# Transconnectome/multimodal_neuroimage

Hardware: NVIDIA B200
Metric: window_attn_fwd_bwd (higher is better)
Workload: dtype bf16

## Files before the change

### include/mmn_b200.h

```cpp
#ifndef MMN_B200_H_
#define MMN_B200_H_

#include <stddef.h>
#include <stdint.h>

#ifdef __cplusplus
extern "C" {
#endif

#define MMN_ABI_VERSION 6
#define MMN_WINATTN_WORK_BYTES 2048

enum { MMN_OK = 0, MMN_ERR_INVALID = -1, MMN_ERR_UNSUPPORTED = -2, MMN_ERR_CUDA = -3 };
enum { MMN_DT_F32 = 0, MMN_DT_BF16 = 1 };
enum { MMN_SCORE_SCALED = 0,
       MMN_SCORE_COSINE = 1 };
enum { MMN_MASK_NONE = 0,
       MMN_MASK_SHIFT = 1,
       MMN_MASK_TENSOR = 2,
       MMN_MASK_FUTURE = 3 };
enum { MMN_PATH_AUTO = 0, MMN_PATH_GENERIC = 1, MMN_PATH_TCGEN05 = 2 };

typedef struct mmn_winattn_desc {
  int32_t ndim;
  int32_t batch;
  int32_t grid[3];
  int32_t window[3];
  int32_t shift[3];
  int32_t num_heads, head_dim;
  int32_t score_kind;
  int32_t mask_kind;
  int32_t mask_windows;
  int32_t io_dtype;
  int32_t path;
  float scale;
  float dropout_p;
  uint64_t seed, offset;
  int64_t q_row_stride, k_row_stride, v_row_stride, o_row_stride;
  int64_t do_row_stride, dq_row_stride, dk_row_stride, dv_row_stride;
  int32_t deterministic;
  const uint64_t* rng;
} mmn_winattn_desc;

typedef struct mmn_mha_desc {
  int32_t tgt_len, src_len, batch, num_heads, head_dim;
  int32_t mask_kind;
  int32_t mask_diagonal;
  int32_t io_dtype, path;
  float scale;
  float dropout_p;
  uint64_t seed, offset;
  int64_t q_stride_t, q_stride_b, k_stride_t, k_stride_b, v_stride_t, v_stride_b;
  int64_t o_stride_t, o_stride_b;
  int64_t do_stride_t, do_stride_b, dq_stride_t, dq_stride_b, dk_stride_t, dk_stride_b;
  int64_t dv_stride_t, dv_stride_b;
  const uint64_t* rng;
} mmn_mha_desc;

int mmn_abi_version(void);
const char* mmn_last_error(void);
const char* mmn_winattn_path(const mmn_winattn_desc* desc);
const char* mmn_mha_path(const mmn_mha_desc* desc);
uint64_t mmn_launch_count(void);

int mmn_winattn_fwd(const mmn_winattn_desc* desc, const void* q, const void* k, const void* v,
                    const float* bias, const float* head_scale, const float* mask,
                    void* out, float* lse, void* workspace, int device, void* stream);

size_t mmn_winattn_bwd_workspace_bytes(const mmn_winattn_desc* desc);
int mmn_winattn_bwd(const mmn_winattn_desc* desc, const void* q, const void* k, const void* v,
                    const float* bias, const float* head_scale, const float* mask,
                    const void* out, const float* lse, const void* dout,
                    void* dq, void* dk, void* dv, float* dbias, float* dhead_scale, float* dcolsum,
                    float* workspace, int device, void* stream);

int mmn_mha_fwd(const mmn_mha_desc* desc, const void* q, const void* k, const void* v,
                const float* mask, void* out, float* lse, int device, void* stream);

int mmn_mha_bwd(const mmn_mha_desc* desc, const void* q, const void* k, const void* v,
                const float* mask, const void* out, const float* lse, const void* dout,
                void* dq, void* dk, void* dv, float* workspace ,
                int device, void* stream);

int mmn_mha_avg_weights(const mmn_mha_desc* desc, const void* q, const void* k, const float* mask,
                        const float* lse, float* avg, int device, void* stream);

size_t mmn_colsum_workspace_bytes(int64_t rows, int32_t cols);
int mmn_colsum(const void* x, int io_dtype, int64_t rows, int32_t cols, int64_t row_stride, float* out,
               float* workspace, int deterministic, int device, void* stream);

int mmn_cpb_bias_fwd(const float* coords, const float* w1, const float* b1, const float* w2, const int64_t* index,
                     int32_t T, int32_t n_in, int32_t J, int32_t num_heads, int32_t NN,
                     float* tab16, float* bias, int device, void* stream);
int mmn_cpb_bias_bwd(const float* coords, const float* w1, const float* b1, const float* w2, const int64_t* index,
                     const int32_t* inv_perm, const int32_t* inv_offsets,
                     const float* tab16, const float* dbias, int32_t T, int32_t n_in, int32_t J, int32_t num_heads, int32_t NN,
                     float* scratch, float* dw1, float* db1, float* dw2, int device, void* stream);

int mmn_table_bias_fwd(const float* table, const int64_t* index, int32_t T, int32_t num_heads, int32_t NN, float* bias,
                       int device, void* stream);
int mmn_table_bias_bwd(const float* dbias, const int64_t* index, const int32_t* inv_perm, const int32_t* inv_offsets, int32_t T,
                       int32_t num_heads, int32_t NN, float* dtable, int device, void* stream);

enum { MMN_ACT_NONE = 0, MMN_ACT_RELU = 1, MMN_ACT_GELU = 2 };
int mmn_linear_supported(int io_dtype, int64_t rows, int32_t in_features, int32_t out_features, int64_t ld_x, int64_t ld_y);
int mmn_linear_fwd(const void* x, const void* w, const float* bias, void* y, void* y_pre, int act, int io_dtype, int64_t rows,
                   int32_t in_features, int32_t out_features, int64_t ld_x, int64_t ld_y, int device, void* stream);
int mmn_linear_bwd_supported(int io_dtype, int64_t rows, int32_t in_features, int32_t out_features,
                             int64_t ld_dy, int64_t ld_x, int64_t ld_dx);
size_t mmn_linear_bwd_workspace_bytes(int64_t rows, int32_t in_features, int32_t out_features, int deterministic);
int mmn_linear_bwd(const void* dy, const void* x, const void* w, void* dx, float* dw, float* db, void* workspace,
                   const void* act_aux, int64_t ld_aux, int act, int io_dtype, int64_t rows, int32_t in_features,
                   int32_t out_features, int64_t ld_dy, int64_t ld_x, int64_t ld_dx, int deterministic, int device, void* stream);

enum { MMN_LN_PRE = 0, MMN_LN_POST = 1 };
int mmn_layernorm_supported(int32_t cols);
int mmn_layernorm_fwd(const void* resid, int resid_dtype, const void* delta, int delta_dtype, const float* gamma, const float* beta,
                      float eps, int mode, void* out_sum, int sum_dtype, void* out_norm, int norm_dtype, float* mean, float* rstd,
                      int64_t rows, int32_t cols, int device, void* stream);
size_t mmn_layernorm_bwd_workspace_bytes(int64_t rows, int32_t cols);
int mmn_layernorm_bwd(const void* g_sum, int gs_dtype, const void* g_norm, int gn_dtype, const void* x, int x_dtype,
                      const float* gamma, const float* mean, const float* rstd, int mode, void* d_resid, int dr_dtype,
                      void* d_delta, int dd_dtype, float* dgamma, float* dbeta, float* workspace, int deterministic,
                      int64_t rows, int32_t cols, int device, void* stream);

#ifdef __cplusplus
}
#endif
#endif
```

### multimodal_neuroimage_b200/_lib.py

```python
from __future__ import annotations

import ctypes as C
import os
import shutil
import subprocess
import threading

PKG_DIR = os.path.dirname(os.path.abspath(__file__))
ROOT = os.path.dirname(PKG_DIR)
CSRC = os.path.join(PKG_DIR, "csrc")
LIB_PATH = os.environ.get("MMN_LIB") or os.path.join(PKG_DIR, "libmmn_b200.so")
SOURCES = {"mmn_abi.cu": ["generic_launch.h", "attn_generic.cuh", "winattn_tc.h", "dropout_rng.cuh", "zero_fill.h"],
           "generic_launch.cu": ["generic_launch.h", "attn_generic.cuh", "dropout_rng.cuh", "zero_fill.h"],
           "winattn_tc.cu": ["winattn_tc.h", "winattn_tc_fwd.cuh", "winattn_tc_bwd.cuh", "tc_window.cuh", "tc_sched.cuh", "tc_common.cuh",
                             "zero_fill.h"],
           "linbwd_tc.cu": ["winattn_tc.h", "tc_window.cuh", "tc_common.cuh"],
           "gemm_tc.cu": ["winattn_tc.h", "tc_window.cuh", "tc_common.cuh"],
           "mha_tc.cu": ["winattn_tc.h", "tc_window.cuh", "tc_common.cuh", "dropout_rng.cuh"],
           "layernorm.cu": ["generic_launch.h", "attn_generic.cuh", "dropout_rng.cuh"],
           "cpb_bias.cu": ["generic_launch.h", "attn_generic.cuh", "dropout_rng.cuh", "zero_fill.h"]}
NVCC_FLAGS = ["-gencode", "arch=compute_100a,code=sm_100a", "-lineinfo", "-O3", "-std=c++17",
              "-Xcompiler", "-fPIC"]
if os.environ.get("MMN_BUILD_TRACE"):
    NVCC_FLAGS.append("-DMMN_TC_TRACING")
NVCC_FLAGS += os.environ.get("MMN_NVCC_DEFINES", "").split()

DT_F32, DT_BF16 = 0, 1
SCORE_SCALED, SCORE_COSINE = 0, 1
MASK_NONE, MASK_SHIFT, MASK_TENSOR, MASK_FUTURE = 0, 1, 2, 3
PATH_AUTO, PATH_GENERIC, PATH_TCGEN05 = 0, 1, 2
ACT_NONE, ACT_RELU, ACT_GELU = 0, 1, 2
LN_PRE, LN_POST = 0, 1
ABI_VERSION = 6
WINATTN_WORK_BYTES = 2048

EXPORTS = ["mmn_abi_version", "mmn_last_error", "mmn_winattn_path", "mmn_mha_path", "mmn_launch_count",
           "mmn_winattn_fwd", "mmn_winattn_bwd", "mmn_winattn_bwd_workspace_bytes", "mmn_mha_fwd", "mmn_mha_bwd", "mmn_mha_avg_weights",
           "mmn_colsum", "mmn_colsum_workspace_bytes", "mmn_layernorm_bwd_workspace_bytes",
           "mmn_linear_supported", "mmn_linear_fwd", "mmn_linear_bwd", "mmn_linear_bwd_supported", "mmn_linear_bwd_workspace_bytes",
           "mmn_cpb_bias_fwd", "mmn_cpb_bias_bwd", "mmn_table_bias_fwd", "mmn_table_bias_bwd", "mmn_layernorm_supported", "mmn_layernorm_fwd", "mmn_layernorm_bwd"]


class WinAttnDesc(C.Structure):
    _fields_ = [("ndim", C.c_int32), ("batch", C.c_int32),
                ("grid", C.c_int32 * 3), ("window", C.c_int32 * 3), ("shift", C.c_int32 * 3),
                ("num_heads", C.c_int32), ("head_dim", C.c_int32),
                ("score_kind", C.c_int32), ("mask_kind", C.c_int32), ("mask_windows", C.c_int32),
                ("io_dtype", C.c_int32), ("path", C.c_int32),
                ("scale", C.c_float), ("dropout_p", C.c_float),
                ("seed", C.c_uint64), ("offset", C.c_uint64),
                ("q_row_stride", C.c_int64), ("k_row_stride", C.c_int64), ("v_row_stride", C.c_int64),
                ("o_row_stride", C.c_int64), ("do_row_stride", C.c_int64), ("dq_row_stride", C.c_int64),
                ("dk_row_stride", C.c_int64), ("dv_row_stride", C.c_int64), ("deterministic", C.c_int32),
                ("rng", C.c_void_p)]


class MhaDesc(C.Structure):
    _fields_ = [("tgt_len", C.c_int32), ("src_len", C.c_int32), ("batch", C.c_int32),
                ("num_heads", C.c_int32), ("head_dim", C.c_int32),
                ("mask_kind", C.c_int32), ("mask_diagonal", C.c_int32),
                ("io_dtype", C.c_int32), ("path", C.c_int32),
                ("scale", C.c_float), ("dropout_p", C.c_float),
                ("seed", C.c_uint64), ("offset", C.c_uint64)] + \
               [(f"{t}_stride_{a}", C.c_int64) for t in ("q", "k", "v", "o", "do", "dq", "dk", "dv") for a in ("t", "b")] + \
               [("rng", C.c_void_p)]


def _stamp(files) -> float:
    return max(os.path.getmtime(f) for f in files if os.path.exists(f))


def build(force: bool = False, verbose: bool = False) -> str:
    nvcc = shutil.which("nvcc") or "/usr/local/cuda/bin/nvcc"
    if not os.path.exists(nvcc):
        raise RuntimeError("nvcc not found: cannot build libmmn_b200.so")
    objdir = os.path.join(PKG_DIR, "build")
    os.makedirs(objdir, exist_ok=True)
    header = os.path.join(ROOT, "include", "mmn_b200.h")
    objs, procs = [], []
    for src, deps in SOURCES.items():
        obj = os.path.join(objdir, src.replace(".cu", ".o"))
        objs.append(obj)
        stamp = _stamp([os.path.join(CSRC, src), header] + [os.path.join(CSRC, d) for d in deps])
        if force or os.environ.get("MMN_BUILD_TRACE") or os.environ.get("MMN_NVCC_DEFINES") or not os.path.exists(obj) or os.path.getmtime(obj) < stamp:
            cmd = [nvcc] + NVCC_FLAGS + ["-c", os.path.join(CSRC, src), "-o", obj]
            if verbose:
                print(" ".join(cmd), flush=True)
            procs.append((src, subprocess.Popen(cmd, stdout=subprocess.PIPE, stderr=subprocess.STDOUT, text=True)))
    for src, p in procs:
        out, _ = p.communicate()
        if p.returncode != 0:
            raise RuntimeError(f"nvcc failed on {src}:\n{out}")
    if procs or not os.path.exists(LIB_PATH) or os.path.getmtime(LIB_PATH) < _stamp(objs):
        cmd = [nvcc, "-shared", "-o", LIB_PATH + ".tmp"] + objs
        if verbose:
            print(" ".join(cmd), flush=True)
        res = subprocess.run(cmd, capture_output=True, text=True)
        if res.returncode != 0:
            raise RuntimeError("link failed:\n" + res.stdout + res.stderr)
        os.replace(LIB_PATH + ".tmp", LIB_PATH)
    return LIB_PATH


_lock = threading.Lock()
_lib = None


def load() -> C.CDLL:
    global _lib
    with _lock:
        if _lib is not None:
            return _lib
        if not os.path.exists(LIB_PATH):
            raise RuntimeError(f"{LIB_PATH} is missing: run `python -c 'import __graft_entry__ as g; g.build()'` "
                               "(multimodal_neuroimage_b200 has no CPU or PyTorch fallback)")
        lib = C.CDLL(LIB_PATH)
        vp, fp = C.c_void_p, C.c_void_p
        lib.mmn_abi_version.restype = C.c_int
        lib.mmn_last_error.restype = C.c_char_p
        lib.mmn_launch_count.restype = C.c_uint64
        lib.mmn_winattn_path.restype = C.c_char_p
        lib.mmn_winattn_path.argtypes = [C.POINTER(WinAttnDesc)]
        lib.mmn_mha_path.restype = C.c_char_p
        lib.mmn_mha_path.argtypes = [C.POINTER(MhaDesc)]
        lib.mmn_winattn_fwd.restype = C.c_int
        lib.mmn_winattn_fwd.argtypes = [C.POINTER(WinAttnDesc), vp, vp, vp, fp, fp, fp, vp, fp, vp, C.c_int, vp]
        lib.mmn_winattn_bwd_workspace_bytes.restype = C.c_size_t
        lib.mmn_winattn_bwd_workspace_bytes.argtypes = [C.POINTER(WinAttnDesc)]
        lib.mmn_winattn_bwd.restype = C.c_int
        lib.mmn_winattn_bwd.argtypes = [C.POINTER(WinAttnDesc), vp, vp, vp, fp, fp, fp, vp, fp, vp, vp, vp, vp, fp, fp, fp, fp,
                                        C.c_int, vp]
        lib.mmn_mha_fwd.restype = C.c_int
        lib.mmn_mha_fwd.argtypes = [C.POINTER(MhaDesc), vp, vp, vp, fp, vp, fp, C.c_int, vp]
        lib.mmn_mha_bwd.restype = C.c_int
        lib.mmn_mha_bwd.argtypes = [C.POINTER(MhaDesc), vp, vp, vp, fp, vp, fp, vp, vp, vp, vp, fp, C.c_int, vp]
        lib.mmn_mha_avg_weights.restype = C.c_int
        lib.mmn_mha_avg_weights.argtypes = [C.POINTER(MhaDesc), vp, vp, fp, fp, fp, C.c_int, vp]
        lib.mmn_colsum.restype = C.c_int
        lib.mmn_colsum.argtypes = [vp, C.c_int, C.c_int64, C.c_int32, C.c_int64, fp, fp, C.c_int, C.c_int, vp]
        lib.mmn_colsum_workspace_bytes.restype = C.c_size_t
        lib.mmn_colsum_workspace_bytes.argtypes = [C.c_int64, C.c_int32]
        lib.mmn_cpb_bias_fwd.restype = C.c_int
        lib.mmn_cpb_bias_fwd.argtypes = [fp, fp, fp, fp, vp, C.c_int32, C.c_int32, C.c_int32, C.c_int32, C.c_int32, fp, fp, C.c_int, vp]
        lib.mmn_table_bias_fwd.restype = C.c_int
        lib.mmn_table_bias_fwd.argtypes = [fp, vp, C.c_int32, C.c_int32, C.c_int32, fp, C.c_int, vp]
        lib.mmn_table_bias_bwd.restype = C.c_int
        lib.mmn_table_bias_bwd.argtypes = [fp, vp, vp, vp, C.c_int32, C.c_int32, C.c_int32, fp, C.c_int, vp]
        lib.mmn_cpb_bias_bwd.restype = C.c_int
        lib.mmn_cpb_bias_bwd.argtypes = [fp, fp, fp, fp, vp, vp, vp, fp, fp, C.c_int32, C.c_int32, C.c_int32, C.c_int32, C.c_int32,
                                         fp, fp, fp, fp, C.c_int, vp]
        lib.mmn_linear_bwd_supported.restype = C.c_int
        lib.mmn_linear_bwd_supported.argtypes = [C.c_int, C.c_int64, C.c_int32, C.c_int32, C.c_int64, C.c_int64, C.c_int64]
        lib.mmn_linear_bwd_workspace_bytes.restype = C.c_size_t
        lib.mmn_linear_bwd_workspace_bytes.argtypes = [C.c_int64, C.c_int32, C.c_int32, C.c_int]
        lib.mmn_linear_bwd.restype = C.c_int
        lib.mmn_linear_bwd.argtypes = [vp, vp, vp, vp, fp, fp, vp, vp, C.c_int64, C.c_int, C.c_int, C.c_int64, C.c_int32, C.c_int32,
                                       C.c_int64, C.c_int64, C.c_int64, C.c_int, C.c_int, vp]
        lib.mmn_linear_supported.restype = C.c_int
        lib.mmn_linear_supported.argtypes = [C.c_int, C.c_int64, C.c_int32, C.c_int32, C.c_int64, C.c_int64]
        lib.mmn_linear_fwd.restype = C.c_int
        lib.mmn_linear_fwd.argtypes = [vp, vp, fp, vp, vp, C.c_int, C.c_int, C.c_int64, C.c_int32, C.c_int32, C.c_int64, C.c_int64,
                                       C.c_int, vp]
        lib.mmn_layernorm_supported.restype = C.c_int
        lib.mmn_layernorm_supported.argtypes = [C.c_int32]
        lib.mmn_layernorm_fwd.restype = C.c_int
        lib.mmn_layernorm_fwd.argtypes = [vp, C.c_int, vp, C.c_int, fp, fp, C.c_float, C.c_int, vp, C.c_int, vp, C.c_int, fp, fp,
                                          C.c_int64, C.c_int32, C.c_int, vp]
        lib.mmn_layernorm_bwd.restype = C.c_int
        lib.mmn_layernorm_bwd.argtypes = [vp, C.c_int, vp, C.c_int, vp, C.c_int, fp, fp, fp, C.c_int, vp, C.c_int, vp, C.c_int, fp, fp,
                                          fp, C.c_int, C.c_int64, C.c_int32, C.c_int, vp]
        lib.mmn_layernorm_bwd_workspace_bytes.restype = C.c_size_t
        lib.mmn_layernorm_bwd_workspace_bytes.argtypes = [C.c_int64, C.c_int32]
        if lib.mmn_abi_version() != ABI_VERSION:
            raise RuntimeError("libmmn_b200.so ABI version mismatch")
        _lib = lib
        return lib


def check(rc: int, what: str) -> None:
    if rc != 0:
        msg = load().mmn_last_error().decode("utf-8", "replace")
        raise RuntimeError(f"{what} failed (code {rc}): {msg}")


def launch_count() -> int:
    return int(load().mmn_launch_count())
```

### multimodal_neuroimage_b200/csrc/mmn_abi.cu

```cuda
#include <atomic>
#include <cstdarg>
#include <cstdio>
#include <cstring>

#include "../../include/mmn_b200.h"
#include "generic_launch.h"
#include "zero_fill.h"
#include "winattn_tc.h"

namespace {

thread_local char g_err[512] = "";
std::atomic<uint64_t> g_launches{0};

int fail(int code, const char* fmt, ...) {
  va_list ap;
  va_start(ap, fmt);
  vsnprintf(g_err, sizeof(g_err), fmt, ap);
  va_end(ap);
  return code;
}

struct DeviceGuard {
  int prev = -1;
  bool ok = false;
  explicit DeviceGuard(int dev) {
    if (cudaGetDevice(&prev) != cudaSuccess) { cudaGetLastError(); return; }
    if (dev != prev && cudaSetDevice(dev) != cudaSuccess) { cudaGetLastError(); return; }
    ok = true;
  }
  ~DeviceGuard() { if (ok && prev >= 0) cudaSetDevice(prev); }
};

int finish(cudaError_t e, int launches, const char* what) {
  g_launches.fetch_add((uint64_t)launches, std::memory_order_relaxed);
  if (e != cudaSuccess) return fail(MMN_ERR_CUDA, "%s: %s", what, cudaGetErrorString(e));
  return MMN_OK;
}

int validate_win(const mmn_winattn_desc* d) {
  if (!d) return fail(MMN_ERR_INVALID, "null descriptor");
  if (d->ndim < 1 || d->ndim > 3) return fail(MMN_ERR_INVALID, "ndim %d not in 1..3", d->ndim);
  if (d->batch < 1 || d->num_heads < 1 || d->head_dim < 1) return fail(MMN_ERR_INVALID, "batch/heads/head_dim must be positive");
  for (int a = 0; a < d->ndim; ++a) {
    if (d->window[a] < 1 || d->grid[a] < 1 || d->grid[a] % d->window[a] != 0)
      return fail(MMN_ERR_INVALID, "axis %d: window %d does not divide grid %d", a, d->window[a], d->grid[a]);
    if (d->shift[a] < 0 || d->shift[a] >= d->window[a])
      return fail(MMN_ERR_INVALID, "axis %d: shift %d not in [0, window %d)", a, d->shift[a], d->window[a]);
  }
  if (d->score_kind != MMN_SCORE_SCALED && d->score_kind != MMN_SCORE_COSINE) return fail(MMN_ERR_INVALID, "bad score_kind");
  if (d->mask_kind != MMN_MASK_NONE && d->mask_kind != MMN_MASK_SHIFT && d->mask_kind != MMN_MASK_TENSOR)
    return fail(MMN_ERR_INVALID, "bad mask_kind %d for window attention", d->mask_kind);
  if (d->mask_kind == MMN_MASK_TENSOR && d->mask_windows < 1) return fail(MMN_ERR_INVALID, "mask_windows must be >= 1");
  if (d->io_dtype != MMN_DT_F32 && d->io_dtype != MMN_DT_BF16) return fail(MMN_ERR_INVALID, "bad io_dtype");
  if (d->dropout_p < 0.f || d->dropout_p >= 1.f) return fail(MMN_ERR_INVALID, "dropout_p must be in [0,1)");
  if (d->head_dim > 128) return fail(MMN_ERR_UNSUPPORTED, "head_dim %d > 128", d->head_dim);
  return MMN_OK;
}

int validate_mha(const mmn_mha_desc* d) {
  if (!d) return fail(MMN_ERR_INVALID, "null descriptor");
  if (d->tgt_len < 1 || d->src_len < 1 || d->batch < 1 || d->num_heads < 1 || d->head_dim < 1)
    return fail(MMN_ERR_INVALID, "sizes must be positive");
  if (d->mask_kind != MMN_MASK_NONE && d->mask_kind != MMN_MASK_FUTURE && d->mask_kind != MMN_MASK_TENSOR)
    return fail(MMN_ERR_INVALID, "bad mask_kind %d for multi-head attention", d->mask_kind);
  if (d->io_dtype != MMN_DT_F32 && d->io_dtype != MMN_DT_BF16) return fail(MMN_ERR_INVALID, "bad io_dtype");
  if (d->dropout_p < 0.f || d->dropout_p >= 1.f) return fail(MMN_ERR_INVALID, "dropout_p must be in [0,1)");
  if (d->head_dim > 128) return fail(MMN_ERR_UNSUPPORTED, "head_dim %d > 128", d->head_dim);
  return MMN_OK;
}

mmn::GenericProblem problem_from(const mmn_winattn_desc* d, const float* bias, const float* head_scale, const float* mask) {
  mmn::GenericProblem P{};
  P.kind = 0;
  for (int a = 0; a < 3; ++a) { P.grid[a] = 1; P.win[a] = 1; P.shift[a] = 0; P.nwin[a] = 1; }
  for (int a = 0; a < d->ndim; ++a) {
    int t = 3 - d->ndim + a;
    P.grid[t] = d->grid[a]; P.win[t] = d->window[a]; P.shift[t] = d->shift[a]; P.nwin[t] = d->grid[a] / d->window[a];
  }
  P.nW = P.nwin[0] * P.nwin[1] * P.nwin[2];
  P.nq = P.nk = P.win[0] * P.win[1] * P.win[2];
  P.d = d->head_dim; P.nH = d->num_heads;
  P.n_items = d->batch * P.nW * P.nH;
  P.q_s0 = d->q_row_stride; P.k_s0 = d->k_row_stride; P.v_s0 = d->v_row_stride; P.o_s0 = d->o_row_stride;
  P.do_s0 = d->do_row_stride; P.dq_s0 = d->dq_row_stride; P.dk_s0 = d->dk_row_stride; P.dv_s0 = d->dv_row_stride;
  P.cosine = d->score_kind == MMN_SCORE_COSINE;
  P.mask_kind = d->mask_kind; P.mask_windows = d->mask_windows > 0 ? d->mask_windows : 1;
  P.scale = d->scale; P.dropout_p = d->dropout_p; P.seed = d->seed; P.offset = d->offset;
  P.drop = mmn::make_dropout(d->dropout_p, d->seed, d->offset);
  P.rng = reinterpret_cast<const unsigned long long*>(d->rng);
  P.bias = bias; P.head_scale = head_scale; P.mask = mask;
  return P;
}

mmn::GenericProblem problem_from(const mmn_mha_desc* d, const float* mask) {
  mmn::GenericProblem P{};
  P.kind = 1;
  for (int a = 0; a < 3; ++a) { P.grid[a] = 1; P.win[a] = 1; P.shift[a] = 0; P.nwin[a] = 1; }
  P.nW = 1;
  P.nq = d->tgt_len; P.nk = d->src_len; P.d = d->head_dim; P.nH = d->num_heads;
  P.n_items = d->batch * d->num_heads;
  P.q_s0 = d->q_stride_t; P.q_s1 = d->q_stride_b; P.k_s0 = d->k_stride_t; P.k_s1 = d->k_stride_b;
  P.v_s0 = d->v_stride_t; P.v_s1 = d->v_stride_b; P.o_s0 = d->o_stride_t; P.o_s1 = d->o_stride_b;
  P.do_s0 = d->do_stride_t; P.do_s1 = d->do_stride_b; P.dq_s0 = d->dq_stride_t; P.dq_s1 = d->dq_stride_b;
  P.dk_s0 = d->dk_stride_t; P.dk_s1 = d->dk_stride_b; P.dv_s0 = d->dv_stride_t; P.dv_s1 = d->dv_stride_b;
  P.cosine = 0;
  P.mask_kind = d->mask_kind; P.mask_diag = d->mask_diagonal; P.mask_windows = 1;
  P.scale = d->scale; P.dropout_p = d->dropout_p; P.seed = d->seed; P.offset = d->offset;
  P.drop = mmn::make_dropout(d->dropout_p, d->seed, d->offset);
  P.rng = reinterpret_cast<const unsigned long long*>(d->rng);
  P.mask = mask;
  return P;
}

bool have_device() {
  int n = 0;
  if (cudaGetDeviceCount(&n) != cudaSuccess) { cudaGetLastError(); return false; }
  return n > 0;
}

}

extern "C" {

int mmn_abi_version(void) { return MMN_ABI_VERSION; }
const char* mmn_last_error(void) { return g_err; }
uint64_t mmn_launch_count(void) { return g_launches.load(std::memory_order_relaxed); }

const char* mmn_winattn_path(const mmn_winattn_desc* d) {
  if (validate_win(d) != MMN_OK) return "invalid";
  if (d->path == MMN_PATH_GENERIC) return "generic";
  return mmn::tc::fwd_why_not(d) == nullptr ? "tcgen05" : "generic";
}

const char* mmn_mha_path(const mmn_mha_desc* d) {
  if (validate_mha(d) != MMN_OK) return "invalid";
  if (d->path == MMN_PATH_GENERIC) return "generic";
  return mmn::tc::mha_why_not(d, false) == nullptr ? "tcgen05" : "generic";
}

int mmn_winattn_fwd(const mmn_winattn_desc* d, const void* q, const void* k, const void* v, const float* bias,
                    const float* head_scale, const float* mask, void* out, float* lse, void* workspace, int device,
                    void* stream) {
  int rc = validate_win(d);
  if (rc) return rc;
  if (!q || !k || !v || !out || !lse || !workspace) return fail(MMN_ERR_INVALID, "null tensor pointer");
  if (d->score_kind == MMN_SCORE_COSINE && !head_scale) return fail(MMN_ERR_INVALID, "cosine attention needs head_scale");
  if (d->mask_kind == MMN_MASK_TENSOR && !mask) return fail(MMN_ERR_INVALID, "MMN_MASK_TENSOR needs a mask");
  if (!have_device()) return fail(MMN_ERR_CUDA, "no CUDA device: libmmn_b200 has no CPU path");
  DeviceGuard g(device);
  if (!g.ok) return fail(MMN_ERR_CUDA, "cannot select device %d", device);
  cudaStream_t st = (cudaStream_t)stream;
  const char* why = mmn::tc::fwd_why_not(d);
  bool tc_ok = why == nullptr;
  if (d->path == MMN_PATH_TCGEN05 && !tc_ok) return fail(MMN_ERR_UNSUPPORTED, "shape not supported by the tcgen05 path: %s", why);
  if (d->path != MMN_PATH_GENERIC && tc_ok) {
    rc = mmn::tc::winattn_fwd(d, q, k, v, bias, head_scale, mask, out, lse, workspace, st, g_err, sizeof(g_err));
    if (rc == MMN_OK) g_launches.fetch_add(1, std::memory_order_relaxed);
    return rc;
  }
  int n = 0;
  cudaError_t e = mmn::generic_fwd(problem_from(d, bias, head_scale, mask), d->io_dtype, q, k, v, out, lse, st, &n);
  return finish(e, n, "attn_fwd_generic");
}

size_t mmn_winattn_bwd_workspace_bytes(const mmn_winattn_desc* d) {
  if (validate_win(d) != MMN_OK) return 0;
  const mmn::GenericProblem P = problem_from(d, nullptr, nullptr, nullptr);
  const size_t base = mmn::generic_bwd_workspace_floats(P, false) * sizeof(float);
  size_t bytes = base > MMN_WINATTN_WORK_BYTES ? base : MMN_WINATTN_WORK_BYTES;
  if (!d->deterministic) return bytes;
  const size_t det = d->path != MMN_PATH_GENERIC && mmn::tc::bwd_why_not(d) == nullptr ? mmn::tc::bwd_det_workspace_bytes(d)
                                                                                      : mmn::generic_bwd_workspace_floats(P, true) * sizeof(float);
  return det > bytes ? det : bytes;
}

int mmn_winattn_bwd(const mmn_winattn_desc* d, const void* q, const void* k, const void* v, const float* bias,
                    const float* head_scale, const float* mask, const void* out, const float* lse, const void* dout,
                    void* dq, void* dk, void* dv, float* dbias, float* dhead_scale, float* dcolsum, float* workspace,
                    int device, void* stream) {
  int rc = validate_win(d);
  if (rc) return rc;
  if (!q || !k || !v || !lse || !dout || !dq || !dk || !dv || !workspace) return fail(MMN_ERR_INVALID, "null tensor pointer");
  if (d->score_kind == MMN_SCORE_COSINE && !head_scale) return fail(MMN_ERR_INVALID, "cosine attention needs head_scale");
  if (d->mask_kind == MMN_MASK_TENSOR && !mask) return fail(MMN_ERR_INVALID, "MMN_MASK_TENSOR needs a mask");
  if (!have_device()) return fail(MMN_ERR_CUDA, "no CUDA device: libmmn_b200 has no CPU path");
  DeviceGuard g(device);
  if (!g.ok) return fail(MMN_ERR_CUDA, "cannot select device %d", device);
  cudaStream_t st = (cudaStream_t)stream;
  const char* why = mmn::tc::bwd_why_not(d);
  bool tc_ok = why == nullptr;
  if (d->path == MMN_PATH_TCGEN05 && !tc_ok) return fail(MMN_ERR_UNSUPPORTED, "shape not supported by the tcgen05 backward path: %s", why);
  if (d->path != MMN_PATH_GENERIC && tc_ok) {
    int n = 0;
    rc = mmn::tc::winattn_bwd(d, q, k, v, bias, head_scale, mask, out, lse, dout, dq, dk, dv, dbias, dhead_scale, dcolsum, workspace, st, g_err, sizeof(g_err), &n);
    g_launches.fetch_add((uint64_t)n, std::memory_order_relaxed);
    return rc;
  }
  mmn::GenericProblem P = problem_from(d, bias, head_scale, mask);
  int n = 0;
  cudaError_t e = mmn::generic_bwd(P, d->io_dtype, q, k, v, lse, dout, dq, dk, dv, bias ? dbias : nullptr,
                                 P.cosine ? dhead_scale : nullptr, workspace, dcolsum, d->deterministic != 0, st, &n);
  return finish(e, n, "attn_bwd_generic");
}

int mmn_mha_fwd(const mmn_mha_desc* d, const void* q, const void* k, const void* v, const float* mask, void* out,
                float* lse, int device, void* stream) {
  int rc = validate_mha(d);
  if (rc) return rc;
  if (!q || !k || !v || !out || !lse) return fail(MMN_ERR_INVALID, "null tensor pointer");
  if (d->mask_kind == MMN_MASK_TENSOR && !mask) return fail(MMN_ERR_INVALID, "MMN_MASK_TENSOR needs a mask");
  if (!have_device()) return fail(MMN_ERR_CUDA, "no CUDA device: libmmn_b200 has no CPU path");
  DeviceGuard g(device);
  if (!g.ok) return fail(MMN_ERR_CUDA, "cannot select device %d", device);
  int n = 0;
  const char* why = mmn::tc::mha_why_not(d, false);
  if (d->path == MMN_PATH_TCGEN05 && why) return fail(MMN_ERR_UNSUPPORTED, "shape not supported by the tcgen05 MHA path: %s", why);
  if (d->path != MMN_PATH_GENERIC && !why) {
    rc = mmn::tc::mha_fwd(d, q, k, v, mask, out, lse, (cudaStream_t)stream, g_err, sizeof(g_err), &n);
    g_launches.fetch_add((uint64_t)n, std::memory_order_relaxed);
    return rc;
  }
  cudaError_t e = mmn::generic_fwd(problem_from(d, mask), d->io_dtype, q, k, v, out, lse, (cudaStream_t)stream, &n);
  return finish(e, n, "attn_fwd_generic");
}

int mmn_mha_bwd(const mmn_mha_desc* d, const void* q, const void* k, const void* v, const float* mask, const void* out,
                const float* lse, const void* dout, void* dq, void* dk, void* dv, float* workspace, int device,
                void* stream) {
  int rc = validate_mha(d);
  if (rc) return rc;
  if (!q || !k || !v || !lse || !dout || !dq || !dk || !dv || !workspace) return fail(MMN_ERR_INVALID, "null tensor pointer");
  if (d->mask_kind == MMN_MASK_TENSOR && !mask) return fail(MMN_ERR_INVALID, "MMN_MASK_TENSOR needs a mask");
  if (!have_device()) return fail(MMN_ERR_CUDA, "no CUDA device: libmmn_b200 has no CPU path");
  DeviceGuard g(device);
  if (!g.ok) return fail(MMN_ERR_CUDA, "cannot select device %d", device);
  int n = 0;
  const char* why = mmn::tc::mha_why_not(d, true);
  if (d->path == MMN_PATH_TCGEN05 && why) return fail(MMN_ERR_UNSUPPORTED, "shape not supported by the tcgen05 MHA backward path: %s", why);
  if (d->path != MMN_PATH_GENERIC && !why) {
    rc = mmn::tc::mha_bwd(d, q, k, v, mask, out, lse, dout, dq, dk, dv, workspace, (cudaStream_t)stream, g_err, sizeof(g_err), &n);
    g_launches.fetch_add((uint64_t)n, std::memory_order_relaxed);
    return rc;
  }
  cudaError_t e = mmn::generic_bwd(problem_from(d, mask), d->io_dtype, q, k, v, lse, dout, dq, dk, dv, nullptr, nullptr, workspace,
                                 nullptr, false, (cudaStream_t)stream, &n);
  return finish(e, n, "attn_bwd_generic");
}

int mmn_mha_avg_weights(const mmn_mha_desc* d, const void* q, const void* k, const float* mask, const float* lse,
                        float* avg, int device, void* stream) {
  int rc = validate_mha(d);
  if (rc) return rc;
  if (!q || !k || !lse || !avg) return fail(MMN_ERR_INVALID, "null tensor pointer");
  if (!have_device()) return fail(MMN_ERR_CUDA, "no CUDA device: libmmn_b200 has no CPU path");
  DeviceGuard g(device);
  if (!g.ok) return fail(MMN_ERR_CUDA, "cannot select device %d", device);
  int n = 0;
  cudaError_t e = mmn::generic_avg_weights(problem_from(d, mask), d->io_dtype, d->batch, q, k, lse, avg, (cudaStream_t)stream, &n);
  return finish(e, n, "mha_avg_weights_generic");
}

size_t mmn_colsum_workspace_bytes(int64_t rows, int32_t cols) {
  if (rows < 1 || cols < 8 || cols % 8 != 0 || cols > 2048) return 0;
  return mmn::colsum_workspace_floats(rows, cols) * sizeof(float);
}

int mmn_colsum(const void* x, int io_dtype, int64_t rows, int32_t cols, int64_t row_stride, float* out, float* workspace,
               int deterministic, int device, void* stream) {
  if (!x || !out || rows < 0 || cols < 1) return fail(MMN_ERR_INVALID, "bad colsum arguments");
  if (deterministic && !workspace) return fail(MMN_ERR_INVALID, "deterministic colsum needs a workspace");
  if (io_dtype != MMN_DT_F32 && io_dtype != MMN_DT_BF16) return fail(MMN_ERR_INVALID, "bad io_dtype");
  if (cols % 8 != 0 || cols > 2048) return fail(MMN_ERR_UNSUPPORTED, "colsum needs cols %% 8 == 0 and cols <= 2048 (got %d)", cols);
  if (!have_device()) return fail(MMN_ERR_CUDA, "no CUDA device: libmmn_b200 has no CPU path");
  DeviceGuard g(device);
  if (!g.ok) return fail(MMN_ERR_CUDA, "cannot select device %d", device);
  if (rows == 0) return MMN_OK;
  int n = 0;
  cudaError_t e = mmn::colsum(io_dtype, x, rows, cols, row_stride, out, deterministic ? workspace : nullptr, (cudaStream_t)stream, &n);
  return finish(e, n, "colsum_kernel");
}

static int cpb_check(int T, int n_in, int J, int nH, int NN) {
  if (T < 1 || n_in < 1 || n_in > 3 || J < 1 || nH < 1 || nH > 64 || NN < 1) return fail(MMN_ERR_INVALID, "bad cpb_bias sizes");
  if ((long long)T * nH > 12288) return fail(MMN_ERR_UNSUPPORTED, "cpb_bias: T * num_heads = %lld > 12288", (long long)T * nH);
  if (mmn::cpb_bwd_smem_bytes(T) > 227 * 1024) return fail(MMN_ERR_UNSUPPORTED, "cpb_bias: table of %d entries exceeds the backward kernel's shared memory", T);
  if (!have_device()) return fail(MMN_ERR_CUDA, "no CUDA device: libmmn_b200 has no CPU path");
  return MMN_OK;
}

int mmn_table_bias_fwd(const float* table, const int64_t* index, int32_t T, int32_t nH, int32_t NN, float* bias, int device, void* stream) {
  if (!table || !index || !bias) return fail(MMN_ERR_INVALID, "null tensor pointer");
  if (T < 1 || nH < 1 || NN < 1) return fail(MMN_ERR_INVALID, "bad bias table dimensions");
  if (!have_device()) return fail(MMN_ERR_CUDA, "no CUDA device: libmmn_b200 has no CPU path");
  DeviceGuard g(device);
  if (!g.ok) return fail(MMN_ERR_CUDA, "cannot select device %d", device);
  int n = 0;
  cudaError_t e = mmn::table_bias_fwd(table, (const long long*)index, nH, NN, bias, (cudaStream_t)stream, &n);
  return finish(e, n, "table_bias_fwd");
}

int mmn_table_bias_bwd(const float* dbias, const int64_t* index, const int32_t* inv_perm, const int32_t* inv_offsets, int32_t T, int32_t nH,
                       int32_t NN, float* dtable, int device, void* stream) {
  if (!dbias || !index || !dtable) return fail(MMN_ERR_INVALID, "null tensor pointer");
  if (!inv_perm != !inv_offsets) return fail(MMN_ERR_INVALID, "inv_perm and inv_offsets go together");
  if (T < 1 || nH < 1 || NN < 1) return fail(MMN_ERR_INVALID, "bad bias table dimensions");
  if (!have_device()) return fail(MMN_ERR_CUDA, "no CUDA device: libmmn_b200 has no CPU path");
  DeviceGuard g(device);
  if (!g.ok) return fail(MMN_ERR_CUDA, "cannot select device %d", device);
  int n = 0;
  cudaError_t e = mmn::table_bias_bwd(dbias, (const long long*)index, inv_perm, inv_offsets, T, nH, NN, dtable, (cudaStream_t)stream, &n);
  return finish(e, n, "table_bias_bwd");
}

int mmn_cpb_bias_fwd(const float* coords, const float* w1, const float* b1, const float* w2, const int64_t* index, int32_t T,
                     int32_t n_in, int32_t J, int32_t nH, int32_t NN, float* tab16, float* bias, int device, void* stream) {
  if (!coords || !w1 || !b1 || !w2 || !index || !tab16 || !bias) return fail(MMN_ERR_INVALID, "null tensor pointer");
  int rc = cpb_check(T, n_in, J, nH, NN);
  if (rc) return rc;
  DeviceGuard g(device);
  if (!g.ok) return fail(MMN_ERR_CUDA, "cannot select device %d", device);
  int n = 0;
  cudaError_t e = mmn::cpb_bias_fwd(coords, w1, b1, w2, (const long long*)index, T, n_in, J, nH, NN, tab16, bias, (cudaStream_t)stream, &n);
  return finish(e, n, "cpb_bias_fwd");
}

int mmn_cpb_bias_bwd(const float* coords, const float* w1, const float* b1, const float* w2, const int64_t* index,
                     const int32_t* inv_perm, const int32_t* inv_offsets,
                     const float* tab16, const float* dbias, int32_t T, int32_t n_in, int32_t J, int32_t nH, int32_t NN,
                     float* scratch, float* dw1, float* db1, float* dw2, int device, void* stream) {
  if (!coords || !w1 || !b1 || !w2 || !index || !tab16 || !dbias || !scratch || !dw1 || !db1 || !dw2)
    return fail(MMN_ERR_INVALID, "null tensor pointer");
  if (!inv_perm != !inv_offsets) return fail(MMN_ERR_INVALID, "inv_perm and inv_offsets go together");
  int rc = cpb_check(T, n_in, J, nH, NN);
  if (rc) return rc;
  DeviceGuard g(device);
  if (!g.ok) return fail(MMN_ERR_CUDA, "cannot select device %d", device);
  int n = 0;
  cudaError_t e = mmn::cpb_bias_bwd(coords, w1, b1, w2, (const long long*)index, inv_perm, inv_offsets, tab16, dbias, T, n_in, J, nH, NN,
                                    scratch, dw1, db1, dw2, (cudaStream_t)stream, &n);
  return finish(e, n, "cpb_bias_bwd");
}

int mmn_linear_supported(int io_dtype, int64_t rows, int32_t in_features, int32_t out_features, int64_t ld_x, int64_t ld_y) {
  return have_device() && mmn::tc::linear_why_not(io_dtype, rows, in_features, out_features, ld_x, ld_y) == nullptr;
}

int mmn_linear_fwd(const void* x, const void* w, const float* bias, void* y, void* y_pre, int act, int io_dtype, int64_t rows,
                   int32_t in_features, int32_t out_features, int64_t ld_x, int64_t ld_y, int device, void* stream) {
  if (!x || !w || !y) return fail(MMN_ERR_INVALID, "null tensor pointer");
  if (act != MMN_ACT_NONE && act != MMN_ACT_RELU && act != MMN_ACT_GELU) return fail(MMN_ERR_INVALID, "bad activation %d", act);
  if (y_pre && act == MMN_ACT_NONE) return fail(MMN_ERR_INVALID, "y_pre only makes sense with an activation");
  if (!have_device()) return fail(MMN_ERR_CUDA, "no CUDA device: libmmn_b200 has no CPU path");
  const char* why = mmn::tc::linear_why_not(io_dtype, rows, in_features, out_features, ld_x, ld_y);
  if (why) return fail(MMN_ERR_UNSUPPORTED, "shape not supported by the tensor-core projection: %s", why);
  DeviceGuard g(device);
  if (!g.ok) return fail(MMN_ERR_CUDA, "cannot select device %d", device);
  int n = 0;
  int rc = mmn::tc::linear_fwd(x, w, bias, y, y_pre, act, rows, in_features, out_features, ld_x, ld_y, (cudaStream_t)stream, g_err,
                               sizeof(g_err), &n);
  g_launches.fetch_add((uint64_t)n, std::memory_order_relaxed);
  return rc;
}

static bool linbwd_fused_ok(int io_dtype, int64_t rows, int32_t in_features, int32_t out_features, int64_t ld_dy, int64_t ld_x,
                            int64_t ld_dx) {
  return mmn::tc::linbwd_why_not(io_dtype, rows, in_features, out_features, ld_dy, ld_x, ld_dx) == nullptr;
}

int mmn_linear_bwd_supported(int io_dtype, int64_t rows, int32_t in_features, int32_t out_features, int64_t ld_dy, int64_t ld_x,
                             int64_t ld_dx) {
  if (!have_device()) return 0;
  if (linbwd_fused_ok(io_dtype, rows, in_features, out_features, ld_dy, ld_x, ld_dx)) return 1;
  return mmn::tc::linear_why_not(io_dtype, rows, in_features, out_features, ld_x, ld_dy) == nullptr && ld_dx % 8 == 0;
}

size_t mmn_linear_bwd_workspace_bytes(int64_t rows, int32_t in_features, int32_t out_features, int deterministic) {
  const size_t a = mmn::tc::linbwd_workspace_bytes(out_features);
  const size_t b = mmn::tc::linear_wgrad_workspace_bytes(rows, in_features, out_features);
  size_t bytes = a > b ? a : b;
  if (deterministic && rows > 0 && out_features >= 8) {
    const size_t c = mmn::colsum_workspace_floats(rows, out_features < 2048 ? out_features : 2048) * sizeof(float);
    if (c > bytes) bytes = c;
  }
  return bytes;
}

int mmn_linear_bwd(const void* dy, const void* x, const void* w, void* dx, float* dw, float* db, void* workspace,
                   const void* act_aux, int64_t ld_aux, int act, int io_dtype, int64_t rows, int32_t in_features,
                   int32_t out_features, int64_t ld_dy, int64_t ld_x, int64_t ld_dx, int deterministic, int device, void* stream) {
  if (!dy || !w || !workspace || (!dx && !dw)) return fail(MMN_ERR_INVALID, "null tensor pointer");
  if (dw && !x) return fail(MMN_ERR_INVALID, "dw needs x");
  if (act != MMN_ACT_NONE && act != MMN_ACT_RELU && act != MMN_ACT_GELU) return fail(MMN_ERR_INVALID, "bad activation %d", act);
  if (act != MMN_ACT_NONE && (!act_aux || ld_aux % 8 || reinterpret_cast<uintptr_t>(act_aux) % 16))
    return fail(MMN_ERR_INVALID, "activation gradient needs a 16-byte aligned act'(pre) tensor");
  if (!have_device()) return fail(MMN_ERR_CUDA, "no CUDA device: libmmn_b200 has no CPU path");
  if (!mmn_linear_bwd_supported(io_dtype, rows, in_features, out_features, ld_dy, ld_x ? ld_x : in_features, ld_dx ? ld_dx : in_features))
    return fail(MMN_ERR_UNSUPPORTED, "shape not supported by the tensor-core projection backward (bf16, widths multiples of 32)");
  DeviceGuard g(device);
  if (!g.ok) return fail(MMN_ERR_CUDA, "cannot select device %d", device);
  cudaStream_t st = (cudaStream_t)stream;
  int n = 0, rc;
  if (dx && dw && act == MMN_ACT_NONE && linbwd_fused_ok(io_dtype, rows, in_features, out_features, ld_dy, ld_x, ld_dx)) {
    rc = mmn::tc::linbwd(dy, x, w, dx, dw, db, (float*)workspace, rows, in_features, out_features, ld_dy, ld_x, ld_dx, st, g_err,
                         sizeof(g_err), &n);
  } else {
    rc = mmn::tc::linear_bwd_general(dy, x, w, dx, dw, (float*)workspace, act_aux, ld_aux,
                                     act != MMN_ACT_NONE ? 3 : 0, rows, in_features, out_features, ld_dy,
                                     ld_x, ld_dx, st, g_err, sizeof(g_err), &n);
    if (rc == MMN_OK && db) {
      cudaError_t e = mmn::zero_words_async(db, (size_t)out_features, st);
      for (int c0 = 0; e == cudaSuccess && c0 < out_features; c0 += 2048)
        e = mmn::colsum(MMN_DT_BF16, static_cast<const uint16_t*>(dy) + c0, rows, out_features - c0 < 2048 ? out_features - c0 : 2048, ld_dy,
                        db + c0, deterministic ? static_cast<float*>(workspace) : nullptr, st, &n);
      if (e != cudaSuccess) { g_launches.fetch_add((uint64_t)n, std::memory_order_relaxed); return finish(e, 0, "colsum_kernel"); }
    }
  }
  g_launches.fetch_add((uint64_t)n, std::memory_order_relaxed);
  return rc;
}

int mmn_layernorm_supported(int32_t cols) { return have_device() && mmn::layernorm_supported(cols); }

static bool ln_dt_ok(int dt) { return dt == MMN_DT_F32 || dt == MMN_DT_BF16; }

int mmn_layernorm_fwd(const void* resid, int resid_dtype, const void* delta, int delta_dtype, const float* gamma, const float* beta,
                      float eps, int mode, void* out_sum, int sum_dtype, void* out_norm, int norm_dtype, float* mean, float* rstd,
                      int64_t rows, int32_t cols, int device, void* stream) {
  if ((!resid && !delta) || !gamma || !mean || !rstd || (!out_sum && !out_norm)) return fail(MMN_ERR_INVALID, "null tensor pointer");
  if (mode != MMN_LN_PRE && mode != MMN_LN_POST) return fail(MMN_ERR_INVALID, "bad layernorm mode %d", mode);
  if (mode == MMN_LN_POST && !delta) return fail(MMN_ERR_INVALID, "MMN_LN_POST normalises delta: it cannot be null");
  if (!ln_dt_ok(resid_dtype) || !ln_dt_ok(delta_dtype) || !ln_dt_ok(sum_dtype) || !ln_dt_ok(norm_dtype)) return fail(MMN_ERR_INVALID, "bad dtype");
  if (rows < 0) return fail(MMN_ERR_INVALID, "negative row count");
  if (!mmn::layernorm_supported(cols)) return fail(MMN_ERR_UNSUPPORTED, "layernorm: cols = %d (even, <= 1536)", cols);
  if (!have_device()) return fail(MMN_ERR_CUDA, "no CUDA device: libmmn_b200 has no CPU path");
  DeviceGuard g(device);
  if (!g.ok) return fail(MMN_ERR_CUDA, "cannot select device %d", device);
  if (rows == 0) return MMN_OK;
  int n = 0;
  cudaError_t e = mmn::layernorm_fwd(resid, resid_dtype, delta, delta_dtype, gamma, beta, eps, mode, out_sum, sum_dtype, out_norm, norm_dtype,
                                     mean, rstd, rows, cols, (cudaStream_t)stream, &n);
  return finish(e, n, "ln_fwd_kernel");
}

size_t mmn_layernorm_bwd_workspace_bytes(int64_t rows, int32_t cols) {
  if (rows < 1 || !mmn::layernorm_supported(cols)) return 0;
  return mmn::layernorm_bwd_workspace_floats(rows, cols) * sizeof(float);
}

int mmn_layernorm_bwd(const void* g_sum, int gs_dtype, const void* g_norm, int gn_dtype, const void* x, int x_dtype, const float* gamma,
                      const float* mean, const float* rstd, int mode, void* d_resid, int dr_dtype, void* d_delta, int dd_dtype,
                      float* dgamma, float* dbeta, float* workspace, int deterministic, int64_t rows, int32_t cols, int device,
                      void* stream) {
  if ((!g_sum && !g_norm) || !x || !gamma || !mean || !rstd) return fail(MMN_ERR_INVALID, "null tensor pointer");
  if (deterministic && (dgamma || dbeta) && !workspace) return fail(MMN_ERR_INVALID, "deterministic layernorm backward needs a workspace");
  if (mode != MMN_LN_PRE && mode != MMN_LN_POST) return fail(MMN_ERR_INVALID, "bad layernorm mode %d", mode);
  if (!ln_dt_ok(gs_dtype) || !ln_dt_ok(gn_dtype) || !ln_dt_ok(x_dtype) || !ln_dt_ok(dr_dtype) || !ln_dt_ok(dd_dtype)) return fail(MMN_ERR_INVALID, "bad dtype");
  if (!mmn::layernorm_supported(cols)) return fail(MMN_ERR_UNSUPPORTED, "layernorm: cols = %d (even, <= 1536)", cols);
  if (!have_device()) return fail(MMN_ERR_CUDA, "no CUDA device: libmmn_b200 has no CPU path");
  DeviceGuard g(device);
  if (!g.ok) return fail(MMN_ERR_CUDA, "cannot select device %d", device);
  if (rows <= 0) return MMN_OK;
  int n = 0;
  cudaError_t e = mmn::layernorm_bwd(g_sum, gs_dtype, g_norm, gn_dtype, x, x_dtype, gamma, mean, rstd, mode, d_resid, dr_dtype, d_delta,
                                     dd_dtype, dgamma, dbeta, deterministic ? workspace : nullptr, rows, cols, (cudaStream_t)stream, &n);
  return finish(e, n, "ln_bwd_kernel");
}

}
```

### multimodal_neuroimage_b200/csrc/tc_sched.cuh

```cuda
#pragma once

#include <cstdio>
#include <cstdlib>

#include "tc_window.cuh"

namespace mmn { namespace tc {

struct Sched {
  int cnt[8];
  int dim[8][4];
  int wt[8];
  int n_items;
  long long total_wt;
};

inline const int* sched_weights(bool backward) {
  static int wt[2][4] = {{16, 18, 20, 22}, {16, 18, 20, 22}};
  static std::once_flag once;
  std::call_once(once, [] {
    const char* names[2] = {"MMN_SCHED_WT_FWD", "MMN_SCHED_WT_BWD"};
    for (int k = 0; k < 2; ++k)
      if (const char* e = getenv(names[k])) {
        int w[4];
        if (sscanf(e, "%d,%d,%d,%d", &w[0], &w[1], &w[2], &w[3]) == 4 && w[0] > 0 && w[1] > 0 && w[2] > 0 && w[3] > 0)
          for (int i = 0; i < 4; ++i) wt[k][i] = w[i];
      }
  });
  return wt[backward ? 1 : 0];
}

inline Sched make_sched(const WinShape& S, int batch, bool backward) {
  const int* wts = sched_weights(backward);
  Sched sc;
  sc.n_items = 0;
  sc.total_wt = 0;
  for (int c = 0; c < 8; ++c) {
    long long n = batch;
    sc.dim[c][0] = batch;
    for (int a = 0; a < 3; ++a) {
      const int bit = (c >> a) & 1;
      const int d = S.shift[a] ? (bit ? 1 : S.nwin[a] - 1) : (bit ? 0 : S.nwin[a]);
      sc.dim[c][1 + a] = d;
      n *= d;
    }
    sc.cnt[c] = (int)n;
    sc.wt[c] = wts[__builtin_popcount(c)];
    sc.n_items += (sc.cnt[c] + 1) / 2;
    sc.total_wt += (long long)((sc.cnt[c] + 1) / 2) * sc.wt[c];
  }
  return sc;
}

__device__ __forceinline__ int sched_range_begin(const Sched& sc, int k, int G) {
  if (k >= G) return sc.n_items;
  long long target = sc.total_wt * k / G;
  int base = 0;
  for (int c = 0; c < 8; ++c) {
    const int np = (sc.cnt[c] + 1) >> 1;
    const long long cw = (long long)np * sc.wt[c];
    if (target < cw) return base + (int)(target / sc.wt[c]);
    target -= cw;
    base += np;
  }
  return sc.n_items;
}

struct ItemCursor {
  int cls, b, j0, j1, j2;
  int d0, d1, d2;
  int left;

  __device__ __forceinline__ void load_dims(const Sched& sc) {
    d0 = sc.dim[cls][1]; d1 = sc.dim[cls][2]; d2 = sc.dim[cls][3];
  }
  __device__ __forceinline__ void seek(const Sched& sc, int item) {
    cls = 0;
    while (cls < 8) {
      const int np = (sc.cnt[cls] + 1) >> 1;
      if (item < np) break;
      item -= np;
      ++cls;
    }
    if (cls == 8) { left = 0; b = j0 = j1 = j2 = 0; d0 = d1 = d2 = 1; return; }
    load_dims(sc);
    int w = 2 * item;
    left = sc.cnt[cls] - w;
    j2 = w % d2; w /= d2;
    j1 = w % d1; w /= d1;
    j0 = w % d0;
    b = w / d0;
  }
  __device__ __forceinline__ void step_window() {
    if (++j2 == d2) {
      j2 = 0;
      if (++j1 == d1) {
        j1 = 0;
        if (++j0 == d0) { j0 = 0; ++b; }
      }
    }
  }
  __device__ __forceinline__ void next_item(const Sched& sc) {
    if (left <= 2) {
      do { ++cls; } while (cls < 8 && sc.cnt[cls] == 0);
      b = j0 = j1 = j2 = 0;
      if (cls < 8) { left = sc.cnt[cls]; load_dims(sc); } else { left = 0; d0 = d1 = d2 = 1; }
    } else {
      step_window();
      step_window();
      left -= 2;
    }
  }
  __device__ __forceinline__ bool slot_valid(int slot) const { return slot == 0 || left >= 2; }
};

constexpr int kWorkDone = 511, kWorkSlotInts = 512;
struct ClassQueue {
  int cls, pend, tried;
  static __device__ __forceinline__ int chunk_of(int chunk, int c) { return max(1, chunk >> __popc(c)); }
  __device__ __forceinline__ void init(const Sched& sc, int home_item, int* work, int chunk, int lane) {
    cls = 0;
    while (cls < 7) {
      const int np = (sc.cnt[cls] + 1) >> 1;
      if (home_item < np) break;
      home_item -= np;
      ++cls;
    }
    tried = 0;
    pend = 0;
    if (lane == 0) pend = atomicAdd(work + cls, chunk_of(chunk, cls));
  }
  __device__ __forceinline__ bool next(const Sched& sc, int* work, int chunk, int lane, int& item0, int& m) {
    for (;;) {
      const int c0 = __shfl_sync(0xffffffffu, pend, 0);
      const int np = (sc.cnt[cls] + 1) >> 1;
      if (c0 < np) {
        int base = 0;
        for (int c = 0; c < cls; ++c) base += (sc.cnt[c] + 1) >> 1;
        item0 = base + c0;
        m = min(chunk_of(chunk, cls), np - c0);
        if (lane == 0) pend = atomicAdd(work + cls, chunk_of(chunk, cls));
        tried = 0;
        return true;
      }
      if (++tried >= 8) return false;
      cls = (cls + 1) & 7;
      if (lane == 0) pend = atomicAdd(work + cls, chunk_of(chunk, cls));
    }
  }
};

__device__ __forceinline__ int class_region_id(const WinShape& S, int cls, int p) {
  const int a2 = p % S.win[2]; const int t = p / S.win[2];
  const int a1 = t % S.win[1]; const int a0 = t / S.win[1];
  const int a[3] = {a0, a1, a2};
  int rid = 0;
#pragma unroll
  for (int x = 0; x < 3; ++x) rid = rid * 3 + ((cls >> x) & 1 ? (a[x] < S.win[x] - S.shift[x] ? 1 : 2) : 0);
  return rid;
}

__device__ __forceinline__ void build_class_table(float* tbl, int ld, const float* bias, const uint8_t* pos, const uint8_t* rid,
                                                  bool shift_mask, int t, int nthreads) {
  for (int e0 = t; e0 < kN * kN; e0 += 8 * nthreads) {
    float v[8];
#pragma unroll
    for (int u = 0; u < 8; ++u) {
      const int e = e0 + u * nthreads;
      v[u] = (bias && e < kN * kN) ? __ldg(bias + (int)pos[e >> 6] * kN + pos[e & 63]) : 0.f;
    }
#pragma unroll
    for (int u = 0; u < 8; ++u) {
      const int e = e0 + u * nthreads;
      if (e < kN * kN) {
        const int i = e >> 6, j = e & 63;
        if (shift_mask && rid[pos[i]] != rid[pos[j]]) v[u] -= 100.f;
        tbl[i * ld + j] = v[u] * 1.4426950408889634f;
      }
    }
  }
}

struct WinStart {
  int b, s0, s1, s2;
};

__device__ __forceinline__ WinStart cursor_start(const WinShape& S, const ItemCursor& c, int slot, int& w) {
  ItemCursor t = c;
  if (slot) t.step_window();
  const int i0 = (t.cls & 1) ? S.nwin[0] - 1 : t.j0, i1 = (t.cls & 2) ? S.nwin[1] - 1 : t.j1, i2 = (t.cls & 4) ? S.nwin[2] - 1 : t.j2;
  w = t.b * S.nW + (i0 * S.nwin[1] + i1) * S.nwin[2] + i2;
  WinStart r;
  r.b = t.b;
  r.s0 = i0 * S.win[0] + S.shift[0]; r.s1 = i1 * S.win[1] + S.shift[1]; r.s2 = i2 * S.win[2] + S.shift[2];
  return r;
}
template <int T>
struct BoxPlan {
  int cls = -1, nbox = 0;
  int slot[2], o0[2], o1[2], o2[2], dst[2];
  const CUtensorMap* map[2];

  __device__ __forceinline__ void build(const WinShape& S, int c, int lane, const CUtensorMap* const (&maps)[T], const int (&dst_base)[T],
                                        const int (&slot_stride)[T]) {
    cls = c;
    const int lp = __popc(c);
    nbox = (2 * T) << lp;
    const int psize_bytes = (kN >> lp) * 64;
#pragma unroll
    for (int r = 0; r < 2; ++r) {
      const int x = lane + 32 * r;
      const int piece = x & ((1 << lp) - 1);
      const int rest = x >> lp;
      const int sl = rest / T, t = rest - sl * T;
      int qq = piece, off[3];
#pragma unroll
      for (int a = 2; a >= 0; --a) {
        const int bit = (c >> a) & 1;
        off[a] = bit ? (qq & 1) * (S.win[a] >> 1) : 0;
        if (bit) qq >>= 1;
      }
      slot[r] = sl; o0[r] = off[0]; o1[r] = off[1]; o2[r] = off[2];
      const CUtensorMap* m = maps[0];
      int d = dst_base[0], ss = slot_stride[0];
#pragma unroll
      for (int u = 1; u < T; ++u)
        if (t == u) { m = maps[u]; d = dst_base[u]; ss = slot_stride[u]; }
      map[r] = m + c;
      dst[r] = d + sl * ss + piece * psize_bytes;
    }
  }

  template <bool LOAD>
  __device__ __forceinline__ void issue(const WinShape& S, const WinStart& w0, const WinStart& w1, int nvalid, int chan, uint8_t* stage,
                                        uint64_t* bar, int lane, int map_ofs = 0) const {
#pragma unroll
    for (int r = 0; r < 2; ++r) {
      if (lane + 32 * r < nbox && slot[r] < nvalid) {
        const WinStart& w = slot[r] ? w1 : w0;
        int c0 = w.s0 + o0[r], c1 = w.s1 + o1[r], c2 = w.s2 + o2[r];
        if (c0 >= S.grid[0]) c0 -= S.grid[0];
        if (c1 >= S.grid[1]) c1 -= S.grid[1];
        if (c2 >= S.grid[2]) c2 -= S.grid[2];
        if (LOAD) tma_load_5d(map[r] + map_ofs, bar, stage + dst[r], chan, c2, c1, c0, w.b);
        else tma_store_5d(map[r] + map_ofs, stage + dst[r], chan, c2, c1, c0, w.b);
      }
    }
  }
};

}}
```

### multimodal_neuroimage_b200/csrc/winattn_tc.cu

```cuda
#include "winattn_tc.h"

#include "winattn_tc_bwd.cuh"

namespace mmn { namespace tc {

EncodeTiledFn encode_fn() {
  static EncodeTiledFn fn = nullptr;
  static std::once_flag once;
  std::call_once(once, [] {
    void* p = nullptr;
    cudaDriverEntryPointQueryResult qr;
    if (cudaGetDriverEntryPoint("cuTensorMapEncodeTiled", &p, cudaEnableDefault, &qr) == cudaSuccess &&
        qr == cudaDriverEntryPointSuccess)
      fn = reinterpret_cast<EncodeTiledFn>(p);
    else
      cudaGetLastError();
  });
  return fn;
}

namespace {
struct MapKey {
  const void* ptr; long long row_stride; int batch, channels, grid[3], win[3];
  bool operator==(const MapKey& o) const {
    return ptr == o.ptr && row_stride == o.row_stride && batch == o.batch && channels == o.channels && grid[0] == o.grid[0] &&
           grid[1] == o.grid[1] && grid[2] == o.grid[2] && win[0] == o.win[0] && win[1] == o.win[1] && win[2] == o.win[2];
  }
};
struct MapEntry { bool valid = false; MapKey key; CUtensorMap maps[8]; };
constexpr int kMapCacheSize = 256;
std::mutex g_map_mu;
MapEntry g_map_cache[kMapCacheSize];
}

bool make_window_maps(CUtensorMap* out, const void* ptr, long long row_stride, int batch, int channels, const WinShape& g) {
  EncodeTiledFn enc = encode_fn();
  if (!enc) return false;
  if (reinterpret_cast<uintptr_t>(ptr) % 16) return false;
  MapKey key{ptr, row_stride, batch, channels, {g.grid[0], g.grid[1], g.grid[2]}, {g.win[0], g.win[1], g.win[2]}};
  const size_t hsh = (reinterpret_cast<uintptr_t>(ptr) >> 4) * 0x9E3779B97F4A7C15ull ^ (size_t)row_stride * 1315423911u ^
                     (size_t)batch * 2654435761u ^ (size_t)(g.win[0] * 31 + g.win[1] * 7 + g.win[2]);
  MapEntry& slot = g_map_cache[(hsh >> 17) % kMapCacheSize];
  std::lock_guard<std::mutex> lock(g_map_mu);
  if (slot.valid && slot.key == key) {
    for (int c = 0; c < 8; ++c) out[c] = slot.maps[c];
    return true;
  }
  cuuint64_t dims[5] = {(cuuint64_t)channels, (cuuint64_t)g.grid[2], (cuuint64_t)g.grid[1], (cuuint64_t)g.grid[0], (cuuint64_t)batch};
  cuuint64_t rs = (cuuint64_t)row_stride * 2;
  cuuint64_t strides[4] = {rs, rs * g.grid[2], rs * g.grid[2] * g.grid[1], rs * g.grid[2] * g.grid[1] * g.grid[0]};
  cuuint32_t estr[5] = {1, 1, 1, 1, 1};
  for (int cls = 0; cls < 8; ++cls) {
    cuuint32_t box[5] = {kD, (cuuint32_t)(cls & 4 ? g.win[2] / 2 : g.win[2]), (cuuint32_t)(cls & 2 ? g.win[1] / 2 : g.win[1]),
                         (cuuint32_t)(cls & 1 ? g.win[0] / 2 : g.win[0]), 1};
    for (int i = 1; i < 4; ++i) if (box[i] < 1) box[i] = 1;
    CUresult r = enc(&out[cls], CU_TENSOR_MAP_DATA_TYPE_BFLOAT16, 5, const_cast<void*>(ptr), dims, strides, box, estr,
                     CU_TENSOR_MAP_INTERLEAVE_NONE, CU_TENSOR_MAP_SWIZZLE_64B, CU_TENSOR_MAP_L2_PROMOTION_L2_128B,
                     CU_TENSOR_MAP_FLOAT_OOB_FILL_NONE);
    if (r != CUDA_SUCCESS) return false;
  }
  slot.key = key;
  for (int c = 0; c < 8; ++c) slot.maps[c] = out[c];
  slot.valid = true;
  return true;
}

const char* fwd_why_not(const mmn_winattn_desc* d) { return fwd_why_not_impl(d); }
const char* bwd_why_not(const mmn_winattn_desc* d) { return bwd_why_not_impl(d); }

int winattn_fwd(const mmn_winattn_desc* d, const void* q, const void* k, const void* v, const float* bias,
                const float* head_scale, const float* mask, void* out, float* lse, void* workspace, cudaStream_t st, char* err,
                size_t errlen) {
  return winattn_fwd_launch(d, q, k, v, bias, head_scale, mask, out, lse, workspace, st, err, errlen);
}

int winattn_bwd(const mmn_winattn_desc* d, const void* q, const void* k, const void* v, const float* bias,
                const float* head_scale, const float* mask, const void* , const float* lse, const void* dout, void* dq,
                void* dk, void* dv, float* dbias, float* dhead_scale, float* dcolsum, float* workspace, cudaStream_t st,
                char* err, size_t errlen, int* launches) {
  return winattn_bwd_launch(d, q, k, v, bias, head_scale, mask, lse, dout, dq, dk, dv, dbias, dhead_scale, dcolsum, workspace, st, err, errlen,
                            launches);
}

size_t bwd_det_workspace_bytes(const mmn_winattn_desc* d) { return bwd_det_workspace_bytes_impl(d); }

}}
```

### multimodal_neuroimage_b200/csrc/winattn_tc.h

```cpp
#pragma once
#include <cuda_runtime.h>
#include <stddef.h>

#include "../../include/mmn_b200.h"

namespace mmn { namespace tc {
const char* fwd_why_not(const mmn_winattn_desc* d);
const char* bwd_why_not(const mmn_winattn_desc* d);
int winattn_fwd(const mmn_winattn_desc* d, const void* q, const void* k, const void* v, const float* bias,
                const float* head_scale, const float* mask, void* out, float* lse, void* workspace, cudaStream_t st, char* err,
                size_t errlen);
int winattn_bwd(const mmn_winattn_desc* d, const void* q, const void* k, const void* v, const float* bias,
                const float* head_scale, const float* mask, const void* out, const float* lse, const void* dout, void* dq,
                void* dk, void* dv, float* dbias, float* dhead_scale, float* dcolsum, float* workspace, cudaStream_t st,
                char* err, size_t errlen, int* launches);
size_t bwd_det_workspace_bytes(const mmn_winattn_desc* d);
const char* linbwd_why_not(int io_dtype, long long rows, int in_features, int out_features, long long ld_dy, long long ld_x, long long ld_dx);
size_t linbwd_workspace_bytes(int out_features);
int linbwd(const void* dy, const void* x, const void* w, void* dx, float* dw, float* db, float* workspace, long long rows,
           int in_features, int out_features, long long ld_dy, long long ld_x, long long ld_dx, cudaStream_t st, char* err,
           size_t errlen, int* launches);
const char* linear_why_not(int io_dtype, long long rows, int in_features, int out_features, long long ld_x, long long ld_y);
int linear_fwd(const void* x, const void* w, const float* bias, void* y, void* y_pre, int act, long long rows, int in_features,
               int out_features, long long ld_x, long long ld_y, cudaStream_t st, char* err, size_t errlen, int* launches);
size_t linear_wgrad_workspace_bytes(long long rows, int in_features, int out_features);
int linear_bwd_general(const void* dy, const void* x, const void* w, void* dx, float* dw, float* workspace, const void* aux, long long ld_aux,
                       int act_grad, long long rows, int in_features, int out_features, long long ld_dy, long long ld_x, long long ld_dx,
                       cudaStream_t st, char* err, size_t errlen, int* launches);
const char* mha_why_not(const mmn_mha_desc* d, bool backward);
int mha_fwd(const mmn_mha_desc* d, const void* q, const void* k, const void* v, const float* mask, void* out, float* lse, cudaStream_t st,
            char* err, size_t errlen, int* launches);
int mha_bwd(const mmn_mha_desc* d, const void* q, const void* k, const void* v, const float* mask, const void* out, const float* lse,
            const void* dout, void* dq, void* dk, void* dv, float* workspace, cudaStream_t st, char* err, size_t errlen, int* launches);
}}
```

### multimodal_neuroimage_b200/csrc/winattn_tc_fwd.cuh

```cuda
#pragma once

#include <cstdio>
#include <cstdlib>
#include <mutex>

#include "tc_sched.cuh"
#include "zero_fill.h"

namespace mmn { namespace tc {

constexpr int kStagesF = 5;
constexpr int kWinBytes = 64 * 64;
constexpr int kTile = 2 * kWinBytes;
constexpr int kQRegion = 3 * kWinBytes;
constexpr int kStageBytesF = kQRegion + 2 * kTile;
constexpr int kGroupThreads = 128;
constexpr int kGroupsF = 3;
constexpr int kProducerWarp = 4 * kGroupsF, kMmaWarp = kProducerWarp + 1, kStoreWarp = kProducerWarp + 2, kProducerWarpKV = kProducerWarp + 3;
constexpr int kFwdThreads = 32 * (kProducerWarp + 4);
constexpr int kRegSoftmaxF = 136, kRegAuxF = 104;
constexpr int kTblLd = 68;
constexpr int kTmemColsF = 512;
constexpr int kTmemGroup = 160;
constexpr int kItemRing = 16;
constexpr int kChunkF = 16;
constexpr float kLog2e = 1.4426950408889634f;
constexpr float kLn2 = 0.6931471805599453f;

constexpr int kTraceCtaOfs = 5 * 32 * 16;
constexpr int kTraceWords = kTraceCtaOfs + 2 * 1024;
struct TraceCfg { long long* buf; int cta; int item0; };
__device__ __forceinline__ long long global_ns() { long long t; asm volatile("mov.u64 %0, %%globaltimer;" : "=l"(t)); return t; }

struct FwdParams {
  CUtensorMap q[8], k[8], v[8], o[8];
  WinShape S;
  Sched sc;
  int nH, per_head;
  int mask_windows;
  float scale;
  const float* bias;
  const float* head_scale;
  const float* mask;
  float* lse;
  long long slab;
  int* work;
  TraceCfg trace;
};

__device__ __forceinline__ void trace_stamp(const TraceCfg& t, int role, int item, int ev) {
  if (t.buf && (int)blockIdx.x == t.cta && (threadIdx.x & 31) == 0 && (unsigned)(item - t.item0) < 32u)
    t.buf[(role * 32 + item - t.item0) * 16 + ev] = clock64();
}
__device__ __forceinline__ void trace_cta_time(const TraceCfg& t, int which) {
  if (t.buf && threadIdx.x == 0 && blockIdx.x < 1024) t.buf[kTraceCtaOfs + 2 * blockIdx.x + which] = global_ns();
}
__device__ __forceinline__ void trace_ev(const TraceCfg& trace, int role, int item, int ev) {
#ifdef MMN_TC_TRACING
  trace_stamp(trace, role, item, ev);
#endif
}
__device__ __forceinline__ void trace_evf(const TraceCfg& trace, int role, int item, int ev) { trace_ev(trace, role, item, ev); }

__device__ __forceinline__ float row_sumsq(const uint8_t* rowp, int row) {
  const int sw = (row >> 1) & 3;
  uint64_t ss[4] = {0ull, 0ull, 0ull, 0ull};
#pragma unroll
  for (int c = 0; c < 4; ++c) {
    const uint4 a = *reinterpret_cast<const uint4*>(rowp + ((c ^ sw) << 4));
    const uint32_t u[4] = {a.x, a.y, a.z, a.w};
#pragma unroll
    for (int e = 0; e < 4; ++e) {
      const uint64_t x = pk2u(u[e] << 16, u[e] & 0xffff0000u);
      ss[c] = fma2(x, x, ss[c]);
    }
  }
  float lo, hi;
  upk2(add2(add2(ss[0], ss[1]), add2(ss[2], ss[3])), lo, hi);
  return lo + hi;
}

template <bool COS, int MASK>
__global__ void __launch_bounds__(kFwdThreads, 1)
winattn_fwd_tc_kernel(const __grid_constant__ FwdParams P) {
  constexpr int G = kGroupsF;
  extern __shared__ uint8_t smem_raw[];
  uint8_t* smem = smem_raw + ((1024u - (smem_u32(smem_raw) & 1023u)) & 1023u);
  uint8_t* sStage = smem;
  uint8_t* sO = sStage + kStagesF * kStageBytesF;
  float* sTbl = reinterpret_cast<float*>(sO + G * kTile);
  float* sRk = sTbl + G * kN * kTblLd;
  uint8_t* sPos = reinterpret_cast<uint8_t*>(sRk + G * 256);
  uint8_t* sRid = sPos + 512;
  int4* sItem = reinterpret_cast<int4*>(sRid + 512);
  int4* sGeo = sItem + kItemRing;
  int* sEnd = reinterpret_cast<int*>(sGeo + 2 * kItemRing);
  uint64_t* bars = reinterpret_cast<uint64_t*>(sEnd + 4);
  uint64_t* full = bars;
  uint64_t* empty = bars + kStagesF;
  uint64_t* s_full = bars + 2 * kStagesF;
  uint64_t* p_full = s_full + G;
  uint64_t* o_full = s_full + 2 * G;
  uint64_t* so_ready = s_full + 3 * G;
  uint64_t* so_free = s_full + 4 * G;
  uint64_t* desc_ready = s_full + 5 * G;
  uint32_t* tmem_slot = reinterpret_cast<uint32_t*>(desc_ready + kStagesF);

  const WinShape& S = P.S;
  const Sched& sc = P.sc;
  const int tid = threadIdx.x, warp = tid >> 5, lane = tid & 31;
  const int h = blockIdx.x % P.nH;

  for (int i = tid; i < (kStagesF * kStageBytesF) / 16; i += kFwdThreads)
    reinterpret_cast<uint4*>(smem)[i] = make_uint4(0, 0, 0, 0);
  for (int i = tid; i < 512; i += kFwdThreads) {
    sPos[i] = (uint8_t)piece_position(S, i >> 6, i & 63);
    sRid[i] = (uint8_t)class_region_id(S, i >> 6, i & 63);
  }
  if (tid == 0) {
    for (int g = 0; g < G; ++g) sEnd[g] = 0x7fffffff;
    for (int s = 0; s < kStagesF; ++s) { mbar_init(&full[s], 2); mbar_init(&empty[s], 1); mbar_init(&desc_ready[s], 1); }
    for (int g = 0; g < G; ++g) {
      mbar_init(&s_full[g], 1); mbar_init(&p_full[g], kGroupThreads / 32); mbar_init(&o_full[g], 1);
      mbar_init(&so_ready[g], kGroupThreads / 32); mbar_init(&so_free[g], 1);
    }
    fence_barrier_init();
  }
  if (warp == kProducerWarp && lane == 0)
    for (int i = 0; i < 8; ++i) tma_prefetch_desc(&P.q[i]);
  if (warp == kProducerWarpKV && lane == 0)
    for (int i = 0; i < 8; ++i) { tma_prefetch_desc(&P.k[i]); tma_prefetch_desc(&P.v[i]); }
  if (warp == kStoreWarp && lane == 0)
    for (int i = 0; i < 8; ++i) tma_prefetch_desc(&P.o[i]);
  if (warp == kMmaWarp) tmem_alloc<kTmemColsF>(tmem_slot);
  fence_proxy_async_smem();
  tcgen05_fence_before();
  __syncthreads();
  tcgen05_fence_after();
  const uint32_t tmem = *tmem_slot;
  trace_cta_time(P.trace, 0);

  if (warp >= kProducerWarp) {
    setmaxnreg_dec<kRegAuxF>();
    if (warp == kProducerWarp) {
      const CUtensorMap* const maps[1] = {P.q};
      const int dst_base[1] = {0};
      const int slot_stride[1] = {2 * kWinBytes};
      BoxPlan<1> plan;
      int n = 0;
      ClassQueue wq;
      const int chunk = max(1, min(kChunkF, sc.n_items / (P.per_head * 8)));
      wq.init(sc, sched_range_begin(sc, blockIdx.x / P.nH, P.per_head), P.work + h * 8, chunk, lane);
      for (int c0, m; wq.next(sc, P.work + h * 8, chunk, lane, c0, m);) {
        ItemCursor cur;
        cur.seek(sc, c0);
        for (int t = 0; t < m; ++t, ++n, cur.next_item(sc)) {
          const int stage = n % kStagesF, phase = (n / kStagesF) & 1;
          if (cur.cls != plan.cls) plan.build(S, cur.cls, lane, maps, dst_base, slot_stride);
          const int nvalid = cur.slot_valid(1) ? 2 : 1;
          int w0, w1;
          const WinStart ws0 = cursor_start(S, cur, 0, w0), ws1 = cursor_start(S, cur, 1, w1);
          trace_evf(P.trace, 2, n, 0);
          mbar_wait(&empty[stage], phase ^ 1);
          trace_evf(P.trace, 2, n, 1);
          if (lane == 0) {
            sItem[n % kItemRing] = make_int4(cur.cls, w0, w1, nvalid);
            sGeo[(n % kItemRing) * 2] = make_int4(ws0.b, ws0.s0, ws0.s1, ws0.s2);
            sGeo[(n % kItemRing) * 2 + 1] = make_int4(ws1.b, ws1.s0, ws1.s1, ws1.s2);
            mbar_arrive(&desc_ready[stage]);
            mbar_arrive_expect_tx(&full[stage], nvalid * kWinBytes);
          }
          __syncwarp();
          plan.issue<true>(S, ws0, ws1, nvalid, h * kD, sStage + stage * kStageBytesF, &full[stage], lane);
          trace_evf(P.trace, 2, n, 2);
        }
      }
      for (int e = 0; e < G; ++e, ++n) {
        const int stage = n % kStagesF, phase = (n / kStagesF) & 1;
        mbar_wait(&empty[stage], phase ^ 1);
        if (lane == 0) {
          sItem[n % kItemRing] = make_int4(-1, 0, 0, 0);
          mbar_arrive(&desc_ready[stage]);
          mbar_arrive(&full[stage]);
        }
        __syncwarp();
      }
    } else if (warp == kMmaWarp) {
      constexpr uint32_t idescS = umma_idesc_bf16(128, 64, 0, 0);
      constexpr uint32_t idescO = umma_idesc_bf16(128, 32, 0, 1);
      const uint64_t dQK = umma_smem_desc(0, 0, 512, kSwz64);
      const uint64_t dV = umma_smem_desc(0, 8192, 512, kSwz64);
      const uint32_t stage0 = smem_u32(sStage) >> 4;
      int total = 0x7fffffff;
      int ns = 0, np = 0;
      uint32_t idle = 0;
      while (np < total) {
        bool progressed = false;
        if (total == 0x7fffffff && ns < np + G) {
          const int stage = ns % kStagesF, phase = (ns / kStagesF) & 1;
          if (mbar_test(&full[stage], phase)) {
            progressed = true;
            if (sItem[ns % kItemRing].x < 0) {
              total = ns;
            } else {
              tcgen05_fence_after();
              if (elect_one()) {
                const uint64_t aq = dQK + (stage0 + stage * (kStageBytesF >> 4)), bk = aq + (kQRegion >> 4);
                const uint32_t tS = tmem + (ns % G) * kTmemGroup;
#pragma unroll
                for (int ks = 0; ks < 4; ++ks)
                  umma_bf16_ss(tS, aq + ((ks >> 1) * (kWinBytes >> 4) + (ks & 1) * 2), bk + ((ks >> 1) * (kWinBytes >> 4) + (ks & 1) * 2), idescS, ks);
                umma_commit(&s_full[ns % G]);
              }
              __syncwarp();
              ++ns;
            }
          }
        }
        if (np < ns) {
          const int g = np % G, kk = np / G, stage = np % kStagesF;
          if (mbar_test(&p_full[g], kk & 1)) {
            progressed = true;
            trace_evf(P.trace, 3, np, 1);
            tcgen05_fence_after();
            if (elect_one()) {
              const uint32_t tP = tmem + g * kTmemGroup + 64, tO = tmem + g * kTmemGroup + 128;
              const uint64_t bv = dV + (stage0 + stage * (kStageBytesF >> 4) + ((kQRegion + kTile) >> 4));
#pragma unroll
              for (int ks = 0; ks < 8; ++ks)
                umma_bf16_ts(tO, tP + ks * 8, bv + ks * (1024 >> 4), idescO, ks);
              umma_commit(&o_full[g]);
              umma_commit(&empty[stage]);
            }
            __syncwarp();
            trace_evf(P.trace, 3, np, 2);
            ++np;
          }
        }
        if (progressed) idle = 0;
        else if (++idle > (1u << 24)) __trap();
      }
    } else if (warp == kStoreWarp) {
      const CUtensorMap* const maps[1] = {P.o};
      const int dst_base[1] = {0};
      const int slot_stride[1] = {kWinBytes};
      BoxPlan<1> plan;
      int n = 0;
      for (;; ++n) {
        const int g = n % G, kk = n / G;
        trace_evf(P.trace, 4, n, 0);
        mbar_wait(&so_ready[g], kk & 1);
        if (kk >= *reinterpret_cast<volatile int*>(&sEnd[g])) break;
        trace_evf(P.trace, 4, n, 1);
        const int4 item = sItem[n % kItemRing], a0 = sGeo[(n % kItemRing) * 2], a1 = sGeo[(n % kItemRing) * 2 + 1];
        if (item.x != plan.cls) plan.build(S, item.x, lane, maps, dst_base, slot_stride);
        WinStart w0, w1;
        w0.b = a0.x; w0.s0 = a0.y; w0.s1 = a0.z; w0.s2 = a0.w;
        w1.b = a1.x; w1.s0 = a1.y; w1.s1 = a1.z; w1.s2 = a1.w;
        plan.issue<false>(S, w0, w1, item.w, h * kD, sO + g * kTile, nullptr, lane);
        tma_store_commit();
        tma_store_wait_read<1>();
        __syncwarp();
        if (lane == 0 && n > 0) mbar_arrive(&so_free[(n - 1) % G]);
        trace_evf(P.trace, 4, n, 2);
      }
      tma_store_wait_read<0>();
      __syncwarp();
      if (lane == 0 && n > 0) mbar_arrive(&so_free[(n - 1) % G]);
      tma_store_wait_all<0>();
    } else {
      const CUtensorMap* const maps[2] = {P.k, P.v};
      const int dst_base[2] = {kQRegion, kQRegion + kTile};
      const int slot_stride[2] = {kWinBytes, kWinBytes};
      BoxPlan<2> plan;
      int ends = 0;
      for (int n = 0; ends < G; ++n) {
        const int stage = n % kStagesF, phase = (n / kStagesF) & 1;
        mbar_wait(&desc_ready[stage], phase);
        const int4 item = sItem[n % kItemRing], a0 = sGeo[(n % kItemRing) * 2], a1 = sGeo[(n % kItemRing) * 2 + 1];
        if (item.x < 0) {
          if (lane == 0) mbar_arrive(&full[stage]);
          __syncwarp();
          ++ends;
          continue;
        }
        if (item.x != plan.cls) plan.build(S, item.x, lane, maps, dst_base, slot_stride);
        WinStart w0, w1;
        w0.b = a0.x; w0.s0 = a0.y; w0.s1 = a0.z; w0.s2 = a0.w;
        w1.b = a1.x; w1.s0 = a1.y; w1.s1 = a1.z; w1.s2 = a1.w;
        if (lane == 0) mbar_arrive_expect_tx(&full[stage], item.w * 2 * kWinBytes);
        __syncwarp();
        plan.issue<true>(S, w0, w1, item.w, h * kD, sStage + stage * kStageBytesF, &full[stage], lane);
      }
    }
  } else {
    setmaxnreg_inc<kRegSoftmaxF>();
    const int g = warp >> 2;
    const int r = tid & 127;
    const int slot = r >> 6, i = r & 63;
    const uint32_t lane_base = (uint32_t)((warp & 3) * 32) << 16;
    const uint32_t tS = tmem + lane_base + g * kTmemGroup, tP = tS + 64 + slot * 32, tO = tS + 128;
    const float hscale = COS ? __ldg(P.head_scale + h) * kLog2e : P.scale * kLog2e;
    float* tbl = sTbl + g * kN * kTblLd;
    uint8_t* obuf = sO + g * kTile + r * 64;
    const float* bias_h = P.bias ? P.bias + (size_t)h * kN * kN : nullptr;
    const int trole = (warp & 3) == 0 && g < 2 ? g : -1;
#define TR(item, ev) do { if (trole >= 0) trace_evf(P.trace, trole, item, ev); } while (0)

    {
      uint32_t z[32];
#pragma unroll
      for (int j = 0; j < 32; ++j) z[j] = 0u;
      tmem_st_32x32b_x32(tS + 64, z);
      tmem_st_32x32b_x32(tS + 96, z);
      tmem_st_wait();
    }

    int cls_loaded = -1;
    int kk = 0;
    for (int n = g;; n += G, ++kk) {
      const int stage = n % kStagesF, phase = (n / kStagesF) & 1;
      TR(n, 0);
      mbar_wait(&full[stage], phase);
      const int4 item = sItem[n % kItemRing];
      if (item.x < 0) break;
      const int cls = item.x, gw = slot ? item.z : item.y;
      const bool valid = slot < item.w;
      if (cls != cls_loaded) {
        named_bar_sync(1 + g, kGroupThreads);
        build_class_table(tbl, kTblLd, bias_h, sPos + cls * 64, sRid + cls * 64, MASK == MMN_MASK_SHIFT && cls != 0, r, kGroupThreads);
        cls_loaded = cls;
      }
      const int ipos = sPos[cls * 64 + i];
      const int gwh = gw * P.nH + h;
      const uint8_t* base = sStage + stage * kStageBytesF;
      float* rkbuf = sRk + (g * 2 + (kk & 1)) * 128;
      TR(n, 1);
      float a_i = hscale;
      if (COS) {
        const float ssq = row_sumsq(base + slot * 2 * kWinBytes + i * 64, i);
        const float ssk = row_sumsq(base + kQRegion + r * 64, i);
        const float rq = rsqrtf(fmaxf(ssq, 1e-24f)), rkk = rsqrtf(fmaxf(ssk, 1e-24f));
        a_i *= rq;
        rkbuf[r] = rkk;
        if (valid) {
          float* rec = P.lse + P.slab + (long long)gwh * (3 * kN) + i;
          rec[0] = rq;
          rec[kN] = rkk;
        }
      }
      named_bar_sync(1 + g, kGroupThreads);
      TR(n, 2);

      mbar_wait(&s_full[g], kk & 1);
      tcgen05_fence_after();
      TR(n, 3);
      uint64_t s2[32];
      {
        uint32_t raw0[32], raw1[32];
        tmem_ld_32x32b_x32(tS, raw0);
        tmem_ld_32x32b_x32(tS + 32, raw1);
        tmem_ld_wait();
#pragma unroll
        for (int j = 0; j < 16; ++j) { s2[j] = pk2u(raw0[2 * j], raw0[2 * j + 1]); s2[16 + j] = pk2u(raw1[2 * j], raw1[2 * j + 1]); }
      }
      TR(n, 4);
      {
        const float4* trow = reinterpret_cast<const float4*>(tbl + i * kTblLd);
        const float4* krow = reinterpret_cast<const float4*>(rkbuf + slot * 64);
        const float* mrow = (MASK == MMN_MASK_TENSOR) ? P.mask + ((size_t)(gw % P.mask_windows) * kN + ipos) * kN : nullptr;
        const uint64_t a2 = pk2(a_i, a_i);
#pragma unroll
        for (int j4 = 0; j4 < 16; ++j4) {
          float4 tt = trow[j4];
          if (MASK == MMN_MASK_TENSOR) {
            const float4 mm = __ldg(reinterpret_cast<const float4*>(mrow) + j4);
            tt.x = fmaf(mm.x, kLog2e, tt.x); tt.y = fmaf(mm.y, kLog2e, tt.y); tt.z = fmaf(mm.z, kLog2e, tt.z); tt.w = fmaf(mm.w, kLog2e, tt.w);
          }
          if (COS) {
            const float4 kv = krow[j4];
            s2[j4 * 2 + 0] = fma2(s2[j4 * 2 + 0], mul2(pk2(kv.x, kv.y), a2), pk2(tt.x, tt.y));
            s2[j4 * 2 + 1] = fma2(s2[j4 * 2 + 1], mul2(pk2(kv.z, kv.w), a2), pk2(tt.z, tt.w));
          } else {
            s2[j4 * 2 + 0] = fma2(s2[j4 * 2 + 0], a2, pk2(tt.x, tt.y));
            s2[j4 * 2 + 1] = fma2(s2[j4 * 2 + 1], a2, pk2(tt.z, tt.w));
          }
        }
      }
      float mx;
      {
        float m8[8];
#pragma unroll
        for (int j = 0; j < 4; ++j) upk2(s2[j], m8[2 * j], m8[2 * j + 1]);
#pragma unroll
        for (int j = 4; j < 32; j += 2) {
          float a, b, c, d;
          upk2(s2[j], a, b); upk2(s2[j + 1], c, d);
          const int ch = (j >> 1) & 7;
          m8[ch] = fmaxf(fmaxf(m8[ch], a), b);
          m8[(ch + 4) & 7] = fmaxf(fmaxf(m8[(ch + 4) & 7], c), d);
        }
        mx = fmaxf(fmaxf(fmaxf(m8[0], m8[1]), fmaxf(m8[2], m8[3])), fmaxf(fmaxf(m8[4], m8[5]), fmaxf(m8[6], m8[7])));
      }
      uint32_t pp[32];
      float l;
      {
        const uint64_t nmx2 = pk2(-mx, -mx);
        uint64_t l2[4] = {0ull, 0ull, 0ull, 0ull};
#pragma unroll
        for (int j = 0; j < 32; ++j) {
          float a, b;
          upk2(add2(s2[j], nmx2), a, b);
          a = fast_exp2(a); b = fast_exp2(b);
          l2[j & 3] = add2(l2[j & 3], pk2(a, b));
          pp[j] = valid ? pack_bf16x2(a, b) : 0u;
        }
        float la, lb;
        upk2(add2(add2(l2[0], l2[1]), add2(l2[2], l2[3])), la, lb);
        l = la + lb;
      }
      TR(n, 5);
      tmem_st_32x32b_x32(tP, pp);
      tmem_st_wait();
      tcgen05_fence_before();
      mbar_arrive_warp(&p_full[g]);
      TR(n, 6);

      const float lse2 = mx + __log2f(l), inv_l = __frcp_rn(l);
      if (valid) {
        P.lse[(long long)gwh * kN + ipos] = lse2 * kLn2;
        P.lse[P.slab + (long long)gwh * (3 * kN) + 2 * kN + i] = lse2;
      }

      mbar_wait(&o_full[g], kk & 1);
      tcgen05_fence_after();
      TR(n, 7);
      uint32_t oraw[32];
      tmem_ld_32x32b_x32(tO, oraw);
      tmem_ld_wait();
      tcgen05_fence_before();
      mbar_wait(&so_free[g], (kk & 1) ^ 1);
      const uint64_t inv2 = pk2(inv_l, inv_l);
#pragma unroll
      for (int c = 0; c < 4; ++c) {
        uint4 v4 = make_uint4(pack_bf16x2(mul2(pk2u(oraw[c * 8 + 0], oraw[c * 8 + 1]), inv2)), pack_bf16x2(mul2(pk2u(oraw[c * 8 + 2], oraw[c * 8 + 3]), inv2)),
                              pack_bf16x2(mul2(pk2u(oraw[c * 8 + 4], oraw[c * 8 + 5]), inv2)), pack_bf16x2(mul2(pk2u(oraw[c * 8 + 6], oraw[c * 8 + 7]), inv2)));
        *reinterpret_cast<uint4*>(obuf + ((c ^ ((r >> 1) & 3)) << 4)) = v4;
      }
      fence_proxy_async_smem();
      mbar_arrive_warp(&so_ready[g]);
      TR(n, 8);
    }
    if (kk > 0) mbar_wait(&so_free[g], (kk - 1) & 1);
    if (r == 0) sEnd[g] = kk;
    mbar_arrive_warp(&so_ready[g]);
#undef TR
  }

  tcgen05_fence_before();
  __syncthreads();
  trace_cta_time(P.trace, 1);
  if (warp == kMmaWarp) tmem_dealloc<kTmemColsF>(tmem);
}

constexpr size_t kFwdSmemBytes = 1024  + kStagesF * kStageBytesF + kGroupsF * kTile + kGroupsF * kN * kTblLd * 4 +
                                 kGroupsF * 256 * 4 + 1024 + kItemRing * 48 + 16 + (3 * kStagesF + 5 * kGroupsF + 1) * 8;

inline const char* fwd_why_not_impl(const mmn_winattn_desc* d) {
  if (d->io_dtype != MMN_DT_BF16) return "io dtype is not bf16";
  if (d->head_dim != kD) return "head_dim != 32";
  if (d->num_heads * 8 > kWorkDone) return "more than 63 heads";
  if (d->dropout_p > 0.f) return "attention dropout is only implemented in the generic path";
  WinShape g = shape_from(d);
  if (g.win[0] * g.win[1] * g.win[2] != kN) return "window does not hold 64 tokens";
  for (int a = 0; a < 3; ++a)
    if (g.shift[a] != 0 && (2 * g.shift[a] != g.win[a] || g.nwin[a] < 2)) return "shift is neither 0 nor window/2";
  if (d->mask_kind == MMN_MASK_TENSOR && (g.shift[0] | g.shift[1] | g.shift[2])) return "mask tensor together with a cyclic shift";
  if (d->q_row_stride % 8 || d->k_row_stride % 8 || d->v_row_stride % 8 || d->o_row_stride % 8) return "row stride not 16-byte aligned";
  if (!encode_fn()) return "cuTensorMapEncodeTiled unavailable";
  return nullptr;
}

inline void dump_trace(long long* dev, const char* path, cudaStream_t st) {
  static long long host[kTraceWords];
  cudaStreamSynchronize(st);
  cudaMemcpy(host, dev, sizeof(host), cudaMemcpyDeviceToHost);
  cudaFree(dev);
  if (FILE* f = fopen(path, "w")) {
    for (int role = 0; role < 5; ++role)
      for (int item = 0; item < 32; ++item) {
        fprintf(f, "%d %d", role, item);
        for (int ev = 0; ev < 16; ++ev) fprintf(f, " %lld", host[(role * 32 + item) * 16 + ev]);
        fprintf(f, "\n");
      }
    for (int cta = 0; cta < 1024; ++cta)
      if (host[kTraceCtaOfs + 2 * cta]) fprintf(f, "cta %d %lld %lld\n", cta, host[kTraceCtaOfs + 2 * cta], host[kTraceCtaOfs + 2 * cta + 1]);
    fclose(f);
  }
}
inline TraceCfg trace_setup(const char* path, cudaStream_t st) {
  TraceCfg t{nullptr, 0, 0};
  if (path && *path) {
    cudaMalloc(&t.buf, kTraceWords * sizeof(long long));
    cudaMemsetAsync(t.buf, 0, kTraceWords * sizeof(long long), st);
    const char* cta = getenv("MMN_TC_TRACE_CTA");
    const char* it0 = getenv("MMN_TC_TRACE_ITEM0");
    t.cta = cta ? atoi(cta) : 0;
    t.item0 = it0 ? atoi(it0) : 0;
  }
  return t;
}

inline int* arm_work_counters(void* workspace, cudaStream_t st, char* err, size_t errlen) {
  if (!workspace || reinterpret_cast<uintptr_t>(workspace) % 4) { snprintf(err, errlen, "workspace missing or misaligned"); return nullptr; }
  if (mmn::zero_words_async(workspace, kWorkSlotInts, st) != cudaSuccess) {
    snprintf(err, errlen, "zeroing the work counters: %s", cudaGetErrorString(cudaGetLastError()));
    return nullptr;
  }
  return static_cast<int*>(workspace);
}

inline int winattn_fwd_launch(const mmn_winattn_desc* d, const void* q, const void* k, const void* v, const float* bias,
                              const float* head_scale, const float* mask, void* out, float* lse, void* workspace, cudaStream_t st,
                              char* err, size_t errlen) {
  FwdParams P;
  P.S = shape_from(d);
  P.sc = make_sched(P.S, d->batch, false);
  const int C = d->num_heads * d->head_dim;
  if (!make_window_maps(P.q, q, d->q_row_stride, d->batch, C, P.S) || !make_window_maps(P.k, k, d->k_row_stride, d->batch, C, P.S) ||
      !make_window_maps(P.v, v, d->v_row_stride, d->batch, C, P.S) || !make_window_maps(P.o, out, d->o_row_stride, d->batch, C, P.S)) {
    snprintf(err, errlen, "cuTensorMapEncodeTiled failed (pointer alignment or strides)");
    return MMN_ERR_CUDA;
  }
  P.nH = d->num_heads;
  P.mask_windows = d->mask_windows > 0 ? d->mask_windows : 1;
  P.scale = d->scale;
  P.bias = bias; P.head_scale = head_scale; P.mask = mask; P.lse = lse;
  P.slab = (long long)P.S.n_windows * d->num_heads * kN;
  P.work = arm_work_counters(workspace, st, err, errlen);
  if (!P.work) return MMN_ERR_CUDA;
  const char* trace_path = getenv("MMN_TC_TRACE");
  P.trace = trace_setup(trace_path, st);

  using Kern = void (*)(const FwdParams);
  static const Kern kernels[2][3] = {
      {winattn_fwd_tc_kernel<false, MMN_MASK_NONE>, winattn_fwd_tc_kernel<false, MMN_MASK_SHIFT>, winattn_fwd_tc_kernel<false, MMN_MASK_TENSOR>},
      {winattn_fwd_tc_kernel<true, MMN_MASK_NONE>, winattn_fwd_tc_kernel<true, MMN_MASK_SHIFT>, winattn_fwd_tc_kernel<true, MMN_MASK_TENSOR>}};
  static std::once_flag once;
  std::call_once(once, [] {
    for (int c = 0; c < 2; ++c)
      for (int m = 0; m < 3; ++m) cudaFuncSetAttribute(kernels[c][m], cudaFuncAttributeMaxDynamicSharedMemorySize, (int)kFwdSmemBytes);
  });
  const Kern kern = kernels[d->score_kind == MMN_SCORE_COSINE ? 1 : 0][d->mask_kind];
  int per_head = num_sms_cached() / P.nH;
  if (per_head < 1) per_head = 1;
  if (per_head > P.sc.n_items) per_head = P.sc.n_items;
  P.per_head = per_head;
  kern<<<per_head * P.nH, kFwdThreads, kFwdSmemBytes, st>>>(P);
  cudaError_t e = cudaGetLastError();
  if (e != cudaSuccess) {
    snprintf(err, errlen, "winattn_fwd_tc_kernel: %s", cudaGetErrorString(e));
    return MMN_ERR_CUDA;
  }
  if (P.trace.buf) dump_trace(P.trace.buf, trace_path, st);
  return MMN_OK;
}

}}
```

### multimodal_neuroimage_b200/fused.py

```python
from __future__ import annotations

from typing import Optional

import torch
import torch.nn.functional as F

from . import _lib, ops


def _mm_f32(a: torch.Tensor, b: torch.Tensor) -> torch.Tensor:
    if a.dtype == torch.float32:
        return a @ b
    try:
        return torch.mm(a, b, out_dtype=torch.float32)
    except TypeError:
        return (a @ b).float()


def _project(x2: torch.Tensor, w: torch.Tensor, b) -> torch.Tensor:
    if ops.linear_supported(x2, w):
        return torch.ops.mmn_b200.linear_fwd(x2, w, None if b is None else b.float(), _lib.ACT_NONE, False)[0]
    return F.linear(x2, w, None if b is None else b.to(x2.dtype))


class WindowAttentionModuleFn(torch.autograd.Function):
    @staticmethod
    def forward(ctx, x, y, w_a, b_a, w_b, b_b, w_proj, b_proj, bias, head_scale, grid, window, shift, num_heads,
                score_kind, mask_kind, scale, dropout, path):
        odt = torch.get_autocast_dtype("cuda") if torch.is_autocast_enabled("cuda") else x.dtype
        cdt = torch.bfloat16 if odt == torch.float16 else odt
        B, L, C = x.shape
        with torch.autocast("cuda", enabled=False):
            cast = lambda t: None if t is None else t.to(cdt)
            xc, yc = cast(x).reshape(B * L, C), (cast(y).reshape(B * L, C) if y is not None else None)
            castw = (lambda t: None if t is None else ops.weight_bf16(t)) if cdt == torch.bfloat16 else cast
            wa, wb, wp = castw(w_a), castw(w_b), castw(w_proj)
            a = _project(xc, wa, b_a).view(B, *grid, -1)
            b = _project(yc, wb, b_b).view(B, *grid, -1) if y is not None else None
            p, seed, off, rng = dropout
            out, lse = torch.ops.mmn_b200.winattn_fwd(a, b, bias, head_scale, None, list(grid), list(window), list(shift),
                                                      num_heads, score_kind, mask_kind, scale, p, seed, off, path, rng)
            res = _project(out.view(B * L, C), wp, b_proj).view(B, L, C).to(odt)
        ctx.save_for_backward(xc, yc, a, b, out, lse, wa, wb, wp, bias, head_scale, rng)
        ctx.cfg = (list(grid), list(window), list(shift), num_heads, score_kind, mask_kind, scale, p, seed, off, path)
        ctx.meta = (x.dtype, None if y is None else y.dtype, w_a.dtype, None if b_a is None else b_a.dtype,
                    None if w_b is None else w_b.dtype, None if b_b is None else b_b.dtype, w_proj.dtype,
                    None if b_proj is None else b_proj.dtype, (B, L, C))
        return res

    @staticmethod
    @torch.autograd.function.once_differentiable
    def backward(ctx, dres):
        xc, yc, a, b, out, lse, wa, wb, wp, bias, head_scale, rng = ctx.saved_tensors
        xdt, ydt, wadt, badt, wbdt, bbdt, wpdt, bpdt, (B, L, C) = ctx.meta
        with torch.autocast("cuda", enabled=False):
            dy = dres.to(xc.dtype).reshape(B * L, C)
            if not dy.is_contiguous():
                dy = dy.contiguous()
            out2 = out.view(B * L, C)
            if ops.linear_bwd_supported(dy, out2, wp):
                dout2, d_wp, d_bp = torch.ops.mmn_b200.linear_bwd(dy, out2, wp)
                dout = dout2.view(out.shape)
                d_wp = d_wp.to(wpdt)
                d_bp = d_bp.to(bpdt) if bpdt is not None else None
            else:
                d_bp = None
                if bpdt is not None:
                    d_bp = (torch.ops.mmn_b200.colsum(dy) if C % 8 == 0 and C <= 2048 else dy.float().sum(0)).to(bpdt)
                d_wp = _mm_f32(dy.t(), out2).to(wpdt)
                dout = (dy @ wp).view(out.shape)
            da, db, dbias, dhs, dcs = torch.ops.mmn_b200.winattn_bwd(dout, a, b, bias, head_scale, None, out, lse, *ctx.cfg,
                                                                     True, rng)
            da2 = da.view(B * L, -1)
            if ops.linear_bwd_supported(da2, xc, wa):
                dx, d_wa, _ = torch.ops.mmn_b200.linear_bwd(da2, xc, wa)
                dx, d_wa = dx.view(B, L, C).to(xdt), d_wa.to(wadt)
            else:
                d_wa = _mm_f32(da2.t(), xc).to(wadt)
                dx = (da2 @ wa).view(B, L, C).to(xdt)
            if b is None:
                d_ba = dcs.reshape(-1).to(badt) if badt is not None else None
                d_y = d_wb = d_bb = None
            else:
                db2 = db.view(B * L, -1)
                d_ba = dcs[0].to(badt) if badt is not None else None
                d_bb = dcs[1:].reshape(-1).to(bbdt) if bbdt is not None else None
                if ops.linear_bwd_supported(db2, yc, wb):
                    d_y, d_wb, _ = torch.ops.mmn_b200.linear_bwd(db2, yc, wb)
                    d_y, d_wb = d_y.view(B, L, C).to(ydt), d_wb.to(wbdt)
                else:
                    d_wb = _mm_f32(db2.t(), yc).to(wbdt)
                    d_y = (db2 @ wb).view(B, L, C).to(ydt)
        return (dx, d_y, d_wa, d_ba, d_wb, d_bb, d_wp, d_bp, dbias if bias is not None else None,
                dhs if head_scale is not None else None) + (None,) * 9


def window_attention_module(x: torch.Tensor, y: Optional[torch.Tensor], w_a, b_a, w_b, b_b, w_proj, b_proj, bias, head_scale,
                            grid, window, shift, num_heads: int, score_kind: int, mask_kind: int, scale: float,
                            dropout=(0.0, 0, 0, None), path: int = 0) -> torch.Tensor:
    return WindowAttentionModuleFn.apply(x, y, w_a, b_a, w_b, b_b, w_proj, b_proj, bias, head_scale, tuple(grid), tuple(window),
                                         tuple(shift), num_heads, score_kind, mask_kind, float(scale), dropout, path)


class MlpFn(torch.autograd.Function):

    @staticmethod
    def forward(ctx, x, w1, b1, w2, b2, act):
        x2 = x.reshape(-1, x.shape[-1])
        w1c, w2c = ops.weight_bf16(w1), ops.weight_bf16(w2)
        h, dact = torch.ops.mmn_b200.linear_fwd(x2, w1c, None if b1 is None else b1.float(), act, True)
        y, _ = torch.ops.mmn_b200.linear_fwd(h, w2c, None if b2 is None else b2.float(), _lib.ACT_NONE, False)
        ctx.save_for_backward(x2, dact, h, w1c, w2c)
        ctx.meta = (x.shape, w1.dtype, None if b1 is None else b1.dtype, w2.dtype, None if b2 is None else b2.dtype, act,
                    x.requires_grad)
        return y.view(*x.shape[:-1], w2.shape[0])

    @staticmethod
    @torch.autograd.function.once_differentiable
    def backward(ctx, dy):
        x2, dact, h, w1c, w2c = ctx.saved_tensors
        shape, w1dt, b1dt, w2dt, b2dt, act, need_dx = ctx.meta
        dy2 = dy.reshape(-1, dy.shape[-1]).to(torch.bfloat16)
        if not dy2.is_contiguous():
            dy2 = dy2.contiguous()
        dpre, dw2, db2 = torch.ops.mmn_b200.linear_bwd(dy2, h, w2c, dact, act, True, True)
        dx, dw1, db1 = torch.ops.mmn_b200.linear_bwd(dpre, x2, w1c, None, 0, need_dx, True)
        return (dx.view(shape) if need_dx else None, dw1.to(w1dt), db1.to(b1dt) if b1dt is not None else None, dw2.to(w2dt),
                db2.to(b2dt) if b2dt is not None else None, None)


def mlp(x: torch.Tensor, fc1: torch.nn.Linear, fc2: torch.nn.Linear, act: str, drop: float = 0.0, training: bool = False,
        drop_out=None):
    drop_out = drop if drop_out is None else drop_out
    cdt = torch.get_autocast_dtype("cuda") if torch.is_autocast_enabled("cuda") else x.dtype
    odt = cdt
    if cdt == torch.float16:
        cdt = torch.bfloat16
    widths_ok = all(d % 32 == 0 for d in (fc1.in_features, fc1.out_features, fc2.out_features))
    if x.is_cuda and cdt == torch.bfloat16 and widths_ok and x.numel() > 0 and not (training and (drop > 0.0 or drop_out > 0.0)):
        with torch.autocast("cuda", enabled=False):
            xc = x.to(torch.bfloat16)
            if not xc.is_contiguous():
                xc = xc.contiguous()
            return MlpFn.apply(xc, fc1.weight, fc1.bias, fc2.weight, fc2.bias, ops._ACT[act]).to(odt)
    h = fc1(x)
    h = F.gelu(h) if act == "gelu" else F.relu(h)
    h = F.dropout(h, drop, training)
    return F.dropout(fc2(h), drop_out, training)


def _ln_ok(x: torch.Tensor, ln) -> bool:
    return (isinstance(ln, torch.nn.LayerNorm) and ln.weight is not None and len(ln.normalized_shape) == 1
            and ops.layernorm_supported(x, x.shape[-1]) and ln.normalized_shape[0] == x.shape[-1])


def _act_dtype(x: torch.Tensor):
    if torch.is_autocast_enabled("cuda"):
        dt = torch.get_autocast_dtype("cuda")
        return torch.bfloat16 if dt == torch.float16 else dt
    return x.dtype


def layer_norm(x: torch.Tensor, ln, out_dtype=None) -> torch.Tensor:
    if not _ln_ok(x, ln):
        return ln(x)
    out_dtype = out_dtype or _act_dtype(x)
    with torch.autocast("cuda", enabled=False):
        return ops.AddLayerNormFn.apply(x, None, ln.weight, ln.bias, ln.eps, _lib.LN_PRE, out_dtype)[1]


def add_layer_norm(resid: torch.Tensor, delta: torch.Tensor, ln, out_dtype=None):
    if not _ln_ok(resid, ln) or delta.dtype not in (torch.float32, torch.bfloat16) or delta.shape != resid.shape:
        s = resid + delta
        return s, ln(s)
    out_dtype = out_dtype or _act_dtype(resid)
    with torch.autocast("cuda", enabled=False):
        return ops.AddLayerNormFn.apply(resid, delta, ln.weight, ln.bias, ln.eps, _lib.LN_PRE, out_dtype)


def post_norm_add(resid: torch.Tensor, delta: torch.Tensor, ln, copy_dtype=None):
    if not _ln_ok(resid, ln) or delta.dtype not in (torch.float32, torch.bfloat16) or delta.shape != resid.shape:
        s = resid + ln(delta)
        return s, (s.to(copy_dtype) if copy_dtype is not None else None)
    with torch.autocast("cuda", enabled=False):
        return ops.AddLayerNormFn.apply(resid, delta, ln.weight, ln.bias, ln.eps, _lib.LN_POST, copy_dtype)


PARALLEL_BRANCHES = False
_side_streams = {}


def parallel(fn_a, fn_b, ref: torch.Tensor, inputs_b=()):
    if not (PARALLEL_BRANCHES and ref.is_cuda):
        return fn_a(), fn_b()
    cur = torch.cuda.current_stream(ref.device)
    side = _side_streams.get(ref.device.index)
    if side is None:
        side = _side_streams[ref.device.index] = torch.cuda.Stream(ref.device)
    side.wait_stream(cur)
    for t in inputs_b:
        if isinstance(t, torch.Tensor):
            t.record_stream(side)
    with torch.cuda.stream(side):
        b = fn_b()
    a = fn_a()
    cur.wait_stream(side)
    for t in (b if isinstance(b, (tuple, list)) else (b,)):
        if isinstance(t, torch.Tensor):
            t.record_stream(cur)
    return a, b
```

### multimodal_neuroimage_b200/ops.py

```python
from __future__ import annotations

import ctypes as C
from typing import List, Optional, Tuple

import torch

from . import _lib, geometry
from ._lib import MhaDesc, WinAttnDesc

Tensor = torch.Tensor

_DT = {torch.float32: _lib.DT_F32, torch.bfloat16: _lib.DT_BF16}


def kernel_io(t: Optional[Tensor]) -> Optional[Tensor]:
    return t.to(torch.bfloat16) if t is not None and t.dtype == torch.float16 else t


_BF16_SHADOWS = {}


def weight_bf16(w: Tensor) -> Tensor:
    if w.dtype == torch.bfloat16:
        return w
    hit = _BF16_SHADOWS.get(id(w))
    if hit is not None and hit[0]() is w and hit[2] == w._version:
        return hit[1]
    return w.to(torch.bfloat16)


class Bf16Shadows:

    def __init__(self, params):
        import weakref
        self._ref = weakref.ref
        self.src = [p for p in params if p.dtype == torch.float32 and p.dim() >= 2]
        self.dst = [torch.empty_like(p, dtype=torch.bfloat16) for p in self.src]
        self.refresh()

    def refresh(self):
        if not self.src:
            return
        with torch.no_grad():
            torch._foreach_copy_(self.dst, self.src)
        for p, d in zip(self.src, self.dst):
            key = id(p)
            _BF16_SHADOWS[key] = (self._ref(p, lambda _r, key=key: _BF16_SHADOWS.pop(key, None)), d, p._version)

    def close(self):
        for p in self.src:
            hit = _BF16_SHADOWS.get(id(p))
            if hit is not None and hit[0]() is p:
                del _BF16_SHADOWS[id(p)]
        self.src, self.dst = [], []


def _require_cuda(*ts):
    for t in ts:
        if t is not None and not t.is_cuda:
            raise RuntimeError("multimodal_neuroimage_b200 ops run on CUDA tensors only (there is no CPU path); "
                               f"got a tensor on {t.device}")


def _ptr(t: Optional[Tensor], elem_offset: int = 0):
    if t is None:
        return None
    return C.c_void_p(t.data_ptr() + elem_offset * t.element_size())


def _row_stride(t: Tensor) -> int:
    if t.stride(-1) != 1:
        raise RuntimeError("channel dimension must be contiguous")
    rs = t.stride(-2)
    exp = rs
    for i in range(t.dim() - 2, -1, -1):
        if t.shape[i] != 1 and t.stride(i) != exp:
            raise RuntimeError(f"token rows are not uniformly strided: shape {tuple(t.shape)} strides {t.stride()}")
        exp *= t.shape[i]
    return rs


def _stream(t: Tensor):
    return C.c_void_p(torch.cuda.current_stream(t.device).cuda_stream)


def _deterministic() -> bool:
    return torch.are_deterministic_algorithms_enabled()


def _workspace(nbytes: int, like: Tensor) -> Tensor:
    return torch.empty((nbytes + 3) // 4, dtype=torch.float32, device=like.device)


_INVERSE = {}


def _inverse_index(index: Tensor, T: int) -> Tuple[Tensor, Tensor]:
    key = (index.device, index.data_ptr(), index.numel(), index._version, T)
    hit = _INVERSE.get(key)
    if hit is not None:
        return hit[1], hit[2]
    perm, offsets = geometry.inverse_index(index.reshape(-1), T)
    if not torch.cuda.is_current_stream_capturing():
        _INVERSE[key] = (index, perm, offsets)
    return perm, offsets


KERNEL_EVENTS = None


class _timed:
    def __init__(self, name, t):
        self.name, self.t = name, t

    def __enter__(self):
        if KERNEL_EVENTS is not None:
            self.e0 = torch.cuda.Event(enable_timing=True)
            self.e1 = torch.cuda.Event(enable_timing=True)
            self.e0.record(torch.cuda.current_stream(self.t.device))

    def __exit__(self, *exc):
        if KERNEL_EVENTS is not None:
            self.e1.record(torch.cuda.current_stream(self.t.device))
            KERNEL_EVENTS.setdefault(self.name, []).append((self.e0, self.e1))
        return False


def _rng_ptr(rng: Optional[Tensor], like: Tensor) -> Optional[int]:
    if rng is None:
        return None
    if rng.dtype != torch.int64 or rng.numel() != 2 or not rng.is_contiguous() or rng.device != like.device:
        raise RuntimeError("rng must be a contiguous (2,) int64 tensor {seed, offset} on the attention's device")
    return rng.data_ptr()


def _win_desc(a: Tensor, b: Optional[Tensor], grid, window, shift, num_heads, score_kind, mask_kind, mask_windows,
              scale, dropout_p, seed, offset, path, rng=None) -> Tuple[WinAttnDesc, int]:
    n = len(grid)
    if a.dtype not in _DT:
        raise RuntimeError(f"unsupported dtype {a.dtype}: the window-attention kernels take float32 or bfloat16")
    Cc = a.shape[-1] // 3 if b is None else a.shape[-1]
    if Cc % num_heads:
        raise RuntimeError("channels not divisible by heads")
    d = WinAttnDesc()
    d.ndim, d.batch = n, a.shape[0]
    for i in range(n):
        d.grid[i], d.window[i], d.shift[i] = int(grid[i]), int(window[i]), int(shift[i])
    d.num_heads, d.head_dim = num_heads, Cc // num_heads
    d.score_kind, d.mask_kind, d.mask_windows = score_kind, mask_kind, mask_windows
    d.io_dtype, d.path = _DT[a.dtype], path
    d.scale, d.dropout_p, d.seed, d.offset = scale, dropout_p, seed, offset
    d.rng = _rng_ptr(rng, a)
    return d, Cc


@torch.library.custom_op("mmn_b200::winattn_fwd", mutates_args=())
def winattn_fwd(a: Tensor, b: Optional[Tensor], bias: Optional[Tensor], head_scale: Optional[Tensor],
                mask: Optional[Tensor], grid: List[int], window: List[int], shift: List[int], num_heads: int,
                score_kind: int, mask_kind: int, scale: float, dropout_p: float, seed: int, offset: int,
                path: int, rng: Optional[Tensor] = None) -> Tuple[Tensor, Tensor]:
    _require_cuda(a, b, bias, head_scale, mask)
    lib = _lib.load()
    d, Cc = _win_desc(a, b, grid, window, shift, num_heads, score_kind, mask_kind,
                      mask.shape[0] if mask is not None else 0, scale, dropout_p, seed, offset, path, rng)
    if tuple(a.shape[1:-1]) != tuple(grid):
        raise RuntimeError(f"tensor grid {tuple(a.shape[1:-1])} != geometry {tuple(grid)}")
    out = torch.empty(*a.shape[:-1], Cc, dtype=a.dtype, device=a.device)
    N = 1
    nW = 1
    for g, w in zip(grid, window):
        N *= w
        nW *= g // w
    lse = torch.empty(4, a.shape[0] * nW, num_heads, N, dtype=torch.float32, device=a.device)
    if b is None:
        q, k, v = _ptr(a), _ptr(a, Cc), _ptr(a, 2 * Cc)
        d.q_row_stride = d.k_row_stride = d.v_row_stride = _row_stride(a)
    else:
        q, k, v = _ptr(a), _ptr(b), _ptr(b, Cc)
        d.q_row_stride = _row_stride(a)
        d.k_row_stride = d.v_row_stride = _row_stride(b)
    d.o_row_stride = Cc
    for t in (bias, head_scale, mask):
        if t is not None and (t.dtype != torch.float32 or not t.is_contiguous()):
            raise RuntimeError("bias / head_scale / mask must be contiguous float32")
    work = torch.empty(_lib.WINATTN_WORK_BYTES, dtype=torch.uint8, device=a.device)
    with _timed("winattn_fwd", a):
        _lib.check(lib.mmn_winattn_fwd(C.byref(d), q, k, v, _ptr(bias), _ptr(head_scale), _ptr(mask), _ptr(out),
                                       _ptr(lse), _ptr(work), a.device.index, _stream(a)), "mmn_winattn_fwd")
    return out, lse


@winattn_fwd.register_fake
def _(a, b, bias, head_scale, mask, grid, window, shift, num_heads, score_kind, mask_kind, scale, dropout_p, seed,
      offset, path, rng=None):
    Cc = a.shape[-1] // 3 if b is None else a.shape[-1]
    N = nW = 1
    for g, w in zip(grid, window):
        N *= w
        nW *= g // w
    return a.new_empty(*a.shape[:-1], Cc), a.new_empty(4, a.shape[0] * nW, num_heads, N, dtype=torch.float32)


@torch.library.custom_op("mmn_b200::winattn_bwd", mutates_args=())
def winattn_bwd(dout: Tensor, a: Tensor, b: Optional[Tensor], bias: Optional[Tensor], head_scale: Optional[Tensor],
                mask: Optional[Tensor], out: Tensor, lse: Tensor, grid: List[int], window: List[int], shift: List[int],
                num_heads: int, score_kind: int, mask_kind: int, scale: float, dropout_p: float, seed: int,
                offset: int, path: int, want_colsum: bool = False,
                rng: Optional[Tensor] = None) -> Tuple[Tensor, Tensor, Tensor, Tensor, Tensor]:
    _require_cuda(dout, a, b, bias, head_scale, mask, out, lse)
    lib = _lib.load()
    d, Cc = _win_desc(a, b, grid, window, shift, num_heads, score_kind, mask_kind,
                      mask.shape[0] if mask is not None else 0, scale, dropout_p, seed, offset, path, rng)
    dout = dout.contiguous()
    da = torch.empty(a.shape, dtype=a.dtype, device=a.device)
    db = torch.empty(b.shape, dtype=b.dtype, device=b.device) if b is not None else a.new_empty(0)
    if b is None:
        q, k, v = _ptr(a), _ptr(a, Cc), _ptr(a, 2 * Cc)
        dq, dk, dv = _ptr(da), _ptr(da, Cc), _ptr(da, 2 * Cc)
        d.q_row_stride = d.k_row_stride = d.v_row_stride = _row_stride(a)
        d.dq_row_stride = d.dk_row_stride = d.dv_row_stride = 3 * Cc
    else:
        q, k, v = _ptr(a), _ptr(b), _ptr(b, Cc)
        dq, dk, dv = _ptr(da), _ptr(db), _ptr(db, Cc)
        d.q_row_stride = _row_stride(a)
        d.k_row_stride = d.v_row_stride = _row_stride(b)
        d.dq_row_stride = Cc
        d.dk_row_stride = d.dv_row_stride = 2 * Cc
    d.o_row_stride = _row_stride(out)
    d.do_row_stride = Cc
    d.deterministic = int(_deterministic())
    dbias = torch.zeros_like(bias) if bias is not None else a.new_empty(0, dtype=torch.float32)
    dhs = torch.zeros_like(head_scale) if head_scale is not None else a.new_empty(0, dtype=torch.float32)
    ws = _workspace(lib.mmn_winattn_bwd_workspace_bytes(C.byref(d)), lse)
    dcs = torch.zeros(3, Cc, dtype=torch.float32, device=a.device) if want_colsum else a.new_empty(0, dtype=torch.float32)
    with _timed("winattn_bwd", a):
        _lib.check(lib.mmn_winattn_bwd(C.byref(d), q, k, v, _ptr(bias), _ptr(head_scale), _ptr(mask), _ptr(out), _ptr(lse),
                                       _ptr(dout), dq, dk, dv, _ptr(dbias) if bias is not None else None,
                                       _ptr(dhs) if head_scale is not None else None, _ptr(dcs) if want_colsum else None,
                                       _ptr(ws), a.device.index, _stream(a)), "mmn_winattn_bwd")
    return da, db, dbias, dhs, dcs


@winattn_bwd.register_fake
def _(dout, a, b, bias, head_scale, mask, out, lse, grid, window, shift, num_heads, score_kind, mask_kind, scale,
      dropout_p, seed, offset, path, want_colsum=False, rng=None):
    Cc = a.shape[-1] // 3 if b is None else a.shape[-1]
    return (torch.empty_like(a), torch.empty_like(b) if b is not None else a.new_empty(0),
            torch.empty_like(bias) if bias is not None else a.new_empty(0, dtype=torch.float32),
            torch.empty_like(head_scale) if head_scale is not None else a.new_empty(0, dtype=torch.float32),
            a.new_empty((3, Cc) if want_colsum else (0,), dtype=torch.float32))


def _winattn_setup(ctx, inputs, output):
    (a, b, bias, head_scale, mask, grid, window, shift, num_heads, score_kind, mask_kind, scale, dropout_p, seed,
     offset, path, rng) = inputs
    out, lse = output
    ctx.save_for_backward(a, b, bias, head_scale, mask, out, lse, rng)
    ctx.cfg = (grid, window, shift, num_heads, score_kind, mask_kind, scale, dropout_p, seed, offset, path)


def _winattn_backward(ctx, dout, dlse):
    a, b, bias, head_scale, mask, out, lse, rng = ctx.saved_tensors
    da, db, dbias, dhs, _ = torch.ops.mmn_b200.winattn_bwd(dout, a, b, bias, head_scale, mask, out, lse, *ctx.cfg, False, rng)
    return (da, db if b is not None else None, dbias if bias is not None else None,
            dhs if head_scale is not None else None, None) + (None,) * 12


torch.library.register_autograd("mmn_b200::winattn_fwd", _winattn_backward, setup_context=_winattn_setup)


def _tb_strides(t: Tensor) -> Tuple[int, int]:
    if t.dim() != 3 or t.stride(2) != 1:
        raise RuntimeError("expected a (len, batch, embed) tensor with contiguous embed dimension")
    return t.stride(0), t.stride(1)


def _mha_desc(q, k, num_heads, mask_kind, mask_diag, scale, dropout_p, seed, offset, rng=None) -> MhaDesc:
    if q.dtype not in _DT:
        raise RuntimeError(f"unsupported dtype {q.dtype}: the attention kernels take float32 or bfloat16")
    d = MhaDesc()
    d.tgt_len, d.batch, E = q.shape
    d.src_len = k.shape[0]
    if E % num_heads:
        raise RuntimeError("embed_dim not divisible by heads")
    d.num_heads, d.head_dim = num_heads, E // num_heads
    d.mask_kind, d.mask_diagonal = mask_kind, mask_diag
    d.io_dtype, d.path = _DT[q.dtype], _lib.PATH_AUTO
    d.scale, d.dropout_p, d.seed, d.offset = scale, dropout_p, seed, offset
    d.rng = _rng_ptr(rng, q)
    return d


@torch.library.custom_op("mmn_b200::mha_fwd", mutates_args=())
def mha_fwd(q: Tensor, k: Tensor, v: Tensor, mask: Optional[Tensor], num_heads: int, mask_kind: int, mask_diag: int,
            scale: float, dropout_p: float, seed: int, offset: int, rng: Optional[Tensor] = None) -> Tuple[Tensor, Tensor]:
    _require_cuda(q, k, v, mask)
    lib = _lib.load()
    d = _mha_desc(q, k, num_heads, mask_kind, mask_diag, scale, dropout_p, seed, offset, rng)
    out = torch.empty(q.shape, dtype=q.dtype, device=q.device)
    lse = torch.empty(q.shape[1] * num_heads, q.shape[0], dtype=torch.float32, device=q.device)
    d.q_stride_t, d.q_stride_b = _tb_strides(q)
    d.k_stride_t, d.k_stride_b = _tb_strides(k)
    d.v_stride_t, d.v_stride_b = _tb_strides(v)
    d.o_stride_t, d.o_stride_b = _tb_strides(out)
    if mask is not None and (mask.dtype != torch.float32 or not mask.is_contiguous()):
        raise RuntimeError("attn_mask must be contiguous float32")
    with _timed("mha_fwd", q):
        _lib.check(lib.mmn_mha_fwd(C.byref(d), _ptr(q), _ptr(k), _ptr(v), _ptr(mask), _ptr(out), _ptr(lse), q.device.index,
                                   _stream(q)), "mmn_mha_fwd")
    return out, lse


@mha_fwd.register_fake
def _(q, k, v, mask, num_heads, mask_kind, mask_diag, scale, dropout_p, seed, offset, rng=None):
    return torch.empty_like(q, memory_format=torch.contiguous_format), q.new_empty(q.shape[1] * num_heads, q.shape[0],
                                                                                    dtype=torch.float32)


@torch.library.custom_op("mmn_b200::mha_bwd", mutates_args=())
def mha_bwd(dout: Tensor, q: Tensor, k: Tensor, v: Tensor, mask: Optional[Tensor], out: Tensor, lse: Tensor,
            num_heads: int, mask_kind: int, mask_diag: int, scale: float, dropout_p: float, seed: int,
            offset: int, rng: Optional[Tensor] = None) -> Tuple[Tensor, Tensor, Tensor]:
    _require_cuda(dout, q, k, v, mask, out, lse)
    lib = _lib.load()
    d = _mha_desc(q, k, num_heads, mask_kind, mask_diag, scale, dropout_p, seed, offset, rng)
    dout = dout.contiguous()
    dq = torch.empty(q.shape, dtype=q.dtype, device=q.device)
    dk = torch.empty(k.shape, dtype=k.dtype, device=k.device)
    dv = torch.empty(v.shape, dtype=v.dtype, device=v.device)
    d.q_stride_t, d.q_stride_b = _tb_strides(q)
    d.k_stride_t, d.k_stride_b = _tb_strides(k)
    d.v_stride_t, d.v_stride_b = _tb_strides(v)
    d.o_stride_t, d.o_stride_b = _tb_strides(out)
    d.do_stride_t, d.do_stride_b = _tb_strides(dout)
    d.dq_stride_t, d.dq_stride_b = _tb_strides(dq)
    d.dk_stride_t, d.dk_stride_b = _tb_strides(dk)
    d.dv_stride_t, d.dv_stride_b = _tb_strides(dv)
    ws = lse.new_empty(2 * lse.shape[0] * ((lse.shape[1] + 127) // 128 * 128))
    with _timed("mha_bwd", q):
        _lib.check(lib.mmn_mha_bwd(C.byref(d), _ptr(q), _ptr(k), _ptr(v), _ptr(mask), _ptr(out), _ptr(lse), _ptr(dout),
                                   _ptr(dq), _ptr(dk), _ptr(dv), _ptr(ws), q.device.index, _stream(q)), "mmn_mha_bwd")
    return dq, dk, dv


@mha_bwd.register_fake
def _(dout, q, k, v, mask, out, lse, num_heads, mask_kind, mask_diag, scale, dropout_p, seed, offset, rng=None):
    c = torch.contiguous_format
    return torch.empty_like(q, memory_format=c), torch.empty_like(k, memory_format=c), torch.empty_like(v, memory_format=c)


def _mha_setup(ctx, inputs, output):
    q, k, v, mask, num_heads, mask_kind, mask_diag, scale, dropout_p, seed, offset, rng = inputs
    out, lse = output
    ctx.save_for_backward(q, k, v, mask, out, lse, rng)
    ctx.cfg = (num_heads, mask_kind, mask_diag, scale, dropout_p, seed, offset)


def _mha_backward(ctx, dout, dlse):
    q, k, v, mask, out, lse, rng = ctx.saved_tensors
    dq, dk, dv = torch.ops.mmn_b200.mha_bwd(dout, q, k, v, mask, out, lse, *ctx.cfg, rng)
    return (dq, dk, dv, None) + (None,) * 8


torch.library.register_autograd("mmn_b200::mha_fwd", _mha_backward, setup_context=_mha_setup)


@torch.library.custom_op("mmn_b200::mha_avg_weights", mutates_args=())
def mha_avg_weights(q: Tensor, k: Tensor, mask: Optional[Tensor], lse: Tensor, num_heads: int, mask_kind: int,
                    mask_diag: int, scale: float, dropout_p: float, seed: int, offset: int,
                    rng: Optional[Tensor] = None) -> Tensor:
    _require_cuda(q, k, mask, lse)
    lib = _lib.load()
    d = _mha_desc(q, k, num_heads, mask_kind, mask_diag, scale, dropout_p, seed, offset, rng)
    d.q_stride_t, d.q_stride_b = _tb_strides(q)
    d.k_stride_t, d.k_stride_b = _tb_strides(k)
    avg = torch.empty(q.shape[1], q.shape[0], k.shape[0], dtype=torch.float32, device=q.device)
    _lib.check(lib.mmn_mha_avg_weights(C.byref(d), _ptr(q), _ptr(k), _ptr(mask), _ptr(lse), _ptr(avg), q.device.index,
                                       _stream(q)), "mmn_mha_avg_weights")
    return avg


@mha_avg_weights.register_fake
def _(q, k, mask, lse, num_heads, mask_kind, mask_diag, scale, dropout_p, seed, offset, rng=None):
    return q.new_empty(q.shape[1], q.shape[0], k.shape[0], dtype=torch.float32)


@torch.library.custom_op("mmn_b200::colsum", mutates_args=())
def colsum(x: Tensor) -> Tensor:
    _require_cuda(x)
    if x.dim() != 2 or x.stride(1) != 1 or x.dtype not in _DT:
        raise RuntimeError("colsum expects a 2-D float32/bfloat16 tensor with contiguous columns")
    out = torch.zeros(x.shape[1], dtype=torch.float32, device=x.device)
    lib, det = _lib.load(), _deterministic()
    ws = _workspace(lib.mmn_colsum_workspace_bytes(x.shape[0], x.shape[1]), x) if det else None
    with _timed("colsum", x):
        _lib.check(lib.mmn_colsum(_ptr(x), _DT[x.dtype], x.shape[0], x.shape[1], x.stride(0), _ptr(out), _ptr(ws), int(det),
                                  x.device.index, _stream(x)), "mmn_colsum")
    return out


@colsum.register_fake
def _(x):
    return x.new_empty(x.shape[1], dtype=torch.float32)


@torch.library.custom_op("mmn_b200::table_bias_fwd", mutates_args=())
def table_bias_fwd(table: Tensor, index: Tensor) -> Tensor:
    _require_cuda(table, index)
    if table.dim() != 2 or table.dtype != torch.float32 or not table.is_contiguous() or index.dtype != torch.int64 or \
            not index.is_contiguous():
        raise RuntimeError("table_bias_fwd expects a contiguous fp32 (T, heads) table and a contiguous int64 index")
    T, nH, NN = table.shape[0], table.shape[1], index.numel()
    bias = torch.empty(nH, NN, dtype=torch.float32, device=table.device)
    _lib.check(_lib.load().mmn_table_bias_fwd(_ptr(table), _ptr(index), T, nH, NN, _ptr(bias), table.device.index, _stream(table)),
               "mmn_table_bias_fwd")
    return bias


@table_bias_fwd.register_fake
def _(table, index):
    return table.new_empty(table.shape[1], index.numel())


@torch.library.custom_op("mmn_b200::table_bias_bwd", mutates_args=())
def table_bias_bwd(dbias: Tensor, index: Tensor, table_rows: int) -> Tensor:
    _require_cuda(dbias, index)
    dbias = dbias.contiguous()
    nH, NN = dbias.shape[0], index.numel()
    dtable = torch.empty(table_rows, nH, dtype=torch.float32, device=dbias.device)
    perm, offsets = _inverse_index(index, table_rows) if _deterministic() else (None, None)
    _lib.check(_lib.load().mmn_table_bias_bwd(_ptr(dbias), _ptr(index), _ptr(perm), _ptr(offsets), table_rows, nH, NN, _ptr(dtable),
                                             dbias.device.index, _stream(dbias)), "mmn_table_bias_bwd")
    return dtable


@table_bias_bwd.register_fake
def _(dbias, index, table_rows):
    return dbias.new_empty(table_rows, dbias.shape[0])


def _table_bias_setup(ctx, inputs, output):
    table, index = inputs
    ctx.save_for_backward(index)
    ctx.rows = table.shape[0]


def _table_bias_backward(ctx, dbias):
    index, = ctx.saved_tensors
    return torch.ops.mmn_b200.table_bias_bwd(dbias.float().reshape(dbias.shape[0], -1), index, ctx.rows), None


torch.library.register_autograd("mmn_b200::table_bias_fwd", _table_bias_backward, setup_context=_table_bias_setup)


def cpb_bias_supported(coords: Tensor, w1: Tensor, w2: Tensor) -> bool:
    ok = coords.is_cuda and all(t.dtype == torch.float32 for t in (coords, w1, w2))
    T = coords.numel() // coords.shape[-1]
    return bool(ok and coords.shape[-1] <= 3 and w2.shape[0] <= 64 and T * w2.shape[0] <= 12288 and (11 * T + 4100) * 4 <= 227 * 1024)


@torch.library.custom_op("mmn_b200::cpb_bias_fwd", mutates_args=())
def cpb_bias_fwd(coords: Tensor, w1: Tensor, b1: Tensor, w2: Tensor, index: Tensor) -> Tuple[Tensor, Tensor]:
    _require_cuda(coords, w1, b1, w2, index)
    T, n_in, J, nH, NN = coords.shape[0], coords.shape[1], w1.shape[0], w2.shape[0], index.numel()
    tab16 = torch.empty(T, nH, dtype=torch.float32, device=coords.device)
    bias = torch.empty(nH, NN, dtype=torch.float32, device=coords.device)
    _lib.check(_lib.load().mmn_cpb_bias_fwd(_ptr(coords), _ptr(w1), _ptr(b1), _ptr(w2), _ptr(index), T, n_in, J, nH, NN,
                                           _ptr(tab16), _ptr(bias), coords.device.index, _stream(coords)), "mmn_cpb_bias_fwd")
    return bias, tab16


@cpb_bias_fwd.register_fake
def _(coords, w1, b1, w2, index):
    return (coords.new_empty(w2.shape[0], index.numel()), coords.new_empty(coords.shape[0], w2.shape[0]))


@torch.library.custom_op("mmn_b200::cpb_bias_bwd", mutates_args=())
def cpb_bias_bwd(dbias: Tensor, coords: Tensor, w1: Tensor, b1: Tensor, w2: Tensor, index: Tensor,
                 tab16: Tensor) -> Tuple[Tensor, Tensor, Tensor]:
    _require_cuda(dbias, coords, w1, b1, w2, index, tab16)
    T, n_in, J, nH, NN = coords.shape[0], coords.shape[1], w1.shape[0], w2.shape[0], index.numel()
    dbias = dbias.contiguous()
    dw1, db1, dw2 = torch.empty_like(w1), torch.empty_like(b1), torch.empty_like(w2)
    scratch = torch.empty(T, nH, dtype=torch.float32, device=coords.device)
    perm, offsets = _inverse_index(index, T) if _deterministic() else (None, None)
    _lib.check(_lib.load().mmn_cpb_bias_bwd(_ptr(coords), _ptr(w1), _ptr(b1), _ptr(w2), _ptr(index), _ptr(perm), _ptr(offsets),
                                           _ptr(tab16), _ptr(dbias),
                                           T, n_in, J, nH, NN, _ptr(scratch), _ptr(dw1), _ptr(db1), _ptr(dw2),
                                           coords.device.index, _stream(coords)), "mmn_cpb_bias_bwd")
    return dw1, db1, dw2


@cpb_bias_bwd.register_fake
def _(dbias, coords, w1, b1, w2, index, tab16):
    return torch.empty_like(w1), torch.empty_like(b1), torch.empty_like(w2)


def _cpb_setup(ctx, inputs, output):
    coords, w1, b1, w2, index = inputs
    ctx.save_for_backward(coords, w1, b1, w2, index, output[1])


def _cpb_backward(ctx, dbias, _dtab16):
    coords, w1, b1, w2, index, tab16 = ctx.saved_tensors
    dw1, db1, dw2 = torch.ops.mmn_b200.cpb_bias_bwd(dbias, coords, w1, b1, w2, index, tab16)
    return None, dw1, db1, dw2, None


cpb_bias_fwd.register_autograd(_cpb_backward, setup_context=_cpb_setup)


_ACT = {"none": _lib.ACT_NONE, "relu": _lib.ACT_RELU, "gelu": _lib.ACT_GELU}


def _rows2d(t: Tensor) -> bool:
    return t.dim() == 2 and t.stride(1) == 1 and t.is_cuda and t.dtype == torch.bfloat16


def linear_supported(x: Tensor, w: Tensor) -> bool:
    if not (_rows2d(x) and w.is_cuda and w.dtype == torch.bfloat16 and w.dim() == 2 and w.is_contiguous()) or x.shape[0] < 1:
        return False
    return bool(_lib.load().mmn_linear_supported(_lib.DT_BF16, x.shape[0], x.shape[1], w.shape[0], x.stride(0), w.shape[0]))


@torch.library.custom_op("mmn_b200::linear_fwd", mutates_args=())
def linear_fwd(x: Tensor, w: Tensor, bias: Optional[Tensor], act: int, want_pre: bool) -> Tuple[Tensor, Tensor]:
    _require_cuda(x, w, bias)
    if not _rows2d(x) or w.dtype != torch.bfloat16 or not w.is_contiguous():
        raise RuntimeError("linear_fwd expects bf16 x (rows, in) with contiguous columns and a contiguous bf16 weight")
    if bias is not None and (bias.dtype != torch.float32 or not bias.is_contiguous()):
        raise RuntimeError("linear_fwd takes its bias in float32")
    rows, n_in, n_out = x.shape[0], x.shape[1], w.shape[0]
    y = torch.empty(rows, n_out, dtype=x.dtype, device=x.device)
    pre = torch.empty(rows, n_out, dtype=x.dtype, device=x.device) if want_pre else x.new_empty(0)
    with _timed("linear_fwd", x):
        _lib.check(_lib.load().mmn_linear_fwd(_ptr(x), _ptr(w), _ptr(bias), _ptr(y), _ptr(pre) if want_pre else None, act,
                                              _lib.DT_BF16, rows, n_in, n_out, x.stride(0), n_out, x.device.index, _stream(x)),
                   "mmn_linear_fwd")
    return y, pre


@linear_fwd.register_fake
def _(x, w, bias, act, want_pre):
    return x.new_empty(x.shape[0], w.shape[0]), (x.new_empty(x.shape[0], w.shape[0]) if want_pre else x.new_empty(0))


def linear_bwd_supported(dy: Tensor, x: Tensor, w: Tensor) -> bool:
    if not (_rows2d(dy) and _rows2d(x) and w.is_cuda and w.dtype == torch.bfloat16 and w.is_contiguous()) or dy.shape[0] < 1:
        return False
    return bool(_lib.load().mmn_linear_bwd_supported(_lib.DT_BF16, dy.shape[0], x.shape[1], dy.shape[1], dy.stride(0),
                                                     x.stride(0), x.shape[1]))


@torch.library.custom_op("mmn_b200::linear_bwd", mutates_args=())
def linear_bwd(dy: Tensor, x: Tensor, w: Tensor, act_aux: Optional[Tensor] = None, act: int = 0, want_dx: bool = True,
               want_dw: bool = True) -> Tuple[Tensor, Tensor, Tensor]:
    _require_cuda(dy, x, w, act_aux)
    lib = _lib.load()
    rows, n_out, n_in = dy.shape[0], dy.shape[1], x.shape[1]
    dx = torch.empty(rows, n_in, dtype=dy.dtype, device=dy.device) if want_dx else dy.new_empty(0)
    dw = torch.empty(n_out, n_in, dtype=torch.float32, device=dy.device) if want_dw else dy.new_empty(0, dtype=torch.float32)
    db = torch.empty(n_out, dtype=torch.float32, device=dy.device) if want_dw else dy.new_empty(0, dtype=torch.float32)
    det = _deterministic()
    ws = torch.empty(lib.mmn_linear_bwd_workspace_bytes(rows, n_in, n_out, int(det)), dtype=torch.uint8, device=dy.device)
    if act_aux is not None and (not _rows2d(act_aux) or act_aux.shape != (rows, n_in)):
        raise RuntimeError("act_aux must be a bf16 (rows, in) tensor with contiguous columns")
    with _timed("linear_bwd", dy):
        _lib.check(lib.mmn_linear_bwd(_ptr(dy), _ptr(x), _ptr(w), _ptr(dx) if want_dx else None, _ptr(dw) if want_dw else None,
                                      _ptr(db) if want_dw else None, _ptr(ws), _ptr(act_aux),
                                      act_aux.stride(0) if act_aux is not None else 0, act if act_aux is not None else 0,
                                      _DT[dy.dtype], rows, n_in, n_out, dy.stride(0), x.stride(0), n_in, int(det), dy.device.index,
                                      _stream(dy)), "mmn_linear_bwd")
    return dx, dw, db


@linear_bwd.register_fake
def _(dy, x, w, act_aux=None, act=0, want_dx=True, want_dw=True):
    f32 = dict(dtype=torch.float32)
    return (dy.new_empty(dy.shape[0], x.shape[1]) if want_dx else dy.new_empty(0),
            dy.new_empty(dy.shape[1], x.shape[1], **f32) if want_dw else dy.new_empty(0, **f32),
            dy.new_empty(dy.shape[1], **f32) if want_dw else dy.new_empty(0, **f32))


class LinearFn(torch.autograd.Function):

    @staticmethod
    def forward(ctx, x, w, b, act):
        x2 = x.reshape(-1, x.shape[-1])
        wc = weight_bf16(w)
        y, pre = torch.ops.mmn_b200.linear_fwd(x2, wc, None if b is None else b.float(), act, act != _lib.ACT_NONE)
        ctx.save_for_backward(x2, wc, pre)
        ctx.meta = (x.shape, w.dtype, None if b is None else b.dtype, act, x.requires_grad)
        return y.view(*x.shape[:-1], w.shape[0])

    @staticmethod
    @torch.autograd.function.once_differentiable
    def backward(ctx, dy):
        x2, wc, pre = ctx.saved_tensors
        shape, wdt, bdt, act, need_dx = ctx.meta
        dy2 = dy.reshape(-1, dy.shape[-1]).to(torch.bfloat16)
        if act != _lib.ACT_NONE:
            dy2 = dy2 * pre
        dx, dw, db = torch.ops.mmn_b200.linear_bwd(dy2.contiguous(), x2, wc, None, 0, need_dx, True)
        return (dx.view(shape) if need_dx else None, dw.to(wdt), db.to(bdt) if bdt is not None else None, None)


def linear(x: Tensor, w: Tensor, b: Optional[Tensor] = None, act: str = "none") -> Tensor:
    x2 = x.reshape(-1, x.shape[-1]) if x.dim() != 2 else x
    if x.is_cuda and x.dtype == torch.bfloat16 and x.numel() > 0 and w.shape[1] % 32 == 0 and w.shape[0] % 32 == 0 and \
            x2.stride(-1) == 1 and x2.stride(0) % 8 == 0 and x2.data_ptr() % 16 == 0:
        return LinearFn.apply(x, w, b, _ACT[act])
    y = torch.nn.functional.linear(x, w.to(x.dtype), None if b is None else b.to(x.dtype))
    return y if act == "none" else (torch.relu(y) if act == "relu" else torch.nn.functional.gelu(y))


_DTC = {torch.float32: _lib.DT_F32, torch.bfloat16: _lib.DT_BF16}
_DTC_INV = {_lib.DT_F32: torch.float32, _lib.DT_BF16: torch.bfloat16}


def layernorm_supported(x: Tensor, cols: int) -> bool:
    return bool(x.is_cuda and x.dtype in _DTC and cols % 2 == 0 and 2 <= cols <= 1536 and x.numel() > 0)


@torch.library.custom_op("mmn_b200::layernorm_fwd", mutates_args=())
def layernorm_fwd(resid: Optional[Tensor], delta: Optional[Tensor], gamma: Tensor, beta: Optional[Tensor], eps: float, mode: int,
                  want_sum: bool, norm_dt: int) -> Tuple[Tensor, Tensor, Tensor, Tensor]:
    _require_cuda(resid, delta, gamma, beta)
    ref = resid if resid is not None else delta
    cols = ref.shape[-1]
    rows = ref.numel() // cols
    for t in (resid, delta):
        if t is not None and (not t.is_contiguous() or t.dtype not in _DTC or t.shape != ref.shape):
            raise RuntimeError("layernorm_fwd expects contiguous float32/bfloat16 tensors of one shape")
    if gamma.dtype != torch.float32 or (beta is not None and beta.dtype != torch.float32):
        raise RuntimeError("layernorm_fwd takes gamma / beta in float32")
    out_sum = torch.empty_like(ref) if want_sum else ref.new_empty(0)
    out_norm = torch.empty(ref.shape, dtype=_DTC_INV[norm_dt], device=ref.device) if norm_dt >= 0 else ref.new_empty(0)
    mean = torch.empty(rows, dtype=torch.float32, device=ref.device)
    rstd = torch.empty(rows, dtype=torch.float32, device=ref.device)
    dt = lambda t: _DTC[t.dtype] if t is not None else 0
    with _timed("layernorm_fwd", ref):
        _lib.check(_lib.load().mmn_layernorm_fwd(_ptr(resid), dt(resid), _ptr(delta), dt(delta), _ptr(gamma), _ptr(beta), eps, mode,
                                                 _ptr(out_sum) if want_sum else None, _DTC[ref.dtype],
                                                 _ptr(out_norm) if norm_dt >= 0 else None, max(norm_dt, 0), _ptr(mean), _ptr(rstd),
                                                 rows, cols, ref.device.index, _stream(ref)), "mmn_layernorm_fwd")
    return out_sum, out_norm, mean, rstd


@layernorm_fwd.register_fake
def _(resid, delta, gamma, beta, eps, mode, want_sum, norm_dt):
    ref = resid if resid is not None else delta
    rows = ref.numel() // ref.shape[-1]
    return (torch.empty_like(ref) if want_sum else ref.new_empty(0),
            ref.new_empty(ref.shape, dtype=_DTC_INV[norm_dt]) if norm_dt >= 0 else ref.new_empty(0),
            ref.new_empty(rows, dtype=torch.float32), ref.new_empty(rows, dtype=torch.float32))


@torch.library.custom_op("mmn_b200::layernorm_bwd", mutates_args=())
def layernorm_bwd(g_sum: Optional[Tensor], g_norm: Optional[Tensor], x: Tensor, gamma: Tensor, mean: Tensor, rstd: Tensor, mode: int,
                  resid_dt: int, delta_dt: int, want_beta: bool) -> Tuple[Tensor, Tensor, Tensor, Tensor]:
    _require_cuda(g_sum, g_norm, x, gamma, mean, rstd)
    cols = x.shape[-1]
    rows = x.numel() // cols
    g_sum = g_sum.contiguous() if g_sum is not None else None
    g_norm = g_norm.contiguous() if g_norm is not None else None
    mk = lambda code: torch.empty(x.shape, dtype=_DTC_INV[code], device=x.device) if code >= 0 else x.new_empty(0)
    d_resid, d_delta = mk(resid_dt), mk(delta_dt)
    dgamma = torch.zeros(cols, dtype=torch.float32, device=x.device)
    dbeta = torch.zeros(cols, dtype=torch.float32, device=x.device) if want_beta else x.new_empty(0, dtype=torch.float32)
    dt = lambda t: _DTC[t.dtype] if t is not None else 0
    lib, det = _lib.load(), _deterministic()
    ws = _workspace(lib.mmn_layernorm_bwd_workspace_bytes(rows, cols), x) if det else None
    with _timed("layernorm_bwd", x):
        _lib.check(lib.mmn_layernorm_bwd(_ptr(g_sum), dt(g_sum), _ptr(g_norm), dt(g_norm), _ptr(x), _DTC[x.dtype], _ptr(gamma),
                                                 _ptr(mean), _ptr(rstd), mode, _ptr(d_resid) if resid_dt >= 0 else None, max(resid_dt, 0),
                                                 _ptr(d_delta) if delta_dt >= 0 else None, max(delta_dt, 0), _ptr(dgamma),
                                                 _ptr(dbeta) if want_beta else None, _ptr(ws), int(det), rows, cols, x.device.index,
                                                 _stream(x)),
                   "mmn_layernorm_bwd")
    return d_resid, d_delta, dgamma, dbeta


@layernorm_bwd.register_fake
def _(g_sum, g_norm, x, gamma, mean, rstd, mode, resid_dt, delta_dt, want_beta):
    mk = lambda code: x.new_empty(x.shape, dtype=_DTC_INV[code]) if code >= 0 else x.new_empty(0)
    return (mk(resid_dt), mk(delta_dt), x.new_empty(x.shape[-1], dtype=torch.float32),
            x.new_empty(x.shape[-1] if want_beta else 0, dtype=torch.float32))


class AddLayerNormFn(torch.autograd.Function):

    @staticmethod
    def forward(ctx, resid, delta, gamma, beta, eps, mode, norm_dtype):
        ref = resid if resid is not None else delta
        want_sum = resid is not None and delta is not None
        g32 = gamma.float()
        b32 = beta.float() if beta is not None else None
        rc = resid.contiguous() if resid is not None else None
        dc = delta.contiguous() if delta is not None else None
        out_sum, out_norm, mean, rstd = torch.ops.mmn_b200.layernorm_fwd(rc, dc, g32, b32, eps, mode, want_sum,
                                                                         _DTC[norm_dtype] if norm_dtype is not None else -1)
        x = (out_sum if want_sum else (rc if rc is not None else dc)) if mode == _lib.LN_PRE else dc
        ctx.save_for_backward(x, g32, mean, rstd)
        ctx.meta = (mode, None if resid is None else resid.dtype, None if delta is None else delta.dtype, gamma.dtype,
                    None if beta is None else beta.dtype, want_sum, norm_dtype is not None)
        ctx.set_materialize_grads(False)
        return (out_sum if want_sum else None), (out_norm if norm_dtype is not None else None)

    @staticmethod
    @torch.autograd.function.once_differentiable
    def backward(ctx, g_sum, g_norm):
        x, g32, mean, rstd = ctx.saved_tensors
        mode, rdt, ddt, gdt, bdt, had_sum, had_norm = ctx.meta
        g_sum = g_sum if had_sum else None
        g_norm = g_norm if had_norm else None
        if g_sum is None and g_norm is None:
            return (None,) * 7
        need_r = rdt is not None and ctx.needs_input_grad[0]
        need_d = ddt is not None and ctx.needs_input_grad[1]
        d_resid, d_delta, dgamma, dbeta = torch.ops.mmn_b200.layernorm_bwd(
            g_sum, g_norm, x, g32, mean, rstd, mode,
            _DTC[rdt] if need_r else -1, _DTC[ddt] if need_d else -1, bdt is not None)
        return (d_resid if need_r else None, d_delta if need_d else None, dgamma.to(gdt), dbeta.to(bdt) if bdt is not None else None,
                None, None, None)


def next_dropout_stream(p: float, training: bool, device) -> Tuple[float, int, int, Optional[Tensor]]:
    if not training or p <= 0.0:
        return 0.0, 0, 0, None
    return float(p), 0, 0, torch.randint(0, 2 ** 62, (2,), dtype=torch.int64, device=device)


def winattn_path_name(a: Tensor, b: Optional[Tensor], grid, window, shift, num_heads, score_kind, mask_kind,
                      dropout_p: float = 0.0) -> str:
    d, _ = _win_desc(a, b, grid, window, shift, num_heads, score_kind, mask_kind, 1, 1.0, dropout_p, 0, 0, _lib.PATH_AUTO)
    return _lib.load().mmn_winattn_path(C.byref(d)).decode()
```

Measured before the change: 265.2.

## Fuse QKV projection into the tcgen05 window-attention forward kernel

Adds a new persistent tcgen05 kernel that computes the QKV projection of each window and runs the attention forward in the same launch, writing both qkv and the output. The aim is to drop the separate projection GEMM launch and its round trip of the qkv activation through memory before attention. It also factors the softmax row and output store into shared helpers and adds an optional swizzle on the bias class table, presumably to cut shared-memory bank conflicts. The fused path is taken only for self-attention in bf16 without dropout on supported shapes; every other case falls back to the old path. The new kernel adds shared-memory pressure and code complexity.

```diff
diff --git a/include/mmn_b200.h b/include/mmn_b200.h
--- a/include/mmn_b200.h
+++ b/include/mmn_b200.h
@@ -8,7 +8,7 @@
 extern "C" {
 #endif
 
-#define MMN_ABI_VERSION 6
+#define MMN_ABI_VERSION 7
 #define MMN_WINATTN_WORK_BYTES 2048
 
 enum { MMN_OK = 0, MMN_ERR_INVALID = -1, MMN_ERR_UNSUPPORTED = -2, MMN_ERR_CUDA = -3 };
@@ -66,6 +66,11 @@
 int mmn_winattn_fwd(const mmn_winattn_desc* desc, const void* q, const void* k, const void* v,
                     const float* bias, const float* head_scale, const float* mask,
                     void* out, float* lse, void* workspace, int device, void* stream);
+
+const char* mmn_winattn_qkv_path(const mmn_winattn_desc* desc, int in_channels);
+int mmn_winattn_qkv_fwd(const mmn_winattn_desc* desc, const void* x, const void* w_qkv, const float* b_qkv,
+                        const float* bias, const float* head_scale, const float* mask,
+                        void* qkv_out, void* out, float* lse, void* workspace, int device, void* stream);
 
 size_t mmn_winattn_bwd_workspace_bytes(const mmn_winattn_desc* desc);
 int mmn_winattn_bwd(const mmn_winattn_desc* desc, const void* q, const void* k, const void* v,
diff --git a/multimodal_neuroimage_b200/_lib.py b/multimodal_neuroimage_b200/_lib.py
--- a/multimodal_neuroimage_b200/_lib.py
+++ b/multimodal_neuroimage_b200/_lib.py
@@ -12,7 +12,7 @@
 LIB_PATH = os.environ.get("MMN_LIB") or os.path.join(PKG_DIR, "libmmn_b200.so")
 SOURCES = {"mmn_abi.cu": ["generic_launch.h", "attn_generic.cuh", "winattn_tc.h", "dropout_rng.cuh", "zero_fill.h"],
            "generic_launch.cu": ["generic_launch.h", "attn_generic.cuh", "dropout_rng.cuh", "zero_fill.h"],
-           "winattn_tc.cu": ["winattn_tc.h", "winattn_tc_fwd.cuh", "winattn_tc_bwd.cuh", "tc_window.cuh", "tc_sched.cuh", "tc_common.cuh",
+           "winattn_tc.cu": ["winattn_tc.h", "winattn_tc_fwd.cuh", "winattn_tc_bwd.cuh", "winattn_tc_qkv_fwd.cuh", "tc_window.cuh", "tc_sched.cuh", "tc_common.cuh",
                              "zero_fill.h"],
            "linbwd_tc.cu": ["winattn_tc.h", "tc_window.cuh", "tc_common.cuh"],
            "gemm_tc.cu": ["winattn_tc.h", "tc_window.cuh", "tc_common.cuh"],
@@ -31,11 +31,11 @@
 PATH_AUTO, PATH_GENERIC, PATH_TCGEN05 = 0, 1, 2
 ACT_NONE, ACT_RELU, ACT_GELU = 0, 1, 2
 LN_PRE, LN_POST = 0, 1
-ABI_VERSION = 6
+ABI_VERSION = 7
 WINATTN_WORK_BYTES = 2048
 
 EXPORTS = ["mmn_abi_version", "mmn_last_error", "mmn_winattn_path", "mmn_mha_path", "mmn_launch_count",
-           "mmn_winattn_fwd", "mmn_winattn_bwd", "mmn_winattn_bwd_workspace_bytes", "mmn_mha_fwd", "mmn_mha_bwd", "mmn_mha_avg_weights",
+           "mmn_winattn_fwd", "mmn_winattn_qkv_path", "mmn_winattn_qkv_fwd", "mmn_winattn_bwd", "mmn_winattn_bwd_workspace_bytes", "mmn_mha_fwd", "mmn_mha_bwd", "mmn_mha_avg_weights",
            "mmn_colsum", "mmn_colsum_workspace_bytes", "mmn_layernorm_bwd_workspace_bytes",
            "mmn_linear_supported", "mmn_linear_fwd", "mmn_linear_bwd", "mmn_linear_bwd_supported", "mmn_linear_bwd_workspace_bytes",
            "mmn_cpb_bias_fwd", "mmn_cpb_bias_bwd", "mmn_table_bias_fwd", "mmn_table_bias_bwd", "mmn_layernorm_supported", "mmn_layernorm_fwd", "mmn_layernorm_bwd"]
@@ -125,6 +125,10 @@
         lib.mmn_mha_path.argtypes = [C.POINTER(MhaDesc)]
         lib.mmn_winattn_fwd.restype = C.c_int
         lib.mmn_winattn_fwd.argtypes = [C.POINTER(WinAttnDesc), vp, vp, vp, fp, fp, fp, vp, fp, vp, C.c_int, vp]
+        lib.mmn_winattn_qkv_path.restype = C.c_char_p
+        lib.mmn_winattn_qkv_path.argtypes = [C.POINTER(WinAttnDesc), C.c_int]
+        lib.mmn_winattn_qkv_fwd.restype = C.c_int
+        lib.mmn_winattn_qkv_fwd.argtypes = [C.POINTER(WinAttnDesc), vp, vp, fp, fp, fp, fp, vp, vp, fp, vp, C.c_int, vp]
         lib.mmn_winattn_bwd_workspace_bytes.restype = C.c_size_t
         lib.mmn_winattn_bwd_workspace_bytes.argtypes = [C.POINTER(WinAttnDesc)]
         lib.mmn_winattn_bwd.restype = C.c_int
diff --git a/multimodal_neuroimage_b200/csrc/mmn_abi.cu b/multimodal_neuroimage_b200/csrc/mmn_abi.cu
--- a/multimodal_neuroimage_b200/csrc/mmn_abi.cu
+++ b/multimodal_neuroimage_b200/csrc/mmn_abi.cu
@@ -164,6 +164,33 @@
   return finish(e, n, "attn_fwd_generic");
 }
 
+const char* mmn_winattn_qkv_path(const mmn_winattn_desc* d, int in_channels) {
+  if (validate_win(d) != MMN_OK) return "invalid";
+  if (d->path == MMN_PATH_GENERIC) return "generic path requested";
+  const char* why = mmn::tc::qkv_fwd_why_not(d, in_channels);
+  return why ? why : "tcgen05-fused";
+}
+
+int mmn_winattn_qkv_fwd(const mmn_winattn_desc* d, const void* x, const void* w_qkv, const float* b_qkv, const float* bias,
+                        const float* head_scale, const float* mask, void* qkv_out, void* out, float* lse, void* workspace,
+                        int device, void* stream) {
+  int rc = validate_win(d);
+  if (rc) return rc;
+  if (!x || !w_qkv || !qkv_out || !out || !lse || !workspace) return fail(MMN_ERR_INVALID, "null tensor pointer");
+  if (d->score_kind == MMN_SCORE_COSINE && !head_scale) return fail(MMN_ERR_INVALID, "cosine attention needs head_scale");
+  if (d->mask_kind == MMN_MASK_TENSOR && !mask) return fail(MMN_ERR_INVALID, "MMN_MASK_TENSOR needs a mask");
+  if (!have_device()) return fail(MMN_ERR_CUDA, "no CUDA device: libmmn_b200 has no CPU path");
+  if (d->path == MMN_PATH_GENERIC) return fail(MMN_ERR_UNSUPPORTED, "the fused qkv forward has no generic path");
+  if (const char* why = mmn::tc::qkv_fwd_why_not(d, d->num_heads * d->head_dim))
+    return fail(MMN_ERR_UNSUPPORTED, "shape not supported by the fused qkv forward: %s", why);
+  DeviceGuard g(device);
+  if (!g.ok) return fail(MMN_ERR_CUDA, "cannot select device %d", device);
+  rc = mmn::tc::winattn_qkv_fwd(d, x, w_qkv, b_qkv, bias, head_scale, mask, qkv_out, out, lse, workspace, (cudaStream_t)stream,
+                                g_err, sizeof(g_err));
+  if (rc == MMN_OK) g_launches.fetch_add(1, std::memory_order_relaxed);
+  return rc;
+}
+
 size_t mmn_winattn_bwd_workspace_bytes(const mmn_winattn_desc* d) {
   if (validate_win(d) != MMN_OK) return 0;
   const mmn::GenericProblem P = problem_from(d, nullptr, nullptr, nullptr);
diff --git a/multimodal_neuroimage_b200/csrc/tc_sched.cuh b/multimodal_neuroimage_b200/csrc/tc_sched.cuh
--- a/multimodal_neuroimage_b200/csrc/tc_sched.cuh
+++ b/multimodal_neuroimage_b200/csrc/tc_sched.cuh
@@ -161,7 +161,7 @@
 }
 
 __device__ __forceinline__ void build_class_table(float* tbl, int ld, const float* bias, const uint8_t* pos, const uint8_t* rid,
-                                                  bool shift_mask, int t, int nthreads) {
+                                                  bool shift_mask, int t, int nthreads, int swz = 0) {
   for (int e0 = t; e0 < kN * kN; e0 += 8 * nthreads) {
     float v[8];
 #pragma unroll
@@ -175,7 +175,7 @@
       if (e < kN * kN) {
         const int i = e >> 6, j = e & 63;
         if (shift_mask && rid[pos[i]] != rid[pos[j]]) v[u] -= 100.f;
-        tbl[i * ld + j] = v[u] * 1.4426950408889634f;
+        tbl[i * ld + ((((j >> 2) ^ (i & swz)) << 2) | (j & 3))] = v[u] * 1.4426950408889634f;
       }
     }
   }
diff --git a/multimodal_neuroimage_b200/csrc/winattn_tc.cu b/multimodal_neuroimage_b200/csrc/winattn_tc.cu
--- a/multimodal_neuroimage_b200/csrc/winattn_tc.cu
+++ b/multimodal_neuroimage_b200/csrc/winattn_tc.cu
@@ -1,6 +1,7 @@
 #include "winattn_tc.h"
 
 #include "winattn_tc_bwd.cuh"
+#include "winattn_tc_qkv_fwd.cuh"
 
 namespace mmn { namespace tc {
 
@@ -84,4 +85,11 @@
 
 size_t bwd_det_workspace_bytes(const mmn_winattn_desc* d) { return bwd_det_workspace_bytes_impl(d); }
 
+const char* qkv_fwd_why_not(const mmn_winattn_desc* d, int in_channels) { return qkv_fwd_why_not_impl(d, in_channels); }
+
+int winattn_qkv_fwd(const mmn_winattn_desc* d, const void* x, const void* w, const float* b, const float* bias, const float* head_scale,
+                    const float* mask, void* qkv, void* out, float* lse, void* workspace, cudaStream_t st, char* err, size_t errlen) {
+  return winattn_qkv_fwd_launch(d, x, w, b, bias, head_scale, mask, qkv, out, lse, workspace, st, err, errlen);
+}
+
 }}
diff --git a/multimodal_neuroimage_b200/csrc/winattn_tc.h b/multimodal_neuroimage_b200/csrc/winattn_tc.h
--- a/multimodal_neuroimage_b200/csrc/winattn_tc.h
+++ b/multimodal_neuroimage_b200/csrc/winattn_tc.h
@@ -14,6 +14,9 @@
                 const float* head_scale, const float* mask, const void* out, const float* lse, const void* dout, void* dq,
                 void* dk, void* dv, float* dbias, float* dhead_scale, float* dcolsum, float* workspace, cudaStream_t st,
                 char* err, size_t errlen, int* launches);
+const char* qkv_fwd_why_not(const mmn_winattn_desc* d, int in_channels);
+int winattn_qkv_fwd(const mmn_winattn_desc* d, const void* x, const void* w, const float* b, const float* bias, const float* head_scale,
+                    const float* mask, void* qkv, void* out, float* lse, void* workspace, cudaStream_t st, char* err, size_t errlen);
 size_t bwd_det_workspace_bytes(const mmn_winattn_desc* d);
 const char* linbwd_why_not(int io_dtype, long long rows, int in_features, int out_features, long long ld_dy, long long ld_x, long long ld_dx);
 size_t linbwd_workspace_bytes(int out_features);
diff --git a/multimodal_neuroimage_b200/csrc/winattn_tc_fwd.cuh b/multimodal_neuroimage_b200/csrc/winattn_tc_fwd.cuh
--- a/multimodal_neuroimage_b200/csrc/winattn_tc_fwd.cuh
+++ b/multimodal_neuroimage_b200/csrc/winattn_tc_fwd.cuh
@@ -62,22 +62,94 @@
 }
 __device__ __forceinline__ void trace_evf(const TraceCfg& trace, int role, int item, int ev) { trace_ev(trace, role, item, ev); }
 
-__device__ __forceinline__ float row_sumsq(const uint8_t* rowp, int row) {
-  const int sw = (row >> 1) & 3;
+__device__ __forceinline__ float sumsq_bf16x32(const uint32_t (&u)[16]) {
   uint64_t ss[4] = {0ull, 0ull, 0ull, 0ull};
 #pragma unroll
-  for (int c = 0; c < 4; ++c) {
-    const uint4 a = *reinterpret_cast<const uint4*>(rowp + ((c ^ sw) << 4));
-    const uint32_t u[4] = {a.x, a.y, a.z, a.w};
+  for (int c = 0; c < 4; ++c)
 #pragma unroll
     for (int e = 0; e < 4; ++e) {
-      const uint64_t x = pk2u(u[e] << 16, u[e] & 0xffff0000u);
+      const uint64_t x = pk2u(u[4 * c + e] << 16, u[4 * c + e] & 0xffff0000u);
       ss[c] = fma2(x, x, ss[c]);
     }
-  }
   float lo, hi;
   upk2(add2(add2(ss[0], ss[1]), add2(ss[2], ss[3])), lo, hi);
   return lo + hi;
+}
+
+__device__ __forceinline__ float row_sumsq(const uint8_t* rowp, int row) {
+  const int sw = (row >> 1) & 3;
+  uint32_t u[16];
+#pragma unroll
+  for (int c = 0; c < 4; ++c) {
+    const uint4 a = *reinterpret_cast<const uint4*>(rowp + ((c ^ sw) << 4));
+    u[4 * c] = a.x; u[4 * c + 1] = a.y; u[4 * c + 2] = a.z; u[4 * c + 3] = a.w;
+  }
+  return sumsq_bf16x32(u);
+}
+
+template <bool COS, int MASK, int TSWZ>
+__device__ __forceinline__ void softmax_row(uint64_t (&s2)[32], const float* trow_f, int row, const float* krow_f, const float* mrow,
+                                            float a_i, bool valid, uint32_t (&pp)[32], float& mx, float& l) {
+  {
+    const float4* trow = reinterpret_cast<const float4*>(trow_f);
+    const float4* krow = reinterpret_cast<const float4*>(krow_f);
+    const uint64_t a2 = pk2(a_i, a_i);
+#pragma unroll
+    for (int j4 = 0; j4 < 16; ++j4) {
+      float4 tt = trow[j4 ^ (row & TSWZ)];
+      if (MASK == MMN_MASK_TENSOR) {
+        const float4 mm = __ldg(reinterpret_cast<const float4*>(mrow) + j4);
+        tt.x = fmaf(mm.x, kLog2e, tt.x); tt.y = fmaf(mm.y, kLog2e, tt.y); tt.z = fmaf(mm.z, kLog2e, tt.z); tt.w = fmaf(mm.w, kLog2e, tt.w);
+      }
+      if (COS) {
+        const float4 kv = krow[j4];
+        s2[j4 * 2 + 0] = fma2(s2[j4 * 2 + 0], mul2(pk2(kv.x, kv.y), a2), pk2(tt.x, tt.y));
+        s2[j4 * 2 + 1] = fma2(s2[j4 * 2 + 1], mul2(pk2(kv.z, kv.w), a2), pk2(tt.z, tt.w));
+      } else {
+        s2[j4 * 2 + 0] = fma2(s2[j4 * 2 + 0], a2, pk2(tt.x, tt.y));
+        s2[j4 * 2 + 1] = fma2(s2[j4 * 2 + 1], a2, pk2(tt.z, tt.w));
+      }
+    }
+  }
+  {
+    float m8[8];
+#pragma unroll
+    for (int j = 0; j < 4; ++j) upk2(s2[j], m8[2 * j], m8[2 * j + 1]);
+#pragma unroll
+    for (int j = 4; j < 32; j += 2) {
+      float a, b, c, d;
+      upk2(s2[j], a, b); upk2(s2[j + 1], c, d);
+      const int ch = (j >> 1) & 7;
+      m8[ch] = fmaxf(fmaxf(m8[ch], a), b);
+      m8[(ch + 4) & 7] = fmaxf(fmaxf(m8[(ch + 4) & 7], c), d);
+    }
+    mx = fmaxf(fmaxf(fmaxf(m8[0], m8[1]), fmaxf(m8[2], m8[3])), fmaxf(fmaxf(m8[4], m8[5]), fmaxf(m8[6], m8[7])));
+  }
+  {
+    const uint64_t nmx2 = pk2(-mx, -mx);
+    uint64_t l2[4] = {0ull, 0ull, 0ull, 0ull};
+#pragma unroll
+    for (int j = 0; j < 32; ++j) {
+      float a, b;
+      upk2(add2(s2[j], nmx2), a, b);
+      a = fast_exp2(a); b = fast_exp2(b);
+      l2[j & 3] = add2(l2[j & 3], pk2(a, b));
+      pp[j] = valid ? pack_bf16x2(a, b) : 0u;
+    }
+    float la, lb;
+    upk2(add2(add2(l2[0], l2[1]), add2(l2[2], l2[3])), la, lb);
+    l = la + lb;
+  }
+}
+
+__device__ __forceinline__ void o_row_to_smem(const uint32_t (&oraw)[32], float inv_l, uint8_t* obuf, int r) {
+  const uint64_t inv2 = pk2(inv_l, inv_l);
+#pragma unroll
+  for (int c = 0; c < 4; ++c) {
+    uint4 v4 = make_uint4(pack_bf16x2(mul2(pk2u(oraw[c * 8 + 0], oraw[c * 8 + 1]), inv2)), pack_bf16x2(mul2(pk2u(oraw[c * 8 + 2], oraw[c * 8 + 3]), inv2)),
+                          pack_bf16x2(mul2(pk2u(oraw[c * 8 + 4], oraw[c * 8 + 5]), inv2)), pack_bf16x2(mul2(pk2u(oraw[c * 8 + 6], oraw[c * 8 + 7]), inv2)));
+    *reinterpret_cast<uint4*>(obuf + ((c ^ ((r >> 1) & 3)) << 4)) = v4;
+  }
 }
 
 template <bool COS, int MASK>
@@ -365,60 +437,11 @@
         for (int j = 0; j < 16; ++j) { s2[j] = pk2u(raw0[2 * j], raw0[2 * j + 1]); s2[16 + j] = pk2u(raw1[2 * j], raw1[2 * j + 1]); }
       }
       TR(n, 4);
-      {
-        const float4* trow = reinterpret_cast<const float4*>(tbl + i * kTblLd);
-        const float4* krow = reinterpret_cast<const float4*>(rkbuf + slot * 64);
-        const float* mrow = (MASK == MMN_MASK_TENSOR) ? P.mask + ((size_t)(gw % P.mask_windows) * kN + ipos) * kN : nullptr;
-        const uint64_t a2 = pk2(a_i, a_i);
-#pragma unroll
-        for (int j4 = 0; j4 < 16; ++j4) {
-          float4 tt = trow[j4];
-          if (MASK == MMN_MASK_TENSOR) {
-            const float4 mm = __ldg(reinterpret_cast<const float4*>(mrow) + j4);
-            tt.x = fmaf(mm.x, kLog2e, tt.x); tt.y = fmaf(mm.y, kLog2e, tt.y); tt.z = fmaf(mm.z, kLog2e, tt.z); tt.w = fmaf(mm.w, kLog2e, tt.w);
-          }
-          if (COS) {
-            const float4 kv = krow[j4];
-            s2[j4 * 2 + 0] = fma2(s2[j4 * 2 + 0], mul2(pk2(kv.x, kv.y), a2), pk2(tt.x, tt.y));
-            s2[j4 * 2 + 1] = fma2(s2[j4 * 2 + 1], mul2(pk2(kv.z, kv.w), a2), pk2(tt.z, tt.w));
-          } else {
-            s2[j4 * 2 + 0] = fma2(s2[j4 * 2 + 0], a2, pk2(tt.x, tt.y));
-            s2[j4 * 2 + 1] = fma2(s2[j4 * 2 + 1], a2, pk2(tt.z, tt.w));
-          }
-        }
-      }
-      float mx;
-      {
-        float m8[8];
-#pragma unroll
-        for (int j = 0; j < 4; ++j) upk2(s2[j], m8[2 * j], m8[2 * j + 1]);
-#pragma unroll
-        for (int j = 4; j < 32; j += 2) {
-          float a, b, c, d;
-          upk2(s2[j], a, b); upk2(s2[j + 1], c, d);
-          const int ch = (j >> 1) & 7;
-          m8[ch] = fmaxf(fmaxf(m8[ch], a), b);
-          m8[(ch + 4) & 7] = fmaxf(fmaxf(m8[(ch + 4) & 7], c), d);
-        }
-        mx = fmaxf(fmaxf(fmaxf(m8[0], m8[1]), fmaxf(m8[2], m8[3])), fmaxf(fmaxf(m8[4], m8[5]), fmaxf(m8[6], m8[7])));
-      }
       uint32_t pp[32];
-      float l;
-      {
-        const uint64_t nmx2 = pk2(-mx, -mx);
-        uint64_t l2[4] = {0ull, 0ull, 0ull, 0ull};
-#pragma unroll
-        for (int j = 0; j < 32; ++j) {
-          float a, b;
-          upk2(add2(s2[j], nmx2), a, b);
-          a = fast_exp2(a); b = fast_exp2(b);
-          l2[j & 3] = add2(l2[j & 3], pk2(a, b));
-          pp[j] = valid ? pack_bf16x2(a, b) : 0u;
-        }
-        float la, lb;
-        upk2(add2(add2(l2[0], l2[1]), add2(l2[2], l2[3])), la, lb);
-        l = la + lb;
-      }
+      float mx, l;
+      softmax_row<COS, MASK, 0>(s2, tbl + i * kTblLd, i, rkbuf + slot * 64,
+                                (MASK == MMN_MASK_TENSOR) ? P.mask + ((size_t)(gw % P.mask_windows) * kN + ipos) * kN : nullptr,
+                                a_i, valid, pp, mx, l);
       TR(n, 5);
       tmem_st_32x32b_x32(tP, pp);
       tmem_st_wait();
@@ -440,13 +463,7 @@
       tmem_ld_wait();
       tcgen05_fence_before();
       mbar_wait(&so_free[g], (kk & 1) ^ 1);
-      const uint64_t inv2 = pk2(inv_l, inv_l);
-#pragma unroll
-      for (int c = 0; c < 4; ++c) {
-        uint4 v4 = make_uint4(pack_bf16x2(mul2(pk2u(oraw[c * 8 + 0], oraw[c * 8 + 1]), inv2)), pack_bf16x2(mul2(pk2u(oraw[c * 8 + 2], oraw[c * 8 + 3]), inv2)),
-                              pack_bf16x2(mul2(pk2u(oraw[c * 8 + 4], oraw[c * 8 + 5]), inv2)), pack_bf16x2(mul2(pk2u(oraw[c * 8 + 6], oraw[c * 8 + 7]), inv2)));
-        *reinterpret_cast<uint4*>(obuf + ((c ^ ((r >> 1) & 3)) << 4)) = v4;
-      }
+      o_row_to_smem(oraw, inv_l, obuf, r);
       fence_proxy_async_smem();
       mbar_arrive_warp(&so_ready[g]);
       TR(n, 8);
diff --git a/multimodal_neuroimage_b200/csrc/winattn_tc_qkv_fwd.cuh b/multimodal_neuroimage_b200/csrc/winattn_tc_qkv_fwd.cuh
--- /dev/null
+++ b/multimodal_neuroimage_b200/csrc/winattn_tc_qkv_fwd.cuh
@@ -0,0 +1,448 @@
+#pragma once
+
+#include "winattn_tc_fwd.cuh"
+
+namespace mmn { namespace tc {
+
+constexpr int kQkvHeads = kGroupsF;
+constexpr int kQkvC = kQkvHeads * kD;
+constexpr int kXPanel = 128 * 64;
+constexpr int kXStage = (kQkvC / 32) * kXPanel;
+constexpr int kXStages = 2;
+constexpr int kWPanel = 96 * 64;
+constexpr int kWHead = (kQkvC / 32) * kWPanel;
+constexpr int kWBytes = kQkvHeads * kWHead;
+constexpr int kOpTile = 128 * 64;
+constexpr int kOpSet = 3 * kOpTile;
+constexpr int kQkvBars = 2 * kXStages + 8 * kGroupsF;
+constexpr size_t kQkvSmemBytes = 1024  + kWBytes + kXStages * kXStage + kGroupsF * kOpSet + kGroupsF * kN * kN * 4 +
+                                 kGroupsF * 128 * 4 + 1024 + kItemRing * 48 + 16 + kQkvBars * 8 + 8;
+static_assert(kQkvSmemBytes <= 227 * 1024, "fused qkv forward: shared memory over the 227 KB a block may use");
+static_assert(kGroupsF * kTmemGroup <= kTmemColsF && 96 <= 128, "fused qkv forward: TMEM columns");
+
+struct QkvFwdParams {
+  CUtensorMap x[3][8];
+  CUtensorMap q[8], k[8], v[8], o[8];
+  WinShape S;
+  Sched sc;
+  int mask_windows;
+  float scale;
+  const __nv_bfloat16* w;
+  const float* b;
+  const float* bias;
+  const float* head_scale;
+  const float* mask;
+  float* lse;
+  long long slab;
+  int* work;
+};
+
+__device__ __forceinline__ void tmem_st_zero_x32(uint32_t taddr) {
+  const uint32_t z = 0u;
+  asm volatile(
+      "tcgen05.st.sync.aligned.32x32b.x32.b32 [%0], "
+      "{%1, %1, %1, %1, %1, %1, %1, %1, %1, %1, %1, %1, %1, %1, %1, %1, "
+      "%1, %1, %1, %1, %1, %1, %1, %1, %1, %1, %1, %1, %1, %1, %1, %1};" ::"r"(taddr), "r"(z)
+      : "memory");
+}
+
+template <bool COS, int MASK>
+__global__ void __launch_bounds__(kFwdThreads, 1)
+winattn_qkv_fwd_tc_kernel(const __grid_constant__ QkvFwdParams P) {
+  constexpr int G = kGroupsF;
+  extern __shared__ uint8_t smem_raw[];
+  uint8_t* smem = smem_raw + ((1024u - (smem_u32(smem_raw) & 1023u)) & 1023u);
+  uint8_t* sW = smem;
+  uint8_t* sX = sW + kWBytes;
+  uint8_t* sOp = sX + kXStages * kXStage;
+  float* sTbl = reinterpret_cast<float*>(sOp + G * kOpSet);
+  float* sRk = sTbl + G * kN * kN;
+  uint8_t* sPos = reinterpret_cast<uint8_t*>(sRk + G * 128);
+  uint8_t* sRid = sPos + 512;
+  int4* sItem = reinterpret_cast<int4*>(sRid + 512);
+  int4* sGeo = sItem + kItemRing;
+  int* sEnd = reinterpret_cast<int*>(sGeo + 2 * kItemRing);
+  uint64_t* bars = reinterpret_cast<uint64_t*>(sEnd + 4);
+  uint64_t* x_full = bars;
+  uint64_t* x_empty = x_full + kXStages;
+  uint64_t* proj_full = x_empty + kXStages;
+  uint64_t* tiles_full = proj_full + G;
+  uint64_t* s_full = tiles_full + G;
+  uint64_t* p_full = s_full + G;
+  uint64_t* o_full = p_full + G;
+  uint64_t* qkv_free = o_full + G;
+  uint64_t* so_ready = qkv_free + G;
+  uint64_t* so_free = so_ready + G;
+  uint32_t* tmem_slot = reinterpret_cast<uint32_t*>(so_free + G);
+
+  const WinShape& S = P.S;
+  const Sched& sc = P.sc;
+  const int tid = threadIdx.x, warp = tid >> 5, lane = tid & 31;
+
+  for (int e = tid; e < kWBytes / 16; e += kFwdThreads) {
+    const int c = e & 3, j = (e >> 2) % 96, hp = (e >> 2) / 96;
+    const int hh = hp / 3, p = hp - hh * 3;
+    const int row = (j >> 5) * kQkvC + hh * kD + (j & 31);
+    const uint4 v = __ldg(reinterpret_cast<const uint4*>(P.w + (size_t)row * kQkvC + p * 32 + c * 8));
+    *reinterpret_cast<uint4*>(sW + hp * kWPanel + j * 64 + ((c ^ ((j >> 1) & 3)) << 4)) = v;
+  }
+  for (int i = tid; i < (kXStages * kXStage) / 16; i += kFwdThreads) reinterpret_cast<uint4*>(sX)[i] = make_uint4(0, 0, 0, 0);
+  for (int i = tid; i < 512; i += kFwdThreads) {
+    sPos[i] = (uint8_t)piece_position(S, i >> 6, i & 63);
+    sRid[i] = (uint8_t)class_region_id(S, i >> 6, i & 63);
+  }
+  if (tid == 0) {
+    for (int g = 0; g < G; ++g) sEnd[g] = 0x7fffffff;
+    for (int s = 0; s < kXStages; ++s) { mbar_init(&x_full[s], 1); mbar_init(&x_empty[s], 1); }
+    for (int g = 0; g < G; ++g) {
+      mbar_init(&proj_full[g], 2); mbar_init(&tiles_full[g], kGroupThreads / 32); mbar_init(&s_full[g], 1);
+      mbar_init(&p_full[g], kGroupThreads / 32); mbar_init(&o_full[g], 1); mbar_init(&qkv_free[g], 1);
+      mbar_init(&so_ready[g], kGroupThreads / 32); mbar_init(&so_free[g], 1);
+    }
+    fence_barrier_init();
+  }
+  if (warp == kProducerWarp && lane == 0)
+    for (int i = 0; i < 8; ++i) { tma_prefetch_desc(&P.x[0][i]); tma_prefetch_desc(&P.x[1][i]); tma_prefetch_desc(&P.x[2][i]); }
+  if (warp == kProducerWarpKV && lane == 0)
+    for (int i = 0; i < 8; ++i) { tma_prefetch_desc(&P.q[i]); tma_prefetch_desc(&P.k[i]); tma_prefetch_desc(&P.v[i]); }
+  if (warp == kStoreWarp && lane == 0)
+    for (int i = 0; i < 8; ++i) tma_prefetch_desc(&P.o[i]);
+  if (warp == kMmaWarp) tmem_alloc<kTmemColsF>(tmem_slot);
+  fence_proxy_async_smem();
+  tcgen05_fence_before();
+  __syncthreads();
+  tcgen05_fence_after();
+  const uint32_t tmem = *tmem_slot;
+
+  if (warp >= kProducerWarp) {
+    setmaxnreg_dec<kRegAuxF>();
+    if (warp == kProducerWarp) {
+      const CUtensorMap* const maps[3] = {P.x[0], P.x[1], P.x[2]};
+      const int dst_base[3] = {0, kXPanel, 2 * kXPanel};
+      const int slot_stride[3] = {kWinBytes, kWinBytes, kWinBytes};
+      BoxPlan<3> plan;
+      int n = 0;
+      ClassQueue wq;
+      const int chunk = max(1, min(kChunkF, sc.n_items / ((int)gridDim.x * 8)));
+      wq.init(sc, sched_range_begin(sc, blockIdx.x, gridDim.x), P.work, chunk, lane);
+      for (int c0, m; wq.next(sc, P.work, chunk, lane, c0, m);) {
+        ItemCursor cur;
+        cur.seek(sc, c0);
+        for (int t = 0; t < m; ++t, ++n, cur.next_item(sc)) {
+          const int stage = n % kXStages, phase = (n / kXStages) & 1;
+          if (cur.cls != plan.cls) plan.build(S, cur.cls, lane, maps, dst_base, slot_stride);
+          const int nvalid = cur.slot_valid(1) ? 2 : 1;
+          int w0, w1;
+          const WinStart ws0 = cursor_start(S, cur, 0, w0), ws1 = cursor_start(S, cur, 1, w1);
+          mbar_wait(&x_empty[stage], phase ^ 1);
+          if (lane == 0) {
+            sItem[n % kItemRing] = make_int4(cur.cls, w0, w1, nvalid);
+            sGeo[(n % kItemRing) * 2] = make_int4(ws0.b, ws0.s0, ws0.s1, ws0.s2);
+            sGeo[(n % kItemRing) * 2 + 1] = make_int4(ws1.b, ws1.s0, ws1.s1, ws1.s2);
+            mbar_arrive_expect_tx(&x_full[stage], nvalid * 3 * kWinBytes);
+          }
+          __syncwarp();
+          plan.issue<true>(S, ws0, ws1, nvalid, 0, sX + stage * kXStage, &x_full[stage], lane);
+        }
+      }
+      const int stage = n % kXStages, phase = (n / kXStages) & 1;
+      mbar_wait(&x_empty[stage], phase ^ 1);
+      if (lane == 0) {
+        sItem[n % kItemRing] = make_int4(-1, 0, 0, 0);
+        mbar_arrive(&x_full[stage]);
+      }
+      __syncwarp();
+    } else if (warp == kMmaWarp) {
+      constexpr uint32_t idescX = umma_idesc_bf16(128, 96, 0, 0);
+      constexpr uint32_t idescS = umma_idesc_bf16(128, 128, 0, 0);
+      constexpr uint32_t idescO = umma_idesc_bf16(128, 32, 0, 1);
+      const uint64_t dK = umma_smem_desc(0, 0, 512, kSwz64);
+      const uint64_t dV = umma_smem_desc(0, 8192, 512, kSwz64);
+      const uint32_t x0 = smem_u32(sX) >> 4, w0 = smem_u32(sW) >> 4, op0 = smem_u32(sOp) >> 4;
+      int total = 0x7fffffff;
+      int nj = 0, ns = 0, np = 0;
+      uint32_t idle = 0;
+      while (np < total) {
+        bool progressed = false;
+        if (total == 0x7fffffff && nj < np + G) {
+          const int pr = nj / G, h = nj - pr * G, xs = pr % kXStages;
+          if ((h != 0 || mbar_test(&x_full[xs], (pr / kXStages) & 1)) && (nj < G || mbar_test(&o_full[h], (pr - 1) & 1))) {
+            progressed = true;
+            if (h == 0 && sItem[pr % kItemRing].x < 0) {
+              total = nj;
+            } else {
+              tcgen05_fence_after();
+              if (elect_one()) {
+                const uint64_t ax = dK + (x0 + xs * (kXStage >> 4)), bw = dK + (w0 + h * (kWHead >> 4));
+#pragma unroll
+                for (int ks = 0; ks < 6; ++ks)
+                  umma_bf16_ss(tmem + h * kTmemGroup, ax + ((ks >> 1) * (kXPanel >> 4) + (ks & 1) * 2),
+                               bw + ((ks >> 1) * (kWPanel >> 4) + (ks & 1) * 2), idescX, ks);
+                umma_commit(&proj_full[h]);
+                if (h == G - 1) umma_commit(&x_empty[xs]);
+                mbar_arrive(&proj_full[h]);
+              }
+              __syncwarp();
+              ++nj;
+            }
+          }
+        }
+        if (ns < nj) {
+          const int g = ns % G;
+          if (mbar_test(&tiles_full[g], (ns / G) & 1)) {
+            progressed = true;
+            tcgen05_fence_after();
+            if (elect_one()) {
+              const uint64_t aq = dK + (op0 + g * (kOpSet >> 4)), bk = aq + (kOpTile >> 4);
+              umma_bf16_ss(tmem + g * kTmemGroup, aq, bk, idescS, 0);
+              umma_bf16_ss(tmem + g * kTmemGroup, aq + 2, bk + 2, idescS, 1);
+              umma_commit(&s_full[g]);
+            }
+            __syncwarp();
+            ++ns;
+          }
+        }
+        if (np < ns) {
+          const int g = np % G;
+          if (mbar_test(&p_full[g], (np / G) & 1)) {
+            progressed = true;
+            tcgen05_fence_after();
+            if (elect_one()) {
+              const uint32_t tP = tmem + g * kTmemGroup, tO = tP + 128;
+              const uint64_t bv = dV + (op0 + g * (kOpSet >> 4) + ((2 * kOpTile) >> 4));
+#pragma unroll
+              for (int ks = 0; ks < 8; ++ks) umma_bf16_ts(tO, tP + ks * 8, bv + ks * (1024 >> 4), idescO, ks);
+              umma_commit(&o_full[g]);
+            }
+            __syncwarp();
+            ++np;
+          }
+        }
+        if (progressed) idle = 0;
+        else if (++idle > (1u << 24)) __trap();
+      }
+      if (elect_one())
+        for (int g = 0; g < G; ++g) { mbar_arrive(&proj_full[g]); mbar_arrive(&proj_full[g]); }
+      __syncwarp();
+    } else if (warp == kStoreWarp) {
+      const CUtensorMap* const maps[1] = {P.o};
+      const int dst_base[1] = {0};
+      const int slot_stride[1] = {kWinBytes};
+      BoxPlan<1> plan;
+      int n = 0;
+      for (;; ++n) {
+        const int g = n % G, kk = n / G;
+        mbar_wait(&so_ready[g], kk & 1);
+        if (kk >= *reinterpret_cast<volatile int*>(&sEnd[g])) break;
+        const int4 item = sItem[kk % kItemRing], a0 = sGeo[(kk % kItemRing) * 2], a1 = sGeo[(kk % kItemRing) * 2 + 1];
+        if (item.x != plan.cls) plan.build(S, item.x, lane, maps, dst_base, slot_stride);
+        WinStart ws0, ws1;
+        ws0.b = a0.x; ws0.s0 = a0.y; ws0.s1 = a0.z; ws0.s2 = a0.w;
+        ws1.b = a1.x; ws1.s0 = a1.y; ws1.s1 = a1.z; ws1.s2 = a1.w;
+        plan.issue<false>(S, ws0, ws1, item.w, g * kD, sOp + g * kOpSet, nullptr, lane);
+        tma_store_commit();
+        tma_store_wait_read<0>();
+        __syncwarp();
+        if (lane == 0) mbar_arrive(&so_free[g]);
+      }
+      tma_store_wait_all<0>();
+    } else {
+      const CUtensorMap* const maps[3] = {P.q, P.k, P.v};
+      const int dst_base[3] = {0, kOpTile, 2 * kOpTile};
+      const int slot_stride[3] = {kWinBytes, kWinBytes, kWinBytes};
+      BoxPlan<3> plan;
+      for (int n = 0;; ++n) {
+        const int g = n % G, kk = n / G;
+        mbar_wait(&tiles_full[g], kk & 1);
+        const int4 item = sItem[kk % kItemRing], a0 = sGeo[(kk % kItemRing) * 2], a1 = sGeo[(kk % kItemRing) * 2 + 1];
+        if (item.x < 0) break;
+        if (item.x != plan.cls) plan.build(S, item.x, lane, maps, dst_base, slot_stride);
+        WinStart ws0, ws1;
+        ws0.b = a0.x; ws0.s0 = a0.y; ws0.s1 = a0.z; ws0.s2 = a0.w;
+        ws1.b = a1.x; ws1.s0 = a1.y; ws1.s1 = a1.z; ws1.s2 = a1.w;
+        plan.issue<false>(S, ws0, ws1, item.w, g * kD, sOp + g * kOpSet, nullptr, lane);
+        tma_store_commit();
+        tma_store_wait_read<0>();
+        __syncwarp();
+        if (lane == 0) mbar_arrive(&qkv_free[g]);
+      }
+      tma_store_wait_all<0>();
+    }
+  } else {
+    setmaxnreg_inc<kRegSoftmaxF>();
+    const int g = warp >> 2, h = g;
+    const int r = tid & 127;
+    const int slot = r >> 6, i = r & 63;
+    const uint32_t lane_base = (uint32_t)((warp & 3) * 32) << 16;
+    const uint32_t tG = tmem + lane_base + g * kTmemGroup;
+    const float hscale = COS ? __ldg(P.head_scale + h) * kLog2e : P.scale * kLog2e;
+    float* tbl = sTbl + g * kN * kN;
+    float* rkbuf = sRk + g * 128;
+    uint8_t* tiles = sOp + g * kOpSet;
+    const int rsw = (r >> 1) & 3;
+    const float* bias_h = P.bias ? P.bias + (size_t)h * kN * kN : nullptr;
+
+    int cls_loaded = -1;
+    int kk = 0;
+    for (;; ++kk) {
+      mbar_wait(&proj_full[g], kk & 1);
+      const int4 item = sItem[kk % kItemRing];
+      if (item.x < 0) break;
+      tcgen05_fence_after();
+      const int cls = item.x, gw = slot ? item.z : item.y;
+      const bool valid = slot < item.w;
+      if (cls != cls_loaded) {
+        named_bar_sync(1 + g, kGroupThreads);
+        build_class_table(tbl, kN, bias_h, sPos + cls * 64, sRid + cls * 64, MASK == MMN_MASK_SHIFT && cls != 0, r, kGroupThreads, 7);
+        cls_loaded = cls;
+      }
+      const int ipos = sPos[cls * 64 + i];
+      const int gwh = gw * kQkvHeads + h;
+
+      mbar_wait(&so_free[g], (kk & 1) ^ 1);
+      float ssq = 0.f, ssk = 0.f;
+#pragma unroll
+      for (int t = 0; t < 3; ++t) {
+        uint32_t raw[32];
+        tmem_ld_32x32b_x32(tG + t * 32, raw);
+        tmem_ld_wait();
+        uint32_t u[16];
+        if (P.b) {
+          const float4* bp = reinterpret_cast<const float4*>(P.b + t * kQkvC + h * kD);
+#pragma unroll
+          for (int j = 0; j < 8; ++j) {
+            const float4 b4 = __ldg(bp + j);
+            u[2 * j] = pack_bf16x2(__uint_as_float(raw[4 * j]) + b4.x, __uint_as_float(raw[4 * j + 1]) + b4.y);
+            u[2 * j + 1] = pack_bf16x2(__uint_as_float(raw[4 * j + 2]) + b4.z, __uint_as_float(raw[4 * j + 3]) + b4.w);
+          }
+        } else {
+#pragma unroll
+          for (int j = 0; j < 16; ++j) u[j] = pack_bf16x2(__uint_as_float(raw[2 * j]), __uint_as_float(raw[2 * j + 1]));
+        }
+        uint8_t* row = tiles + t * kOpTile + r * 64;
+#pragma unroll
+        for (int c = 0; c < 4; ++c)
+          *reinterpret_cast<uint4*>(row + ((c ^ rsw) << 4)) = make_uint4(u[4 * c], u[4 * c + 1], u[4 * c + 2], u[4 * c + 3]);
+        if (COS && t == 0) ssq = sumsq_bf16x32(u);
+        if (COS && t == 1) ssk = sumsq_bf16x32(u);
+      }
+      tcgen05_fence_before();
+      fence_proxy_async_smem();
+      mbar_arrive_warp(&tiles_full[g]);
+      float a_i = hscale;
+      if (COS) {
+        const float rq = rsqrtf(fmaxf(ssq, 1e-24f)), rkk = rsqrtf(fmaxf(ssk, 1e-24f));
+        a_i *= rq;
+        rkbuf[r] = rkk;
+        if (valid) {
+          float* rec = P.lse + P.slab + (long long)gwh * (3 * kN) + i;
+          rec[0] = rq;
+          rec[kN] = rkk;
+        }
+      }
+      named_bar_sync(1 + g, kGroupThreads);
+
+      mbar_wait(&s_full[g], kk & 1);
+      tcgen05_fence_after();
+      uint64_t s2[32];
+      {
+        uint32_t raw0[32], raw1[32];
+        tmem_ld_32x32b_x32(tG + slot * 64, raw0);
+        tmem_ld_32x32b_x32(tG + slot * 64 + 32, raw1);
+        tmem_ld_wait();
+#pragma unroll
+        for (int j = 0; j < 16; ++j) { s2[j] = pk2u(raw0[2 * j], raw0[2 * j + 1]); s2[16 + j] = pk2u(raw1[2 * j], raw1[2 * j + 1]); }
+      }
+      uint32_t pp[32];
+      float mx, l;
+      softmax_row<COS, MASK, 7>(s2, tbl + i * kN, i, rkbuf + slot * 64,
+                                (MASK == MMN_MASK_TENSOR) ? P.mask + ((size_t)(gw % P.mask_windows) * kN + ipos) * kN : nullptr,
+                                a_i, valid, pp, mx, l);
+      tmem_st_32x32b_x32(tG + slot * 32, pp);
+      tmem_st_zero_x32(tG + (slot ^ 1) * 32);
+      tmem_st_wait();
+      tcgen05_fence_before();
+      mbar_arrive_warp(&p_full[g]);
+
+      const float lse2 = mx + __log2f(l), inv_l = __frcp_rn(l);
+      if (valid) {
+        P.lse[(long long)gwh * kN + ipos] = lse2 * kLn2;
+        P.lse[P.slab + (long long)gwh * (3 * kN) + 2 * kN + i] = lse2;
+      }
+
+      mbar_wait(&o_full[g], kk & 1);
+      tcgen05_fence_after();
+      uint32_t oraw[32];
+      tmem_ld_32x32b_x32(tG + 128, oraw);
+      tmem_ld_wait();
+      tcgen05_fence_before();
+      mbar_wait(&qkv_free[g], kk & 1);
+      o_row_to_smem(oraw, inv_l, tiles + r * 64, r);
+      fence_proxy_async_smem();
+      mbar_arrive_warp(&so_ready[g]);
+    }
+    mbar_arrive_warp(&tiles_full[g]);
+    if (kk > 0) mbar_wait(&so_free[g], (kk - 1) & 1);
+    if (r == 0) sEnd[g] = kk;
+    mbar_arrive_warp(&so_ready[g]);
+  }
+
+  tcgen05_fence_before();
+  __syncthreads();
+  if (warp == kMmaWarp) tmem_dealloc<kTmemColsF>(tmem);
+}
+
+inline const char* qkv_fwd_why_not_impl(const mmn_winattn_desc* d, int in_channels) {
+  if (d->num_heads != kQkvHeads || d->head_dim != kD) return "the fused qkv kernel is built for 3 heads of 32 channels (C = 96)";
+  if (in_channels != kQkvC) return "input channels differ from the attention width";
+  return fwd_why_not_impl(d);
+}
+
+inline int winattn_qkv_fwd_launch(const mmn_winattn_desc* d, const void* x, const void* w, const float* b, const float* bias,
+                                  const float* head_scale, const float* mask, void* qkv, void* out, float* lse, void* workspace,
+                                  cudaStream_t st, char* err, size_t errlen) {
+  QkvFwdParams P;
+  P.S = shape_from(d);
+  P.sc = make_sched(P.S, d->batch, false);
+  const char* xb = static_cast<const char*>(x);
+  char* qb = static_cast<char*>(qkv);
+  bool ok = reinterpret_cast<uintptr_t>(w) % 16 == 0;
+  for (int p = 0; p < 3; ++p) ok = ok && make_window_maps(P.x[p], xb + p * kD * 2, kQkvC, d->batch, kD, P.S);
+  ok = ok && make_window_maps(P.q, qb, 3 * kQkvC, d->batch, kQkvC, P.S) &&
+       make_window_maps(P.k, qb + kQkvC * 2, 3 * kQkvC, d->batch, kQkvC, P.S) &&
+       make_window_maps(P.v, qb + 2 * kQkvC * 2, 3 * kQkvC, d->batch, kQkvC, P.S) &&
+       make_window_maps(P.o, out, kQkvC, d->batch, kQkvC, P.S);
+  if (!ok) {
+    snprintf(err, errlen, "cuTensorMapEncodeTiled failed (pointer alignment or strides)");
+    return MMN_ERR_CUDA;
+  }
+  P.mask_windows = d->mask_windows > 0 ? d->mask_windows : 1;
+  P.scale = d->scale;
+  P.w = static_cast<const __nv_bfloat16*>(w); P.b = b;
+  P.bias = bias; P.head_scale = head_scale; P.mask = mask; P.lse = lse;
+  P.slab = (long long)P.S.n_windows * d->num_heads * kN;
+  P.work = arm_work_counters(workspace, st, err, errlen);
+  if (!P.work) return MMN_ERR_CUDA;
+
+  using Kern = void (*)(const QkvFwdParams);
+  static const Kern kernels[2][3] = {
+      {winattn_qkv_fwd_tc_kernel<false, MMN_MASK_NONE>, winattn_qkv_fwd_tc_kernel<false, MMN_MASK_SHIFT>, winattn_qkv_fwd_tc_kernel<false, MMN_MASK_TENSOR>},
+      {winattn_qkv_fwd_tc_kernel<true, MMN_MASK_NONE>, winattn_qkv_fwd_tc_kernel<true, MMN_MASK_SHIFT>, winattn_qkv_fwd_tc_kernel<true, MMN_MASK_TENSOR>}};
+  static std::once_flag once;
+  std::call_once(once, [] {
+    for (int c = 0; c < 2; ++c)
+      for (int m = 0; m < 3; ++m) cudaFuncSetAttribute(kernels[c][m], cudaFuncAttributeMaxDynamicSharedMemorySize, (int)kQkvSmemBytes);
+  });
+  const Kern kern = kernels[d->score_kind == MMN_SCORE_COSINE ? 1 : 0][d->mask_kind];
+  int grid = num_sms_cached();
+  if (grid > P.sc.n_items) grid = P.sc.n_items;
+  kern<<<grid, kFwdThreads, kQkvSmemBytes, st>>>(P);
+  cudaError_t e = cudaGetLastError();
+  if (e != cudaSuccess) {
+    snprintf(err, errlen, "winattn_qkv_fwd_tc_kernel: %s", cudaGetErrorString(e));
+    return MMN_ERR_CUDA;
+  }
+  return MMN_OK;
+}
+
+}}
diff --git a/multimodal_neuroimage_b200/fused.py b/multimodal_neuroimage_b200/fused.py
--- a/multimodal_neuroimage_b200/fused.py
+++ b/multimodal_neuroimage_b200/fused.py
@@ -35,11 +35,18 @@
             xc, yc = cast(x).reshape(B * L, C), (cast(y).reshape(B * L, C) if y is not None else None)
             castw = (lambda t: None if t is None else ops.weight_bf16(t)) if cdt == torch.bfloat16 else cast
             wa, wb, wp = castw(w_a), castw(w_b), castw(w_proj)
-            a = _project(xc, wa, b_a).view(B, *grid, -1)
-            b = _project(yc, wb, b_b).view(B, *grid, -1) if y is not None else None
             p, seed, off, rng = dropout
-            out, lse = torch.ops.mmn_b200.winattn_fwd(a, b, bias, head_scale, None, list(grid), list(window), list(shift),
-                                                      num_heads, score_kind, mask_kind, scale, p, seed, off, path, rng)
+            if y is None and cdt == torch.bfloat16 and xc.is_contiguous() and ops.winattn_qkv_path_name(
+                    (B, *grid, C), cdt, grid, window, shift, num_heads, score_kind, mask_kind, p, path) == "tcgen05-fused":
+                a, out, lse = torch.ops.mmn_b200.winattn_qkv_fwd(
+                    xc.view(B, *grid, C), wa.contiguous(), None if b_a is None else b_a.float().contiguous(), bias,
+                    head_scale, None, list(grid), list(window), list(shift), num_heads, score_kind, mask_kind, scale, path)
+                b = None
+            else:
+                a = _project(xc, wa, b_a).view(B, *grid, -1)
+                b = _project(yc, wb, b_b).view(B, *grid, -1) if y is not None else None
+                out, lse = torch.ops.mmn_b200.winattn_fwd(a, b, bias, head_scale, None, list(grid), list(window), list(shift),
+                                                          num_heads, score_kind, mask_kind, scale, p, seed, off, path, rng)
             res = _project(out.view(B * L, C), wp, b_proj).view(B, L, C).to(odt)
         ctx.save_for_backward(xc, yc, a, b, out, lse, wa, wb, wp, bias, head_scale, rng)
         ctx.cfg = (list(grid), list(window), list(shift), num_heads, score_kind, mask_kind, scale, p, seed, off, path)
diff --git a/multimodal_neuroimage_b200/ops.py b/multimodal_neuroimage_b200/ops.py
--- a/multimodal_neuroimage_b200/ops.py
+++ b/multimodal_neuroimage_b200/ops.py
@@ -199,6 +199,51 @@
         N *= w
         nW *= g // w
     return a.new_empty(*a.shape[:-1], Cc), a.new_empty(4, a.shape[0] * nW, num_heads, N, dtype=torch.float32)
+
+
+@torch.library.custom_op("mmn_b200::winattn_qkv_fwd", mutates_args=())
+def winattn_qkv_fwd(x: Tensor, w: Tensor, b: Optional[Tensor], bias: Optional[Tensor], head_scale: Optional[Tensor],
+                    mask: Optional[Tensor], grid: List[int], window: List[int], shift: List[int], num_heads: int,
+                    score_kind: int, mask_kind: int, scale: float, path: int) -> Tuple[Tensor, Tensor, Tensor]:
+    _require_cuda(x, w, b, bias, head_scale, mask)
+    Cc = x.shape[-1]
+    if x.dtype != torch.bfloat16 or w.dtype != torch.bfloat16 or not x.is_contiguous() or not w.is_contiguous() \
+            or tuple(w.shape) != (3 * Cc, Cc):
+        raise RuntimeError("winattn_qkv_fwd expects contiguous bf16 x (..., C) and w (3C, C)")
+    if b is not None and (b.dtype != torch.float32 or not b.is_contiguous() or b.numel() != 3 * Cc):
+        raise RuntimeError("winattn_qkv_fwd takes its qkv bias as a contiguous float32 (3C) tensor")
+    if tuple(x.shape[1:-1]) != tuple(grid):
+        raise RuntimeError(f"tensor grid {tuple(x.shape[1:-1])} != geometry {tuple(grid)}")
+    for t in (bias, head_scale, mask):
+        if t is not None and (t.dtype != torch.float32 or not t.is_contiguous()):
+            raise RuntimeError("bias / head_scale / mask must be contiguous float32")
+    qkv = torch.empty(*x.shape[:-1], 3 * Cc, dtype=x.dtype, device=x.device)
+    d, _ = _win_desc(qkv, None, grid, window, shift, num_heads, score_kind, mask_kind,
+                     mask.shape[0] if mask is not None else 0, scale, 0.0, 0, 0, path)
+    d.q_row_stride = d.k_row_stride = d.v_row_stride = 3 * Cc
+    d.o_row_stride = Cc
+    out = torch.empty_like(x)
+    N = nW = 1
+    for g, w_ in zip(grid, window):
+        N *= w_
+        nW *= g // w_
+    lse = torch.empty(4, x.shape[0] * nW, num_heads, N, dtype=torch.float32, device=x.device)
+    work = torch.empty(_lib.WINATTN_WORK_BYTES, dtype=torch.uint8, device=x.device)
+    with _timed("winattn_qkv_fwd", x):
+        _lib.check(_lib.load().mmn_winattn_qkv_fwd(C.byref(d), _ptr(x), _ptr(w), _ptr(b), _ptr(bias), _ptr(head_scale),
+                                                   _ptr(mask), _ptr(qkv), _ptr(out), _ptr(lse), _ptr(work), x.device.index,
+                                                   _stream(x)), "mmn_winattn_qkv_fwd")
+    return qkv, out, lse
+
+
+@winattn_qkv_fwd.register_fake
+def _(x, w, b, bias, head_scale, mask, grid, window, shift, num_heads, score_kind, mask_kind, scale, path):
+    N = nW = 1
+    for g, w_ in zip(grid, window):
+        N *= w_
+        nW *= g // w_
+    return (x.new_empty(*x.shape[:-1], 3 * x.shape[-1]), x.new_empty(x.shape),
+            x.new_empty(4, x.shape[0] * nW, num_heads, N, dtype=torch.float32))
 
 
 @torch.library.custom_op("mmn_b200::winattn_bwd", mutates_args=())
@@ -731,6 +776,15 @@
     return float(p), 0, 0, torch.randint(0, 2 ** 62, (2,), dtype=torch.int64, device=device)
 
 
+def winattn_qkv_path_name(x_shape, dtype, grid, window, shift, num_heads, score_kind, mask_kind, dropout_p: float = 0.0,
+                          path: int = _lib.PATH_AUTO) -> str:
+    a = torch.empty(*x_shape[:-1], 3 * x_shape[-1], dtype=dtype, device="meta")
+    d, Cc = _win_desc(a, None, grid, window, shift, num_heads, score_kind, mask_kind, 1, 1.0, dropout_p, 0, 0, path)
+    d.q_row_stride = d.k_row_stride = d.v_row_stride = 3 * Cc
+    d.o_row_stride = Cc
+    return _lib.load().mmn_winattn_qkv_path(C.byref(d), int(x_shape[-1])).decode()
+
+
 def winattn_path_name(a: Tensor, b: Optional[Tensor], grid, window, shift, num_heads, score_kind, mask_kind,
                       dropout_p: float = 0.0) -> str:
     d, _ = _win_desc(a, b, grid, window, shift, num_heads, score_kind, mask_kind, 1, 1.0, dropout_p, 0, 0, _lib.PATH_AUTO)
```

New measurement: 286.1, median of 6. 7.8% higher.
